# tsubo164/Fujiyama-Renderer

Hardware: AMD Instinct MI355X
Metric: Mray/s primary+secondary (and ms/frame) at 1920x1080 64spp (higher is better)
Workload: dtype f64; 1 GPU; dragon-class scene, 1920x1080, 8x8 spp, tile 32x32, 2040 tiles, 32 point lights; mesh=dragon, parallelism=tiles%1, tile_deal=auto, blas_build=host binned SAH

## Files before the change

### fujiyama-renderer_amd/csrc/device/fjgpu_api.hip

```cpp
#include <hip/hip_runtime.h>
#include <mutex>
#include <map>
#include <dlfcn.h>

#include <algorithm>
#include <array>
#include <cfloat>
#include <cmath>
#include <cstdio>
#include <cstdint>
#include <cstring>
#include <chrono>
#include <functional>
#include <memory>
#include <string>
#include <thread>
#include <vector>

#include "fjgpu.h"
#include "fjgpu_build.h"
#include "fjgpu_denoise.h"
#include "fjgpu_denoise_variance.h"
#include "fjgpu_temporal.h"
#include "fjgpu_kernels.h"
#include "fjgpu_lbvh.h"
#include "fjgpu_light_cone.h"
#include "fjgpu_raysort.h"
#include "fjgpu_tlas.h"

namespace {

thread_local std::string t_last_error;

int fail(int code, const std::string &msg)
{
  t_last_error = msg;
  return code;
}

#define HIP_TRY(expr) do { hipError_t e_ = (expr); if (e_ != hipSuccess) \
  return fail(FJGPU_ENODEV, std::string(#expr) + ": " + hipGetErrorString(e_)); } while (0)

#define FJ_LREC_BUFS 4

struct DeviceBuffers {
  std::vector<void *> ptrs;
  size_t bytes = 0;
  ~DeviceBuffers() { for (void *p : ptrs) (void) hipFree(p); }
  template <class T> int upload(const T *src, size_t n, const T **out)
  {
    *out = nullptr;
    if (n == 0 || src == nullptr) return 0;
    void *d = nullptr;
    if (hipMalloc(&d, n * sizeof(T)) != hipSuccess) return -1;
    ptrs.push_back(d);
    bytes += n * sizeof(T);
    if (hipMemcpy(d, src, n * sizeof(T), hipMemcpyHostToDevice) != hipSuccess) return -1;
    *out = static_cast<const T *>(d);
    return 0;
  }
  template <class T> int alloc(size_t n, T **out)
  {
    void *d = nullptr;
    if (hipMalloc(&d, std::max<size_t>(n, 1) * sizeof(T)) != hipSuccess) return -1;
    ptrs.push_back(d);
    bytes += std::max<size_t>(n, 1) * sizeof(T);
    *out = static_cast<T *>(d);
    return 0;
  }
};

struct Rccl {
  typedef void *comm_t;
  int (*CommInitAll)(comm_t *, int, const int *) = nullptr;
  int (*CommDestroy)(comm_t) = nullptr;
  int (*GroupStart)() = nullptr;
  int (*GroupEnd)() = nullptr;
  int (*Send)(const void *, size_t, int, int, comm_t, hipStream_t) = nullptr;
  int (*Recv)(void *, size_t, int, int, comm_t, hipStream_t) = nullptr;
  const char *(*GetErrorString)(int) = nullptr;
  void *handle = nullptr;
  bool ok = false;
  static constexpr int kFloat = 7;
};

Rccl &rccl()
{
  static Rccl R;
  static std::once_flag once;
  std::call_once(once, []() {
    for (const char *name : {"librccl.so.1", "librccl.so", "/opt/rocm/lib/librccl.so.1"}) { R.handle = dlopen(name, RTLD_NOW | RTLD_LOCAL); if (R.handle) break; }
    if (!R.handle) return;
    auto sym = [&](const char *n) { return dlsym(R.handle, n); };
    R.CommInitAll = (decltype(R.CommInitAll)) sym("ncclCommInitAll");
    R.CommDestroy = (decltype(R.CommDestroy)) sym("ncclCommDestroy");
    R.GroupStart = (decltype(R.GroupStart)) sym("ncclGroupStart");
    R.GroupEnd = (decltype(R.GroupEnd)) sym("ncclGroupEnd");
    R.Send = (decltype(R.Send)) sym("ncclSend");
    R.Recv = (decltype(R.Recv)) sym("ncclRecv");
    R.GetErrorString = (decltype(R.GetErrorString)) sym("ncclGetErrorString");
    R.ok = R.CommInitAll && R.CommDestroy && R.GroupStart && R.GroupEnd && R.Send && R.Recv;
  });
  return R;
}

#define FJ_RCCL_RETRY_CALLS 64
struct RcclSet { std::vector<Rccl::comm_t> comms; std::string why; int calls_since_failure = 0; };
std::mutex g_rccl_mu;
std::map<std::vector<int>, RcclSet> g_rccl_comms;

void rccl_destroy_all()
{
  Rccl &R = rccl();
  std::lock_guard<std::mutex> lock(g_rccl_mu);
  for (auto &kv : g_rccl_comms)
    for (Rccl::comm_t c : kv.second.comms) if (c && R.CommDestroy) (void) R.CommDestroy(c);
  g_rccl_comms.clear();
}

const std::vector<Rccl::comm_t> *rccl_comms(const std::vector<int> &devices, std::string *why)
{
  Rccl &R = rccl();
  if (!R.ok) { *why = "librccl.so not loadable"; return nullptr; }
  std::lock_guard<std::mutex> lock(g_rccl_mu);
  static bool hooked = false;
  if (!hooked) { hooked = true; atexit(rccl_destroy_all); }
  auto it = g_rccl_comms.find(devices);
  if (it != g_rccl_comms.end()) {
    if (!it->second.comms.empty()) return &it->second.comms;
    if (++it->second.calls_since_failure < FJ_RCCL_RETRY_CALLS) { *why = it->second.why + " (remembered)"; return nullptr; }
    g_rccl_comms.erase(it);
  }
  RcclSet set;
  set.comms.assign(devices.size(), nullptr);
  const int e = R.CommInitAll(set.comms.data(), (int) devices.size(), devices.data());
  if (e) { set.why = std::string("ncclCommInitAll: ") + (R.GetErrorString ? R.GetErrorString(e) : "error"); set.comms.clear(); *why = set.why; }
  auto &slot = g_rccl_comms[devices] = set;
  return slot.comms.empty() ? nullptr : &slot.comms;
}

}

struct fjgpu_scene {
  int device;
  DScene S;
  DeviceBuffers mem;
  double cam_fov;
  fj_camera_desc camera;
  int n_light_samples;
  long batch_tiles;
  long batch_samples = 0;
  long aov_batch_samples = 0;
  long render_calls = 0;
  long count_events;
  long light_cones = 1;
  int cone_rows = 0, cone_records = 0;
  long count_all_shadow;
  unsigned long long stack_peak_closest = 0, stack_peak_shadow = 0;
  std::unique_ptr<DeviceBuffers> work;
  size_t work_samples, work_rays;
  double *d_suv;
  uint32_t *d_stk = nullptr;
  float *d_accum;
  double *d_aseen = nullptr, *d_afinal = nullptr;
  uint8_t *d_apstate = nullptr, *d_acells = nullptr;
  const void *a_owner = nullptr;
  size_t a_samples = 0, a_cell_bytes = 0;
  struct Level { DRay *rays; DPath *paths; size_t cap; uint32_t *keys; float *fc; };
  bool has_filter_rays = false;
  std::vector<Level> levels;
  bool uses_sample_uid;
  int max_children;
  bool bounce_diffuse, bounce_reflect, bounce_refract;
  DHit *d_hits;
  DLightRec *d_lrecs[FJ_LREC_BUFS];
  DLightHair *d_lhair[FJ_LREC_BUFS];
  int lrec_bufs = 2;
  long overlap;
  bool overlap_now = false;
  size_t free_cached = 0;
  hipEvent_t ev_frame[2] = {nullptr, nullptr};
  long early_shadow = 0;
  hipStream_t shadow_stream;
  hipStream_t read_stream = nullptr;
  hipEvent_t ev_shaded = nullptr;
  hipEvent_t ev_shadow_done[FJ_LREC_BUFS];
  std::vector<hipEvent_t> ev_pool;
  DShadowRay *d_squeue;
  size_t squeue_rec_bytes = 0;
  size_t squeue_cap;
  uint32_t *d_join = nullptr; size_t join_cap = 0;
  bool split_overflowed = false;
  uint32_t split_kfac = 1;
  bool split_shadow = false;
  DCounters *d_cnt;
  TileDesc *d_tiles;
  double *d_jit, *d_tim;
  size_t tab_len;
  int tiles_cap;
  int stack_need;
  double tri_record_bytes;
  size_t blas_nodes;
  long blas_treelet_passes = 0;
  unsigned long long blas_treelets_changed = 0;
  double blas_sah_cost_initial = 0., blas_sah_cost = 0.;
  size_t squeue_max;
  size_t batch_fit_samples = 0;
  int ray_sort_bits = 0;
  double scene_box[6];
  uint32_t *d_sort[4] = {nullptr, nullptr, nullptr, nullptr};
  void *d_sort_tmp = nullptr; size_t sort_tmp_bytes = 0; size_t sort_cap = 0;
  float *d_frame = nullptr; size_t d_frame_n = 0;
  float *d_slab = nullptr; size_t d_slab_n = 0;
  int32_t *d_rects = nullptr; size_t d_rects_n = 0;
  fjgpu_batch_fn batch_fn = nullptr; void *batch_user = nullptr;
};

static int grow(void **p, size_t *have, size_t want, size_t elem)
{
  if (*have >= want && *p) return 0;
  if (*p) (void) hipFree(*p);
  *p = nullptr; *have = 0;
  if (hipMalloc(p, std::max<size_t>(want, 1) * elem) != hipSuccess) return -1;
  *have = want;
  return 0;
}

#ifndef FJ_OVERLAP_MAX_SAMPLES
#define FJ_OVERLAP_MAX_SAMPLES ((size_t) 24 << 20)
#endif
#ifndef FJ_OVERLAP_CULL_BLOCKS
#define FJ_OVERLAP_CULL_BLOCKS 1
#endif
static int enable_overlap(fjgpu_scene *sc)
{
  if (sc->shadow_stream) return 0;
  int prio_lo = 0, prio_hi = 0;
  if (getenv("FJGPU_OVERLAP_PRIO") && hipDeviceGetStreamPriorityRange(&prio_lo, &prio_hi) == hipSuccess && prio_lo != prio_hi) {
    if (hipStreamCreateWithPriority(&sc->shadow_stream, hipStreamNonBlocking, prio_lo) != hipSuccess) { sc->shadow_stream = nullptr; return -1; }
// ... 124 lines not shown
  for (size_t g = 0; g < hs.groups.size(); g++) if (!build_flat_group(hs, g, max_tris, &flats[g])) return false;
  out->swap(flats);
  return true;
}

static long g_ray_sort = -1;
static long g_ray_sort_min = FJ_RAY_SORT_MIN;
static long g_device_tlas = 1;
static long g_tlas_verify = 0;
static long g_split_shadow = 1;
static long g_compact_squeue = 1;
static long g_flat_groups = 1;
static long g_curve_anyhit = 1;
static long g_inst_lds = 1;
static long g_batch_tiles = 0;
static long g_device_build = -1;
static long g_treelet_passes = 0;
static long g_multi_exchange = 0;
static long g_spec_walk = 1;
static long g_cold_start = 1;
#ifndef FJ_COLD_BATCH_SAMPLES
#define FJ_COLD_BATCH_SAMPLES ((size_t) 16 << 20)
#endif
static long g_cold_batch_samples = (long) FJ_COLD_BATCH_SAMPLES;
static thread_local long g_single_frame = 0;

extern "C" {

int fjgpu_global_option(const char *name, long value)
{
  if (!name) return fail(FJGPU_EINVAL, "bad option call");
  if (std::string(name) == "ray_sort") { g_ray_sort = value < -1 ? -1 : (value > 9 ? 9 : value); return 0; }
  if (std::string(name) == "ray_sort_min") { g_ray_sort_min = value < 1 ? 1 : value; return 0; }
  if (std::string(name) == "device_tlas") { g_device_tlas = value != 0; return 0; }
  if (std::string(name) == "tlas_verify") { g_tlas_verify = value != 0; return 0; }
  if (std::string(name) == "split_shadow") { g_split_shadow = value != 0; return 0; }
  if (std::string(name) == "inst_lds") { g_inst_lds = value != 0; return 0; }
  if (std::string(name) == "curve_anyhit") { g_curve_anyhit = value != 0; return 0; }
  if (std::string(name) == "flat_groups") { g_flat_groups = value < 0 ? 0 : (value > 2 ? 2 : value); return 0; }
  if (std::string(name) == "compact_squeue") { g_compact_squeue = value != 0; return 0; }
  if (std::string(name) == "batch_tiles") { g_batch_tiles = value < 0 ? 0 : value; return 0; }
  if (std::string(name) == "device_build") { g_device_build = value < 0 ? -1 : (value > 2 ? 2 : value); return 0; }
  if (std::string(name) == "blas_treelet_passes") { g_treelet_passes = value < 0 ? 0 : (value > 8 ? 8 : value); return 0; }
  if (std::string(name) == "single_frame_build") { g_single_frame = value != 0; return 0; }
  if (std::string(name) == "speculative_walk") { g_spec_walk = value != 0; return 0; }
  if (std::string(name) == "anyhit_filter_off") { set_anyhit_filter_off(value); return 0; }
  if (std::string(name) == "cold_start") { g_cold_start = value != 0; return 0; }
  if (std::string(name) == "cold_batch_samples") { g_cold_batch_samples = value > 0 ? value : (long) FJ_COLD_BATCH_SAMPLES; return 0; }
  if (std::string(name) == "multi_exchange") { if (value < 0 || value > 1) return fail(FJGPU_EINVAL, "multi_exchange: 0 peer copies, 1 RCCL send / recv"); g_multi_exchange = value; return 0; }
  return fail(FJGPU_EINVAL, std::string("unknown global option ") + name);
}

const char *fjgpu_last_error(void) { return t_last_error.c_str(); }

int fjgpu_device_count(void)
{
  int n = 0;
  if (hipGetDeviceCount(&n) != hipSuccess) return 0;
  return n;
}

int fjgpu_tile_count(const fj_render_desc *render)
{
  if (!render) return 0;
  if (const char *why = bad_tiling(render)) { (void) fail(FJGPU_EINVAL, why); return 0; }
  std::vector<fjgpu::TileRect> t;
  fjgpu::GenerateTiles(*render, &t);
  return (int) t.size();
}

int fjgpu_tile_rect(const fj_render_desc *render, int tile_id, int32_t rect[4])
{
  if (!render || !rect) return fail(FJGPU_EINVAL, "null argument");
  if (const char *why = bad_tiling(render)) return fail(FJGPU_EINVAL, why);
  std::vector<fjgpu::TileRect> t;
  fjgpu::GenerateTiles(*render, &t);
  if (tile_id < 0 || tile_id >= (int) t.size()) return FJGPU_EINVAL;
  rect[0] = t[tile_id].xmin; rect[1] = t[tile_id].ymin; rect[2] = t[tile_id].xmax; rect[3] = t[tile_id].ymax;
  return 0;
}

}

static int upload_scene(const fj_scene_desc *desc, fjgpu::HostScene &hs, int device, fjgpu_scene **out)
{
  *out = nullptr;
  int ndev = 0;
  if (hipGetDeviceCount(&ndev) != hipSuccess || ndev == 0)
    return fail(FJGPU_ENODEV, "no HIP device visible: the fjgpu core has no CPU fallback");
  if (device < 0 || device >= ndev) return fail(FJGPU_EINVAL, "device index out of range");
  HIP_TRY(hipSetDevice(device));

  const auto t_up0 = std::chrono::steady_clock::now();
  auto lap = [&](const char *what) {
    if (getenv("FJGPU_VERBOSE")) { (void) hipDeviceSynchronize(); fprintf(stderr, "fjgpu: upload: %-28s at %.3f s\n", what,
        std::chrono::duration<double>(std::chrono::steady_clock::now() - t_up0).count()); }
  };
  std::unique_ptr<fjgpu_scene> sc(new fjgpu_scene());
  sc->device = device;
  sc->batch_tiles = g_batch_tiles;
  sc->count_events = 0;
  sc->count_all_shadow = 1;
  sc->work_samples = sc->work_rays = 0;
  sc->tab_len = 0;
  sc->overlap = 2;
  sc->shadow_stream = nullptr;
  for (int k = 0; k < FJ_LREC_BUFS; k++) { sc->ev_shadow_done[k] = nullptr; sc->d_lrecs[k] = nullptr; sc->d_lhair[k] = nullptr; }
  if (getenv("FJGPU_EARLY_SHADOW")) sc->early_shadow = atoi(getenv("FJGPU_EARLY_SHADOW"));
  if (const char *e = getenv("FJGPU_OVERLAP")) sc->overlap = std::max(0, std::min(2, atoi(e)));
  DeviceBuffers &M = sc->mem;
  int e = 0;

  std::vector<DPrimSet> dps(hs.primsets.size());
  for (size_t i = 0; i < hs.primsets.size(); i++) {
    const fjgpu::HostPrimSet &h = hs.primsets[i];
    DPrimSet &d = dps[i];
    std::memset(&d, 0, sizeof(d));
    d.type = h.type;
    d.root = h.root;
    d.n_prims = h.n_prims;
    std::memcpy(d.bounds, h.bounds, sizeof(d.bounds));
    for (int k = 0; k < 3; k++) { d.grid_cell[k] = h.grid_cell[k]; d.grid_n[k] = h.grid_n[k]; }
    if (!h.device_build) {
      e |= M.upload(h.nodes.data(), h.nodes.size(), &d.nodes);
      e |= M.upload(h.prim_ids.data(), h.prim_ids.size(), &d.prim_ids);
    }
    if (h.type == FJ_PRIMSET_MESH) {
      const fj_mesh_desc &m = *h.mesh;
      e |= M.upload(m.velocity, m.velocity ? (size_t) m.n_points * 3 : 0, &d.velocity);
      e |= M.upload(m.P, (size_t) m.n_points * 3, &d.P);
      e |= M.upload(m.N, m.N ? (size_t) m.n_points * 3 : 0, &d.N);
      e |= M.upload(m.vertex_N, m.vertex_N ? (size_t) m.n_faces * 9 : 0, &d.vN);
      e |= M.upload(m.uv, m.uv ? (size_t) m.n_points * 2 : 0, &d.uv);
      e |= M.upload(m.indices, (size_t) m.n_faces * 3, &d.indices);
      e |= M.upload(m.face_group, m.face_group ? (size_t) m.n_faces : 0, &d.face_group);
      if (h.device_build) {
        if (e) return fail(FJGPU_ENOMEM, "device allocation / upload failed while creating the scene");
        const auto tb0 = std::chrono::steady_clock::now();
        LbvhOut lo;
        std::string lerr;
        if (LbvhBuildMesh(d.P, d.velocity, d.indices, m.n_faces, m.n_points, h.bounds, h.f32_exact, hs.device_build_quality, hs.device_build_treelet_passes, &lo, &lerr))
          return fail(FJGPU_ENODEV, lerr);
        for (void *p : {(void *) lo.nodes, (void *) lo.prim_ids, (void *) lo.tri_verts, (void *) lo.tri_verts32, (void *) lo.tri_vel})
          if (p) M.ptrs.push_back(p);
        d.nodes = lo.nodes; d.prim_ids = lo.prim_ids; d.root = lo.root;
        d.tri_verts = lo.tri_verts; d.tri_verts32 = lo.tri_verts32; d.tri_vel = lo.tri_vel;
        hs.primsets[i].stack_need = lo.stack_need;
        sc->blas_treelet_passes += lo.treelet_passes; sc->blas_treelets_changed += lo.treelets_changed;
        sc->blas_sah_cost_initial += lo.sah_cost_initial; sc->blas_sah_cost += lo.sah_cost;
        hs.primsets[i].nodes.n = lo.n_nodes;
        if (lo.tri_verts32) hs.primsets[i].tri_verts32.resize(1);
        if (lo.tri_vel) hs.primsets[i].tri_vel.resize(1);
        if (getenv("FJGPU_VERBOSE") && m.n_faces > 100000)
          fprintf(stderr, "fjgpu: device BLAS build of %d triangles: %.3f s, %zu wide nodes\n", m.n_faces,
              std::chrono::duration<double>(std::chrono::steady_clock::now() - tb0).count(), lo.n_nodes);
      } else {
        e |= M.upload(h.tri_verts.data(), h.tri_verts.size(), &d.tri_verts);
        e |= M.upload(h.tri_verts32.data(), h.tri_verts32.size(), &d.tri_verts32);
        e |= M.upload(h.tri_vel.data(), h.tri_vel.size(), &d.tri_vel);
      }
    } else {
      e |= M.upload(h.curve_cp.data(), h.curve_cp.size(), &d.curve_cp);
      e |= M.upload(h.curve_width.data(), h.curve_width.size(), &d.curve_width);
      e |= M.upload(h.curve_Cd.data(), h.curve_Cd.size(), &d.curve_Cd);
      e |= M.upload(h.curve_depth.data(), h.curve_depth.size(), &d.curve_depth);
      e |= M.upload(h.curve_capsule.data(), h.curve_capsule.size(), &d.curve_capsule);
// ... 104 lines not shown
    }
    bool fits = lo != UINTPTR_MAX && lo % 128 == 0 && (hi - lo) / 128 < 0xffffffffull;
    for (size_t i = 0; i < dps.size(); i++) {
      const DPrimSet &P = dps[i];
      if (P.qnodes && (((uintptr_t) P.qnodes - lo) % 128 != 0 || (tris_of(P) - lo) % 128 != 0)) fits = false;
    }
    for (const DPrimSet &P : dps) if (P.qnodes && !P.tri_verts32) fits = false;
    S.blas_base = fits ? (const char *) lo : nullptr;
    if (!fits && lo != UINTPTR_MAX && getenv("FJGPU_VERBOSE"))
      fprintf(stderr, "fjgpu: BLAS arrays span %zu bytes from %p: no 32-bit offsets, the general shadow walk is used\n", (size_t) (hi - lo), (void *) lo);
    std::vector<DAnyInst> ai(hs.instances.size());
    for (size_t i = 0; i < hs.instances.size(); i++) {
      const DInstance &I = hs.instances[i];
      const DPrimSet &P = dps[I.primset];
      DAnyInst &a = ai[i];
      std::memset(&a, 0, sizeof(a));
      std::memcpy(a.Minv, I.Minv, sizeof(a.Minv));
      std::memcpy(a.bounds, P.bounds, sizeof(a.bounds));
      a.root = P.root;
      a.n_prims = (P.qnodes && S.blas_base) ? P.n_prims : 0;
      if (a.n_prims) {
        for (int k = 0; k < 3; k++) { a.qorigin[k] = qgrid[I.primset][k]; a.qcell[k] = qgrid[I.primset][3 + k]; }
        a.node_base = (uint32_t) (((uintptr_t) P.qnodes - lo) / 128);
        a.tri_base = (uint32_t) ((tris_of(P) - lo) / 128);
        a.tris_f32 = P.tri_verts32 ? 1 : 0;
        double bm = 0;
        for (int k = 0; k < 6; k++) bm = std::max(bm, std::fabs(P.bounds[k]));
        a.fbound = std::nextafter((float) bm, INFINITY);
      }
    }
    e |= M.upload(ai.data(), ai.size(), &S.any_insts);
  }
  if (g_device_tlas && e == 0 && !hs.groups.empty()) {
    std::vector<int> mcount(hs.groups.size()), nfirst, ncount;
    for (size_t g = 0; g < hs.groups.size(); g++) mcount[g] = hs.groups[g].n_instances;
    DTNode *d_nodes = nullptr;
    std::string terr;
    if (TlasBuildDevice(S.instances, hs.group_members, hs.group_member_first, mcount, &nfirst, &ncount, &d_nodes, &terr))
      return fail(FJGPU_ENODEV, terr);
    M.ptrs.push_back(d_nodes);
    size_t total = 0;
    for (int c : ncount) total += (size_t) c;
    if (g_tlas_verify) {
      std::vector<DTNode> got(total);
      HIP_TRY(hipMemcpy(got.data(), d_nodes, total * sizeof(DTNode), hipMemcpyDeviceToHost));
      bool same = total == hs.group_nodes.size();
      for (size_t g = 0; same && g < hs.groups.size(); g++) same = nfirst[g] == hs.groups[g].first && ncount[g] == hs.groups[g].count;
      if (same && total) same = std::memcmp(got.data(), hs.group_nodes.data(), total * sizeof(DTNode)) == 0;
      if (!same) return fail(FJGPU_ENODEV, "device TLAS build differs from the host's build");
    }
    std::vector<DGroup> groups = hs.groups;
    for (size_t g = 0; g < groups.size(); g++) { groups[g].first = nfirst[g]; groups[g].count = ncount[g]; }
    e |= M.upload(groups.data(), groups.size(), &S.groups);
    S.group_nodes = d_nodes;
    S.n_group_nodes = (int32_t) total;
  } else {
    e |= M.upload(hs.groups.data(), hs.groups.size(), &S.groups);
    e |= M.upload(hs.group_nodes.data(), hs.group_nodes.size(), &S.group_nodes);
    S.n_group_nodes = (int32_t) hs.group_nodes.size();
  }
  static_assert(sizeof(DInstEntry) == 8 * FJ_INST_LDS_ENTRY_WORDS && sizeof(DTNode) == 56 && sizeof(DGroup) == 64, "LDS copy of the instance level");
  S.curve_anyhit = (g_curve_anyhit && !getenv("FJGPU_NO_CURVE_ANYHIT")) ? 1 : 0;
  S.inst_lds = (g_inst_lds && !getenv("FJGPU_NO_INST_LDS")) ? 1 : 0;
  e |= M.upload(hs.shaders.data(), hs.shaders.size(), &S.shaders);
  e |= M.upload(hs.xforms.data(), hs.xforms.size(), &S.xforms);
  S.cam_xform = nullptr;
  if (!hs.cam_static) e |= M.upload(&hs.cam_xform, 1, &S.cam_xform);
  S.has_motion = hs.xforms.empty() ? 0 : 1;
  for (const auto &ps : hs.primsets) if (!ps.tri_vel.empty() || !ps.curve_vel.empty()) S.has_motion = 1;
  S.multi_shadow_groups = 0;
  for (const DInstance &I : hs.instances) {
    bool gathers = false;
    for (int k = 0; k < I.n_shaders; k++)
      if (I.shaders[k] >= 0 && (hs.shaders[I.shaders[k]].type == FJ_SHADER_PLASTIC || hs.shaders[I.shaders[k]].type == FJ_SHADER_HAIR)) gathers = true;
    if (gathers && I.shadow_target >= 0 && I.shadow_target < (int) hs.groups.size() && hs.groups[I.shadow_target].n_instances > 1)
      S.multi_shadow_groups = 1;
  }
  S.time_tab = nullptr; S.time_start = 0; S.time_end = 0;
  S.lrec_hair = nullptr;
  e |= M.upload(dtex.data(), dtex.size(), &S.textures);
  e |= M.upload(hs.light_samples.data(), hs.light_samples.size(), &S.light_samples);
  e |= M.upload(hs.area_lights.data(), hs.area_lights.size(), &S.area_lights);
  S.light_cones = nullptr; S.cone_rows = nullptr;
  {
    const size_t nl = hs.light_samples.size();
    std::vector<int32_t> rows(hs.groups.size(), -1);
    std::vector<DLightCone> cones;
    for (size_t g = 0; g < hs.groups.size() && nl; g++) {
      if (hs.groups[g].n_instances != 1) continue;
      const size_t at = cones.size();
      cones.resize(at + nl);
      int built = 0;
      double reach = 1e300;
      for (size_t l = 0; l < nl; l++) {
        DLightCone &C = cones[at + l];
        const DLightSample &LS = hs.light_samples[l];
        if (LS.type == FJ_POINT_LIGHT || LS.type == FJ_DOME_LIGHT) light_cone_build(LS.P, hs.groups[g].sbounds, &C);
        else std::memset(&C, 0, sizeof(C));
        if (C.count > 0) { built++; reach = std::min(reach, C.reach); }
      }
      if (!built) { cones.resize(at); continue; }
      for (size_t l = 0; l < nl; l++) cones[at + l].reach = reach;
      rows[g] = (int32_t) (at / nl);
      sc->cone_rows++; sc->cone_records += built;
    }
    if (!cones.empty()) {
      e |= M.upload(cones.data(), cones.size(), &S.light_cones);
      e |= M.upload(rows.data(), rows.size(), &S.cone_rows);
    }
  }
  S.has_area = hs.area_lights.empty() ? 0 : 1;
  if (e) return fail(FJGPU_ENOMEM, "device allocation / upload failed while creating the scene");
  S.n_light_samples = (int) hs.light_samples.size();
  S.n_instances = (int) hs.instances.size();
  S.n_groups = (int) hs.groups.size();
  S.n_primsets = (int) hs.primsets.size();
  int flat_stack_need = 0;
  S.flats = nullptr;
  {
    bool incoherent = false;
    for (int i = 0; i < desc->n_shaders; i++) {
      const fj_shader_desc &sh = desc->shaders[i];
      auto lum = [](const float *c) { return .298912 * c[0] + .586611 * c[1] + .114478 * c[2] > 0.; };
      if (sh.type == FJ_SHADER_GLASS) incoherent = true;
      if (sh.type == FJ_SHADER_PATHTRACING && (lum(sh.diffuse) || (int) lum(sh.reflect) + (int) lum(sh.refract) >= 2)) incoherent = true;
    }
    std::vector<HostFlat> hf;
    const bool flat_fits = S.inst_lds && S.n_instances <= FJ_FLAT_LDS_INSTS;
    const bool flat_wanted = incoherent || g_flat_groups >= 2 || getenv("FJGPU_FLAT_ALL");
    if (flat_wanted && flat_fits && g_flat_groups && !getenv("FJGPU_NO_FLAT") && FJ_CLOSEST_QNODES && build_flat_groups(hs, &hf)) {
      std::vector<DFlat> df(hf.size());
      for (size_t g = 0; g < hf.size() && !e; g++) {
        HostFlat &F = hf[g];
        DFlat &D = df[g];
        std::memset(&D, 0, sizeof(D));
        const DNode *d_nodes = nullptr;
        const size_t n_nodes = std::max<size_t>(1, F.tree.nodes.size());
        e |= M.upload(F.tree.nodes.data(), n_nodes, &d_nodes);
        DNodeQ *q = nullptr;
        if (!e && M.alloc(n_nodes, &q)) e = 1;
        if (!e && launch_quantize_nodes(nullptr, d_nodes, (uint32_t) n_nodes, &F.grid[0], &F.grid[3], q)) e = 1;
        D.nodes = q;
        e |= M.upload(F.refs.data(), F.refs.size(), &D.refs);
        e |= M.upload(F.refbox.data(), F.refbox.size(), &D.refbox);
        for (int a = 0; a < 3; a++) { D.qorigin[a] = F.grid[a]; D.qcell[a] = F.grid[3 + a]; }
        D.root = F.tree.root; D.n_inst = (int32_t) (F.refbox.size() / 6); D.n_prims = F.tree.n_prims;
        flat_stack_need = std::max(flat_stack_need, F.tree.stack_need);
      }
      if (!e) e |= M.upload(df.data(), df.size(), &S.flats);
      if (e) S.flats = nullptr;
      lap("flat groups");
    }
  }
  {
    int need = S.flats ? flat_stack_need : 0;
    for (const auto &ps : hs.primsets) need = std::max(need, ps.stack_need);
    S.stack_overflow = nullptr;
    S.stack_overflow_shadow = nullptr;
    bool any_curves = false;
    for (const auto &ps : hs.primsets) if (ps.type == FJ_PRIMSET_CURVE && ps.n_prims > 0) any_curves = true;
    (void) any_curves;
    const int lds_entries = FJ_STACK_LDS_MIN;
    if (need > lds_entries) {
      const size_t entries = (size_t) (need - lds_entries) * persistent_threads();
      if (M.alloc(entries, &S.stack_overflow) || M.alloc(entries, &S.stack_overflow_shadow)) return fail(FJGPU_ENOMEM, "device allocation failed for the traversal stack overflow area");
    }
    sc->stack_need = need;
    sc->tri_record_bytes = 36; sc->blas_nodes = 0;
    for (const auto &ps : hs.primsets) {
      sc->blas_nodes += ps.nodes.size();
      if (ps.type == FJ_PRIMSET_MESH && ps.n_prims > 0 && ps.tri_verts32.empty()) sc->tri_record_bytes = 72;
    }
    if (getenv("FJGPU_VERBOSE"))
      for (const auto &ps : hs.primsets)
        fprintf(stderr, "fjgpu: primset type %d prims %d nodes %zu binary depth %d stack need %d\n", ps.type, ps.n_prims,
            ps.nodes.size(), ps.max_depth, ps.stack_need);
  }
  S.has_curves = 0;
  S.all_opaque = 1;
  for (const auto &g : hs.groups) if (!g.all_opaque) S.all_opaque = 0;
  S.has_hair = 0;
  for (int i = 0; i < desc->n_shaders; i++) if (desc->shaders[i].type == FJ_SHADER_HAIR) S.has_hair = 1;
  for (const auto &ps : hs.primsets) if (ps.type == FJ_PRIMSET_CURVE && ps.n_prims > 0) S.has_curves = 1;
  S.target_group = hs.target_group;
  std::memcpy(S.cam_M, hs.cam_M, sizeof(S.cam_M));
  S.cam_znear = hs.cam_znear;
  S.cam_zfar = hs.cam_zfar;
  sc->cam_fov = hs.cam_fov;
  sc->camera = desc->camera;
  sc->n_light_samples = S.n_light_samples;
  sc->max_children = 0;
// ... 40 lines not shown
  lap("done");
  *out = sc.release();
  return 0;
}

static int build_host_scene(const fj_scene_desc *desc, fjgpu::HostScene *hs)
{
  std::string err;
  const auto t_build0 = std::chrono::steady_clock::now();
  long device_mode = g_device_build >= 0 ? g_device_build : (g_single_frame ? 1 : 0);
  if (const char *e = getenv("FJGPU_DEVICE_BUILD")) device_mode = std::max(0, std::min(2, atoi(e)));
  const bool device_build = device_mode != 0;
  hs->device_build_quality = device_mode == 2 ? 0 : 1;
  long passes = g_treelet_passes;
  if (const char *e = getenv("FJGPU_TREELET_PASSES")) passes = std::max(0, std::min(8, atoi(e)));
  hs->device_build_treelet_passes = (int) passes;
  const int be = fjgpu::BuildHostScene(desc, hs, &err, device_build);
  if (getenv("FJGPU_VERBOSE"))
    fprintf(stderr, "fjgpu: host scene build (BLAS, transforms, lights) %.3f s\n",
        std::chrono::duration<double>(std::chrono::steady_clock::now() - t_build0).count());
  if (be) return fail(be, err);
  return 0;
}

extern "C" {

int fjgpu_scene_create(const fj_scene_desc *desc, int device, fjgpu_scene **out)
{
  if (!out || !desc) return fail(FJGPU_EINVAL, "null argument");
  *out = nullptr;
  fjgpu::HostScene hs;
  if (const int be = build_host_scene(desc, &hs)) return be;
  return upload_scene(desc, hs, device, out);
}

int fjgpu_scene_create_multi(const fj_scene_desc *desc, const int *devices, int n_devices, fjgpu_scene **out)
{
  if (!out || !desc || !devices || n_devices < 1) return fail(FJGPU_EINVAL, "bad argument");
  for (int k = 0; k < n_devices; k++) out[k] = nullptr;
  fjgpu::HostScene hs;
  if (const int be = build_host_scene(desc, &hs)) return be;
  for (int k = 0; k < n_devices; k++) {
    const int e = upload_scene(desc, hs, devices[k], &out[k]);
    if (e) { for (int j = 0; j < k; j++) { fjgpu_scene_destroy(out[j]); out[j] = nullptr; } return e; }
  }
  return 0;
}

void fjgpu_scene_destroy(fjgpu_scene *scene)
{
  if (!scene) return;
  (void) hipSetDevice(scene->device);
  (void) hipDeviceSynchronize();
  if (getenv("FJGPU_PHASE_STATS")) debug_phase_stats();
  if (scene->shadow_stream) (void) hipStreamDestroy(scene->shadow_stream);
  if (scene->read_stream) (void) hipStreamDestroy(scene->read_stream);
  if (scene->ev_shaded) (void) hipEventDestroy(scene->ev_shaded);
  for (hipEvent_t e : scene->ev_shadow_done) if (e) (void) hipEventDestroy(e);
  for (hipEvent_t e : scene->ev_frame) if (e) (void) hipEventDestroy(e);
  for (hipEvent_t e : scene->ev_pool) (void) hipEventDestroy(e);
  if (scene->d_frame) (void) hipFree(scene->d_frame);
  if (scene->d_slab) (void) hipFree(scene->d_slab);
  if (scene->d_rects) (void) hipFree(scene->d_rects);
  delete scene;
}

int fjgpu_host_instance_level(const fj_scene_desc *desc, int group, int32_t *out_inst, int32_t *out_skip, double *out_box, int cap)
{
  if (!desc || group < 0 || group >= desc->n_groups) return fail(FJGPU_EINVAL, "bad instance-level query");
  fjgpu::HostScene hs;
  std::string err;
  const int e = fjgpu::BuildHostScene(desc, &hs, &err, true);
  if (e) return fail(e, err);
  const DGroup &G = hs.groups[group];
  for (int k = 0; k < G.count && k < cap; k++) {
    const DTNode &nd = hs.group_nodes[G.first + k];
    if (out_inst) out_inst[k] = nd.inst;
    if (out_skip) out_skip[k] = nd.inst < 0 ? nd.skip - G.first : 0;
    if (out_box) std::memcpy(out_box + 6 * (size_t) k, nd.box, sizeof(nd.box));
  }
  return G.count;
}

int fjgpu_scene_query(const fjgpu_scene *scene, const char *name, double *value)
{
  if (!scene || !name || !value) return fail(FJGPU_EINVAL, "bad query call");
  const std::string n(name);
  if (n == "node_record_bytes") { *value = (double) sizeof(DNode); return 0; }
  if (n == "anyhit_node_record_bytes") { *value = (double) sizeof(DNodeQ); return 0; }
  if (n == "tri_record_bytes") { *value = scene->tri_record_bytes; return 0; }
  if (n == "scene_bytes") { *value = (double) scene->mem.bytes; return 0; }
  if (n == "work_bytes") { *value = (double) (scene->work ? scene->work->bytes : 0); return 0; }
  if (n == "stack_need") { *value = scene->stack_need; return 0; }
  if (n == "blas_nodes") { *value = (double) scene->blas_nodes; return 0; }
  if (n == "blas_treelet_passes") { *value = (double) scene->blas_treelet_passes; return 0; }
  if (n == "blas_treelets_changed") { *value = (double) scene->blas_treelets_changed; return 0; }
  if (n == "blas_sah_cost_initial") { *value = scene->blas_sah_cost_initial; return 0; }
  if (n == "blas_sah_cost") { *value = scene->blas_sah_cost; return 0; }
  if (n == "stack_peak") { *value = (double) std::max(scene->stack_peak_closest, scene->stack_peak_shadow); return 0; }
  if (n == "stack_peak_closest") { *value = (double) scene->stack_peak_closest; return 0; }
  if (n == "stack_peak_shadow") { *value = (double) scene->stack_peak_shadow; return 0; }
  if (n == "stack_lds") { *value = FJ_STACK_LDS; return 0; }
  if (n == "stack_lds_anyhit") { *value = FJ_STACK_LDS_ANYHIT; return 0; }
  if (n == "stack_lds_curves") { *value = FJ_STACK_LDS_CURVES; return 0; }
  if (n == "stack_lds_min") { *value = FJ_STACK_LDS_MIN; return 0; }
  if (n == "curve_anyhit") {
    const DScene &S = scene->S;
    *value = (S.has_curves && !S.has_motion && S.all_opaque && S.curve_anyhit && S.inst_lds && S.n_group_nodes <= FJ_INST_LDS_NODES_CURVES &&
              S.n_instances <= FJ_INST_LDS_INSTS_CURVES && S.n_groups <= FJ_INST_LDS_GROUPS_CURVES && FJ_CURVE_QNODES && FJ_CLOSEST_QNODES) ? 1 : 0;
    return 0;
  }
  if (n == "lean_anyhit") { *value = (scene->S.all_opaque && !scene->S.has_curves && !scene->S.has_motion && scene->S.blas_base) ? 1 : 0; return 0; }
  if (n == "closest_kernel") {
    const DScene &S = scene->S;
    const bool flat = !S.has_motion && !S.has_curves && S.flats;
    *value = S.has_motion ? 3 : (S.has_curves ? 2 : (flat ? 4 : (S.incoherent_rays ? 1 : 0)));
    return 0;
  }
  if (n == "closest_node_record_bytes") { *value = (double) ((scene->S.has_motion || (scene->S.has_curves && !FJ_CURVE_QNODES) || !FJ_CLOSEST_QNODES) ? sizeof(DNode) : sizeof(DNodeQ)); return 0; }
  if (n == "light_cone_rows") { *value = scene->cone_rows; return 0; }
  if (n == "light_cone_records") { *value = scene->cone_records; return 0; }
  if (n == "light_cone_verdicts" || n == "light_cone_contradictions") {
    double v = -1, c = -1;
    if (hipSetDevice(scene->device) != hipSuccess || hipDeviceSynchronize() != hipSuccess) return fail(FJGPU_ENODEV, "hipSetDevice / hipDeviceSynchronize");
    light_cone_validate_counts(&v, &c);
    *value = n == "light_cone_verdicts" ? v : c;
    return 0;
  }
  if (n == "has_curves") { *value = scene->S.has_curves; return 0; }
  if (n == "has_motion") { *value = scene->S.has_motion; return 0; }
  return fail(FJGPU_EINVAL, "unknown query " + n);
}

int fjgpu_set_batch_callback(fjgpu_scene *scene, fjgpu_batch_fn fn, void *user)
{
  if (!scene) return fail(FJGPU_EINVAL, "null scene");
  scene->batch_fn = fn; scene->batch_user = fn ? user : nullptr;
  return 0;
}

int fjgpu_dev_rccl_selftest(int device, int n_floats)
{
  int nd = 0;
  if (hipGetDeviceCount(&nd) != hipSuccess || device < 0 || device >= nd) return fail(FJGPU_ENODEV, "no such HIP device");
  if (n_floats < 1) return fail(FJGPU_EINVAL, "bad size");
  HIP_TRY(hipSetDevice(device));
  std::string why;
  const std::vector<Rccl::comm_t> *comms = rccl_comms(std::vector<int>{device}, &why);
  if (!comms) return fail(FJGPU_ENODEV, "RCCL: " + why);
  Rccl &R = rccl();
  DeviceBuffers M;
  std::vector<float> src((size_t) n_floats), got((size_t) n_floats, -1.f);
  for (int i = 0; i < n_floats; i++) src[(size_t) i] = (float) (i % 1013) * .5f;
  const float *d_src = nullptr;
  float *d_dst = nullptr;
  if (M.upload(src.data(), src.size(), &d_src) || M.alloc(src.size(), &d_dst)) return fail(FJGPU_ENOMEM, "device allocation failed");
  HIP_TRY(hipMemset(d_dst, 0xff, sizeof(float) * src.size()));
  int e = R.GroupStart();
  if (!e) e = R.Send(d_src, src.size(), Rccl::kFloat, 0, (*comms)[0], nullptr);
  if (!e) e = R.Recv(d_dst, src.size(), Rccl::kFloat, 0, (*comms)[0], nullptr);
  const int e2 = R.GroupEnd();
  if (e || e2) return fail(FJGPU_ENODEV, std::string("RCCL self exchange: ") + (R.GetErrorString ? R.GetErrorString(e ? e : e2) : "error"));
  HIP_TRY(hipStreamSynchronize(nullptr));
  HIP_TRY(hipMemcpy(got.data(), d_dst, sizeof(float) * got.size(), hipMemcpyDeviceToHost));
  for (size_t i = 0; i < got.size(); i++) if (got[i] != src[i]) return fail(FJGPU_ENODEV, "RCCL self exchange returned other data");
  return 0;
}

int fjgpu_dev_sort_pairs(int device, const uint32_t *keys, int n, int key_bits, uint32_t *keys_out, uint32_t *perm, int repeats, double *sort_ms)
{
  if (n < 0 || key_bits < 1 || key_bits > 32 || (n > 0 && !keys)) return fail(FJGPU_EINVAL, "bad sort call");
  int nd = 0;
  if (hipGetDeviceCount(&nd) != hipSuccess || device < 0 || device >= nd) return fail(FJGPU_ENODEV, "no such HIP device");
  HIP_TRY(hipSetDevice(device));
  if (sort_ms) *sort_ms = 0;
  if (n == 0) return 0;
  DeviceBuffers M;
  const uint32_t *d_keys = nullptr;
  uint32_t *d_out = nullptr, *d_perm = nullptr;
  char *d_tmp = nullptr;
  const size_t tmp_bytes = ray_sort_pairs_temp_bytes((uint32_t) n, key_bits);
  if (M.upload(keys, (size_t) n, &d_keys) || M.alloc((size_t) n, &d_out) || M.alloc((size_t) n, &d_perm) || M.alloc(tmp_bytes, &d_tmp))
    return fail(FJGPU_ENOMEM, "device allocation failed for the sort");
  hipEvent_t e0, e1;
  HIP_TRY(hipEventCreate(&e0));
  HIP_TRY(hipEventCreate(&e1));
  double best = 1e30;
  for (int k = 0; k < std::max(1, repeats); k++) {
    (void) hipEventRecord(e0, nullptr);
    if (ray_sort_pairs(nullptr, d_keys, (uint32_t) n, key_bits, d_out, d_perm, d_tmp, tmp_bytes, keys_out != nullptr)) { (void) hipEventDestroy(e0); (void) hipEventDestroy(e1); return fail(FJGPU_ENODEV, "the sort's launches failed"); }
    (void) hipEventRecord(e1, nullptr);
    if (hipEventSynchronize(e1) != hipSuccess) { (void) hipEventDestroy(e0); (void) hipEventDestroy(e1); return fail(FJGPU_ENODEV, std::string("sort: ") + hipGetErrorString(hipGetLastError())); }
    float ms = 0.f;
    (void) hipEventElapsedTime(&ms, e0, e1);
    best = std::min(best, (double) ms);
  }
  (void) hipEventDestroy(e0); (void) hipEventDestroy(e1);
  if (sort_ms) *sort_ms = best;
  if (keys_out) HIP_TRY(hipMemcpy(keys_out, d_out, sizeof(uint32_t) * (size_t) n, hipMemcpyDeviceToHost));
  if (perm) HIP_TRY(hipMemcpy(perm, d_perm, sizeof(uint32_t) * (size_t) n, hipMemcpyDeviceToHost));
  return 0;
}

int fjgpu_set_option(fjgpu_scene *scene, const char *name, long value)
{
  if (!scene || !name) return fail(FJGPU_EINVAL, "bad option call");
  const std::string n(name);
  if (n == "batch_tiles") { scene->batch_tiles = value; return 0; }
  if (n == "batch_samples") { scene->batch_samples = value < 0 ? 0 : value; return 0; }
  if (n == "aov_batch_samples") { scene->aov_batch_samples = value < 0 ? 0 : value; return 0; }
  if (n == "count_nodes") { scene->count_events = value != 0; return 0; }
  if (n == "count_all_shadow") { scene->count_all_shadow = value != 0; return 0; }
  if (n == "light_cones") { scene->light_cones = value != 0; return 0; }
  if (n == "overlap_shadow") {
    if (value < 0 || value > 2) return fail(FJGPU_EINVAL, "overlap_shadow: 0 off, 1 on, 2 by the batch size");
    scene->overlap = value;
    return 0;
  }
  if (n == "release_work") {
    if (value && scene->work) {
      if (hipSetDevice(scene->device) != hipSuccess) return fail(FJGPU_ENODEV, "hipSetDevice");
      (void) hipDeviceSynchronize();
      scene->work.reset();
      scene->work_samples = scene->work_rays = 0; scene->tiles_cap = 0; scene->lrec_bufs = std::min(scene->lrec_bufs, 2); scene->squeue_rec_bytes = 0;
      scene->sort_cap = 0; scene->a_owner = nullptr; scene->a_samples = 0; scene->a_cell_bytes = 0;
      scene->d_aseen = scene->d_afinal = nullptr; scene->d_apstate = scene->d_acells = nullptr;
      for (auto &L : scene->levels) { L.rays = nullptr; L.paths = nullptr; L.cap = 0; L.keys = nullptr; }
    }
    return 0;
  }
  return fail(FJGPU_EINVAL, "unknown option " + n);
}

}

namespace {

struct BatchTile { fjgpu::TileRect r; int nx, ny; uint32_t offset; };


bool scene_compact_squeue(const DScene &S)
{
  const bool lean = S.all_opaque && !S.has_curves && !S.has_motion && S.blas_base;
  const bool curve_walk = S.has_curves && !S.has_motion && S.all_opaque && S.curve_anyhit && S.inst_lds && S.n_group_nodes <= FJ_INST_LDS_NODES_CURVES &&
      S.n_instances <= FJ_INST_LDS_INSTS_CURVES && S.n_groups <= FJ_INST_LDS_GROUPS_CURVES && FJ_CURVE_QNODES && FJ_CLOSEST_QNODES;
  return (lean || curve_walk) && !S.has_area && g_compact_squeue && !getenv("FJGPU_NO_COMPACT_SQUEUE");
}

int ensure_work(fjgpu_scene *sc, size_t samples, size_t rays, int tiles, size_t tab_len)
{
  const int want_bufs = sc->overlap_now ? FJ_LREC_BUFS : 2;
  const size_t rec_bytes = scene_compact_squeue(sc->S) ? sizeof(DShadowRayC) : sizeof(DShadowRay);
  if (samples > sc->work_samples || rays > sc->work_rays || tiles > sc->tiles_cap || want_bufs > sc->lrec_bufs || rec_bytes > sc->squeue_rec_bytes) {
    samples = std::max(samples, sc->work_samples); rays = std::max(rays, sc->work_rays); tiles = std::max(tiles, sc->tiles_cap);
    const int old_bufs = sc->lrec_bufs;
    sc->lrec_bufs = samples > sc->work_samples ? want_bufs : std::max(sc->lrec_bufs, want_bufs);
    sc->work.reset(new DeviceBuffers());
    sc->sort_cap = 0; sc->a_owner = nullptr; sc->a_samples = 0; sc->a_cell_bytes = 0;
    sc->d_aseen = sc->d_afinal = nullptr; sc->d_apstate = sc->d_acells = nullptr;
    DeviceBuffers &W = *sc->work;
    int e = 0;
    e |= W.alloc(samples * 2, &sc->d_suv);
    sc->d_stk = nullptr;
    if (sc->uses_sample_uid && !sc->S.has_motion && !sc->S.cam_xform) e |= W.alloc(samples * 2, &sc->d_stk);
    e |= W.alloc(samples * 4, &sc->d_accum);
    for (auto &L : sc->levels) { L.rays = nullptr; L.paths = nullptr; L.cap = 0; L.keys = nullptr; }
    e |= W.alloc(rays, &sc->d_hits);
    for (int k = 0; k < sc->lrec_bufs; k++) {
      e |= W.alloc(rays, &sc->d_lrecs[k]);
      sc->d_lhair[k] = nullptr;
      if (sc->S.has_hair) e |= W.alloc(rays, &sc->d_lhair[k]);
    }
    const size_t per_ray = std::max<size_t>(sc->split_shadow ? 16 : 8, std::min<size_t>(64, (size_t) std::max(1, sc->n_light_samples) * (sc->split_shadow ? 2 : 1)));
    const size_t lrec_bound = std::min<size_t>(rays, std::max<size_t>(samples * 4, (size_t) 1 << 16));
    sc->squeue_cap = std::min<size_t>(lrec_bound * per_ray, sc->squeue_max) + 4096 * 1024;
    { char *q = nullptr; e |= W.alloc(sc->squeue_cap * rec_bytes, &q); sc->d_squeue = (DShadowRay *) q; sc->squeue_rec_bytes = e ? 0 : rec_bytes; }
    sc->d_join = nullptr; sc->join_cap = 0;
    if (sc->split_shadow) { sc->join_cap = sc->squeue_cap + 1 + 32 * (persistent_threads() / 64) * 64; e |= W.alloc(sc->join_cap, &sc->d_join); }
    e |= W.alloc(1, &sc->d_cnt);
    e |= W.alloc((size_t) tiles, &sc->d_tiles);
    if (e) { sc->work.reset(); sc->work_samples = sc->work_rays = 0; sc->tiles_cap = 0; sc->lrec_bufs = std::min(old_bufs, 2); sc->squeue_rec_bytes = 0; return -1; }
    sc->work_samples = samples; sc->work_rays = rays; sc->tiles_cap = tiles;
  }
  if (tab_len > sc->tab_len) {
    std::vector<double> draws;
    fjgpu::XorShiftTable(2 * tab_len, &draws);
    if (sc->mem.upload(draws.data(), 2 * tab_len, const_cast<const double **>(&sc->d_jit))) return -1;
    if (sc->mem.upload(draws.data(), tab_len, const_cast<const double **>(&sc->d_tim))) return -1;
    sc->tab_len = tab_len;
  }
  return 0;
}

int ensure_adaptive(fjgpu_scene *sc, size_t samples, size_t cell_bytes)
{
  if (sc->a_owner == sc->work.get() && samples <= sc->a_samples && cell_bytes <= sc->a_cell_bytes) return 0;
  DeviceBuffers &W = *sc->work;
  if (W.alloc(samples * 4, &sc->d_aseen) || W.alloc(samples * 4, &sc->d_afinal) || W.alloc(samples, &sc->d_apstate) ||
      W.alloc(cell_bytes, &sc->d_acells)) { sc->a_owner = nullptr; return -1; }
  sc->a_owner = sc->work.get(); sc->a_samples = samples; sc->a_cell_bytes = cell_bytes;
  return 0;
}

int ensure_level(fjgpu_scene *sc, int level, size_t cap)
{
  fjgpu_scene::Level &L = sc->levels[level];
  if (L.cap >= cap) return 0;
  DeviceBuffers &W = *sc->work;
  if (W.alloc(cap, &L.rays) || W.alloc(cap, &L.paths)) return -1;
  L.keys = nullptr;
  L.fc = nullptr;
  if (sc->has_filter_rays && level >= 1 && W.alloc(cap * 3, &L.fc)) return -1;
  if (sc->ray_sort_bits > 0 && level >= 1 && W.alloc(cap, &L.keys)) return -1;
  L.cap = cap;
  return 0;
}

int ensure_sort(fjgpu_scene *sc, size_t cap)
{
  if (sc->sort_cap >= cap) return 0;
  DeviceBuffers &W = *sc->work;
  sc->d_sort[0] = sc->d_sort[2] = nullptr;
  if (W.alloc(cap, &sc->d_sort[1]) || W.alloc(cap, &sc->d_sort[3])) return -1;
  sc->sort_tmp_bytes = ray_sort_temp_bytes((uint32_t) cap, sc->ray_sort_bits);
  char *tmp = nullptr;
  if (W.alloc(sc->sort_tmp_bytes, &tmp)) return -1;
  sc->d_sort_tmp = tmp;
  sc->sort_cap = cap;
  return 0;
}


}

extern "C" {

static int render_tiles_once(fjgpu_scene *sc, const fj_render_desc *r, const int32_t *tile_ids, int n_tiles,
    float *d_fb, void *hip_stream, fjgpu_stats *stats);

int fjgpu_render_tiles(fjgpu_scene *sc, const fj_render_desc *r, const int32_t *tile_ids, int n_tiles,
    float *d_fb, void *hip_stream, fjgpu_stats *stats)
{
  if (!sc || !r || !d_fb) return fail(FJGPU_EINVAL, "null argument");
  sc->split_overflowed = false;
  int e = render_tiles_once(sc, r, tile_ids, n_tiles, d_fb, hip_stream, stats);
  if (e == FJGPU_ENOMEM && sc->split_overflowed) {
    fprintf(stderr, "fjgpu: shadow queue overflow with rays split per candidate instance: rendering the tiles again without the split, "
        "which stays off for this scene (option split_shadow)\n");
    sc->split_shadow = false;
    e = render_tiles_once(sc, r, tile_ids, n_tiles, d_fb, hip_stream, stats);
  }
  if (!e) sc->render_calls++;
  return e;
}

static int render_tiles_once(fjgpu_scene *sc, const fj_render_desc *r, const int32_t *tile_ids, int n_tiles,
    float *d_fb, void *hip_stream, fjgpu_stats *stats)
{
  const bool adaptive = r->sampler_type == 1;
  if (r->sampler_type != 0 && !adaptive) return fail(FJGPU_EINVAL, "unknown sampler_type");
  if (adaptive && (r->adaptive_max_subdivision < 0 || r->adaptive_max_subdivision > 8 || !(r->adaptive_subdivision_threshold >= 0)))
    return fail(FJGPU_EINVAL, "adaptive_max_subdivision must be in [0, 8] and adaptive_subdivision_threshold >= 0");
  if (const char *why = bad_render(r)) return fail(FJGPU_EINVAL, why);
  HIP_TRY(hipSetDevice(sc->device));
  hipStream_t st = static_cast<hipStream_t>(hip_stream);
  sc->stack_peak_closest = sc->stack_peak_shadow = 0;

  std::vector<fjgpu::TileRect> all;
  fjgpu::GenerateTiles(*r, &all);
  std::vector<int> ids;
  if (tile_ids) ids.assign(tile_ids, tile_ids + n_tiles);
  else for (size_t i = 0; i < all.size(); i++) ids.push_back((int) i);
  for (int id : ids) if (id < 0 || id >= (int) all.size()) return fail(FJGPU_EINVAL, "tile id out of range");

  int margin[2];
  fjgpu::SamplerMargin(*r, margin);
  const int a_div = adaptive ? 1 << r->adaptive_max_subdivision : 1;
  if (adaptive) {
    margin[0] = (int) std::ceil((double) r->filter_w - 1);
    margin[1] = (int) std::ceil((double) r->filter_h - 1);
  }
  const size_t full_tile_samples = adaptive
      ? (size_t) (a_div * (r->tile_w + 2 * margin[0]) + 1) * (size_t) (a_div * (r->tile_h + 2 * margin[1]) + 1)
      : (size_t) (r->rate_x * r->tile_w + 2 * margin[0]) * (r->rate_y * r->tile_h + 2 * margin[1]);

  auto query_free = [&]() {
    size_t free_b = 0, total_b = 0;
    if (hipMemGetInfo(&free_b, &total_b) != hipSuccess) free_b = (size_t) 16 << 30;
    sc->free_cached = free_b + (sc->work ? sc->work->bytes : 0);
  };
  if (!sc->work || sc->free_cached == 0) query_free();
  size_t free_now = sc->free_cached;
  const int deepest = (sc->bounce_diffuse ? std::max(0, r->max_diffuse_depth) : 0) +
      (sc->bounce_reflect ? std::max(0, r->max_reflect_depth) : 0) + (sc->bounce_refract ? std::max(0, r->max_refract_depth) : 0);
  if (sc->levels.size() < (size_t) deepest + 1) sc->levels.resize((size_t) deepest + 1, fjgpu_scene::Level{nullptr, nullptr, 0, nullptr});
  long bt = sc->batch_tiles;
  if (bt <= 0 && sc->batch_samples > 0) bt = std::max<long>(1, (long) ((size_t) sc->batch_samples / full_tile_samples));
  if (bt <= 0 && sc->render_calls == 0 && g_cold_start && !adaptive) {
    static const int on = [] { const char *e = getenv("FJGPU_COLD_START"); return e ? atoi(e) : 1; }();
    if (on) bt = std::max<long>(1, (long) ((size_t) g_cold_batch_samples / full_tile_samples));
  }
  if (bt <= 0) {
    const size_t per_sample = 32 + (size_t) (deepest + 1) * (sizeof(DRay) + sizeof(DPath) + (sc->has_filter_rays ? 12 : 0)) + sizeof(DHit) + 2 * sizeof(DLightRec) + (adaptive ? 72 : 0) +
        ((sc->ray_sort_bits > 0 && deepest >= 1) ? 24 : 0);
    const double share = sc->n_light_samples == 0 ? .6 : .4;
    const size_t target = std::min<size_t>((size_t) 160 << 20, (size_t) (share * (double) free_now) / per_sample);
    bt = std::max<long>(1, (long) (target / full_tile_samples));
  }
  bt = std::min<long>(bt, (long) ids.size());
  bt = std::min<long>(bt, (long) (((size_t) 1 << 31) / full_tile_samples));
  if (sc->batch_fit_samples && full_tile_samples * (size_t) bt > sc->batch_fit_samples) bt = std::max<long>(1, (long) (sc->batch_fit_samples / full_tile_samples));
  if (bt < 1) bt = 1;
  sc->overlap_now = !adaptive && sc->n_light_samples > 0 && (sc->overlap == 1 || (sc->overlap == 2 && deepest >= 1 && full_tile_samples * (size_t) bt <= FJ_OVERLAP_MAX_SAMPLES));
  if (sc->overlap_now && enable_overlap(sc)) sc->overlap_now = false;
  if (!sc->read_stream) {
    if (hipStreamCreateWithFlags(&sc->read_stream, hipStreamNonBlocking) != hipSuccess) sc->read_stream = nullptr;
    else if (hipEventCreateWithFlags(&sc->ev_shaded, hipEventDisableTiming) != hipSuccess) { (void) hipStreamDestroy(sc->read_stream); sc->read_stream = nullptr; sc->ev_shaded = nullptr; }
  }
  sc->squeue_max = std::max<size_t>((size_t) 4 << 20, std::min<size_t>((size_t) 512 << 20, (size_t) (.2 * (double) free_now) / sizeof(DShadowRay)));
  if (sc->n_light_samples == 0) sc->squeue_max = (size_t) 4 << 20;
  if (const char *e = getenv("FJGPU_SQUEUE_M")) sc->squeue_max = (size_t) std::max(1, atoi(e)) << 20;
  size_t cap_samples = 0, cap_rays = 0;
  bool requeried = false;
  for (;;) {
    cap_samples = full_tile_samples * (size_t) bt;
    cap_rays = std::max<size_t>(cap_samples, std::min<size_t>((size_t) 8 << 20, cap_samples * 16)) + 1024;
    if (!requeried && sc->work && (cap_samples > sc->work_samples || cap_rays > sc->work_rays || (int) bt > sc->tiles_cap ||
                                   (sc->overlap_now ? FJ_LREC_BUFS : 2) > sc->lrec_bufs)) {
      requeried = true;
      query_free();
      free_now = sc->free_cached;
      if (!getenv("FJGPU_SQUEUE_M") && sc->n_light_samples != 0)
        sc->squeue_max = std::max<size_t>((size_t) 4 << 20, std::min<size_t>((size_t) 512 << 20, (size_t) (.2 * (double) free_now) / sizeof(DShadowRay)));
    }
    bool ok = ensure_work(sc, cap_samples, cap_rays, (int) bt, full_tile_samples) == 0;
    const bool level0_implicit = !adaptive && sc->S.cam_xform == nullptr && (!sc->uses_sample_uid || !sc->S.has_motion) && !getenv("FJGPU_EXPLICIT_CAMERA_RAYS");
    for (int l = level0_implicit ? 1 : 0; ok && l <= deepest; l++) ok = ensure_level(sc, l, cap_rays) == 0;
    if (ok && sc->ray_sort_bits > 0 && deepest >= 1) ok = ensure_sort(sc, cap_rays) == 0;
    if (ok) break;
    (void) hipGetLastError();
    if (bt == 1) return fail(FJGPU_ENOMEM, "device allocation failed for the wavefront work buffers");
    sc->work.reset(); sc->work_samples = sc->work_rays = 0; sc->tiles_cap = 0; sc->free_cached = 0;
    for (auto &L : sc->levels) { L.rays = nullptr; L.paths = nullptr; L.cap = 0; L.keys = nullptr; }
    sc->a_owner = nullptr; sc->a_samples = 0; sc->a_cell_bytes = 0;
    sc->sort_cap = 0;
    bt = std::max<long>(1, bt / 2);
    sc->batch_fit_samples = full_tile_samples * (size_t) bt;
  }
  const size_t a_cells0_cap = adaptive ? (size_t) bt * (size_t) (r->tile_w + 2 * margin[0]) * (size_t) (r->tile_h + 2 * margin[1]) : 0;
  const size_t a_cell_bytes = a_cells0_cap * (((((size_t) 1) << (2 * (r->adaptive_max_subdivision + 1))) - 1) / 3);
  if (adaptive && a_cells0_cap >= ((size_t) 1 << 32)) return fail(FJGPU_EINVAL, "too many lattice cells per batch: lower the batch_tiles option");
  if (adaptive && ensure_adaptive(sc, cap_samples, a_cell_bytes))
    return fail(FJGPU_ENOMEM, "device allocation failed for the adaptive sampler's buffers");

  DScene S = sc->S;
  const double aspect = r->xres / (double) r->yres;
  S.cam_uv_size[1] = fjgpu::CameraUvSizeY(sc->cam_fov);
  S.cam_uv_size[0] = S.cam_uv_size[1] * aspect;
  S.time_tab = sc->d_tim; S.time_start = r->time_start; S.time_end = r->time_end;
  S.lrec_hair = nullptr;

  GenParams gp;
  gp.rate_x = r->rate_x; gp.rate_y = r->rate_y; gp.margin_x = margin[0]; gp.margin_y = margin[1];
  gp.udelta = 1. / (r->rate_x * r->xres);
  gp.vdelta = 1. / (r->rate_y * r->yres);
  gp.jitter = r->jitter;
  gp.jittered = r->jitter > 0 ? 1 : 0;
  gp.pad = 0;
  ShadeParams shp;
  shp.max_diffuse_depth = r->max_diffuse_depth; shp.max_reflect_depth = r->max_reflect_depth; shp.max_refract_depth = r->max_refract_depth;
  shp.count_all_shadow = (int) sc->count_all_shadow;
  shp.ray_capacity = (uint32_t) cap_rays; shp.light_capacity = (uint32_t) cap_rays;
  shp.fc_in = nullptr; shp.fc_out = nullptr;
  shp.next_keys = nullptr; shp.sort_bits = std::max(1, std::min(9, sc->ray_sort_bits)); shp.pad_ = 0;
  ray_sort_grid(sc->scene_box, shp.sort_bits, shp.sort_lo, shp.sort_scale);
  ShadowParams swp;
  swp.cos_half_pi = std::cos(3.14159265358979323846 / 2.);
  swp.cos_pi = std::cos(3.14159265358979323846);
  swp.pre_resolve = (S.all_opaque && !S.has_curves && !S.has_motion && S.blas_base) ? 1 : 0;
  swp.cast_shadow = r->cast_shadow;
  S.compact_squeue = scene_compact_squeue(S) ? 1 : 0;
  S.pad_cs_ = 0;
  swp.compact = S.compact_squeue;
  swp.light_cones = (sc->light_cones && S.light_cones && S.cone_rows) ? 1 : 0;
  swp.queue_capacity = (uint32_t) sc->squeue_cap;
  swp.join_capacity = (swp.pre_resolve && sc->split_shadow && sc->d_join) ? (uint32_t) sc->join_cap : 0u;
  S.shadow_join = swp.join_capacity ? sc->d_join : nullptr;
  S.shadow_queue_cap = (uint32_t) sc->squeue_cap;
  ResolveParams rp;
  rp.xres = r->xres; rp.yres = r->yres; rp.rate_x = r->rate_x; rp.rate_y = r->rate_y;
  rp.npx_x = r->rate_x + 2 * margin[0]; rp.npx_y = r->rate_y + 2 * margin[1];
  AdaptiveParams ap;
  std::memset(&ap, 0, sizeof(ap));
  if (adaptive) {
    ap.D = r->adaptive_max_subdivision; ap.div = a_div;
    ap.margin_x = margin[0]; ap.margin_y = margin[1];
    ap.udelta = 1. / (a_div * r->xres);
    ap.vdelta = 1. / (a_div * r->yres);
    ap.jitter = r->jitter;
    ap.jittered = r->jitter > 0 ? 1 : 0;
    ap.threshold = (double) r->adaptive_subdivision_threshold;
    ap.ray_capacity = (uint32_t) cap_rays;
    rp.rate_x = rp.rate_y = a_div;
    rp.npx_x = a_div * (1 + 2 * margin[0]) + 1; rp.npx_y = a_div * (1 + 2 * margin[1]) + 1;
  }
  rp.fw = (double) r->filter_w; rp.fh = (double) r->filter_h;

  fjgpu_stats acc;
  std::memset(&acc, 0, sizeof(acc));
  float ms = 0;
  struct Span { size_t a, b; double *bucket; };
  std::vector<Span> spans;
  size_t ev_used = 0;
  auto take_event = [&]() -> size_t {
    if (ev_used == sc->ev_pool.size()) { hipEvent_t e = nullptr; if (hipEventCreate(&e) != hipSuccess) return (size_t) -1; sc->ev_pool.push_back(e); }
    return ev_used++;
  };
  auto timed = [&](hipStream_t stream, double *bucket, auto &&launch) -> int {
    const size_t a = take_event(), b = take_event();
    if (a == (size_t) -1 || b == (size_t) -1) return -1;
    (void) hipEventRecord(sc->ev_pool[a], stream);
    const int le = launch();
    (void) hipEventRecord(sc->ev_pool[b], stream);
    if (le) return le;
    spans.push_back(Span{a, b, bucket});
    return 0;
  };
  hipStream_t sst = (sc->overlap_now && sc->shadow_stream) ? sc->shadow_stream : st;
  unsigned shade_seq = 0;
  bool shadow_pending[FJ_LREC_BUFS] = {false, false, false, false};
  const unsigned lrec_ring = (sst != st && sc->lrec_bufs >= FJ_LREC_BUFS) ? FJ_LREC_BUFS : 2;
  int rc = 0;
  hipEvent_t *ev_all = sc->ev_frame;
  if (!ev_all[0]) { HIP_TRY(hipEventCreate(&ev_all[0])); HIP_TRY(hipEventCreate(&ev_all[1])); }
  (void) hipEventRecord(ev_all[0], st);

  for (size_t b0 = 0; b0 < ids.size() && rc == 0; b0 += (size_t) bt) {
    const int nb = (int) std::min<size_t>((size_t) bt, ids.size() - b0);
    std::vector<TileDesc> td(nb);
    uint32_t off = 0, max_ts = 0, cell_off = 0;
    int max_px = 0, max_w0 = 0, max_h0 = 0;
    for (int k = 0; k < nb; k++) {
      const fjgpu::TileRect &t = all[ids[b0 + k]];
      TileDesc &d = td[k];
      d.xmin = t.xmin; d.ymin = t.ymin; d.xmax = t.xmax; d.ymax = t.ymax; d.id = t.id;
      d.nx = r->rate_x * (t.xmax - t.xmin) + 2 * margin[0];
      d.ny = r->rate_y * (t.ymax - t.ymin) + 2 * margin[1];
      d.cell_offset = cell_off; d.pad = 0;
      if (adaptive) {
        const int w0 = t.xmax - t.xmin + 2 * margin[0], h0 = t.ymax - t.ymin + 2 * margin[1];
        d.nx = a_div * w0 + 1; d.ny = a_div * h0 + 1;
        cell_off += (uint32_t) w0 * (uint32_t) h0;
        max_w0 = std::max(max_w0, w0); max_h0 = std::max(max_h0, h0);
      }
      d.sample_offset = off;
      off += (uint32_t) d.nx * (uint32_t) d.ny;
      max_ts = std::max(max_ts, (uint32_t) d.nx * (uint32_t) d.ny);
      max_px = std::max(max_px, (t.xmax - t.xmin) * (t.ymax - t.ymin));
    }
    const uint32_t n_samples = off;
    if ((hipMemcpyAsync(sc->d_tiles, td.data(), sizeof(TileDesc) * nb, hipMemcpyHostToDevice, st)) != hipSuccess) { rc = -1; break; }
    (void) hipMemsetAsync(sc->d_accum, 0, sizeof(float) * 4 * (size_t) n_samples, st);
    (void) hipMemsetAsync(sc->d_cnt, 0, sizeof(DCounters), st);

    const bool tk_cam = sc->uses_sample_uid && !S.has_motion && sc->d_stk != nullptr;
    const bool implicit_cam = !adaptive && S.cam_xform == nullptr && (!sc->uses_sample_uid || tk_cam) && !getenv("FJGPU_EXPLICIT_CAMERA_RAYS");
    if (!adaptive) {
// ... 122 lines not shown
            bound_is_exact = false;
            sq_dirty = true;
            b += can;
          }
          if (sst != st) { (void) hipEventRecord(sc->ev_shadow_done[lb], sst); shadow_pending[lb] = true; }
          if (sst != st && sc->early_shadow > 0 && level == (int) sc->early_shadow - 1 && can_emit && hc.next_count) { e = flush_shadow(Sl); if (e) return e; }
        }
        if (hc.next_count) {
          if (!can_emit) return fail(FJGPU_EINVAL, "ray recursion deeper than the depth limits allow");
          walk_launched = launched_next;
          e = process(level + 1, hc.next_count);
          if (e) return e;
        }
      }
      return 0;
    };
    auto finish_shadow = [&]() -> int {
      DScene Sf = S; Sf.lrec_hair = nullptr;
      const int fe = flush_shadow(Sf);
      if (fe) return fe;
      if (sst != st) { (void) hipEventRecord(sc->ev_shadow_done[0], sst); shadow_pending[0] = true; }
      for (int k = 0; k < FJ_LREC_BUFS; k++) if (shadow_pending[k] && sst != st) { (void) hipStreamWaitEvent(st, sc->ev_shadow_done[k], 0); shadow_pending[k] = false; }
      return 0;
    };
    if (!adaptive) {
      rc = process(0, n_samples);
      if (rc) break;
      rc = finish_shadow();
      if (rc) break;
    } else {
      ap.cells0 = cell_off;
      (void) hipMemsetAsync(sc->d_apstate, 0, (size_t) n_samples, st);
      (void) hipMemsetAsync(sc->d_acells, 0, (size_t) cell_off * (((((size_t) 1) << (2 * (ap.D + 1))) - 1) / 3), st);
      rc = timed(st, &acc.gen_ms, [&]() { return launch_adaptive_uv(st, ap, sc->d_tiles, nb, max_ts, sc->d_jit, sc->d_suv); });
      for (int level = 0; level <= ap.D && rc == 0; level++) {
        ap.level = level;
        (void) hipMemsetAsync(&sc->d_cnt->cam_count, 0, sizeof(uint32_t), st);
        const uint32_t max_pts = (uint32_t) ((max_w0 << level) + 1) * (uint32_t) ((max_h0 << level) + 1);
        rc = timed(st, &acc.gen_ms, [&]() {
          return launch_adaptive_points(st, S, ap, sc->d_tiles, nb, max_pts, sc->d_acells, sc->d_suv, sc->d_accum, sc->d_apstate,
              sc->d_aseen, sc->levels[0].rays, sc->levels[0].paths, sc->d_cnt);
        });
        if (rc) break;
        DCounters hc;
        if (hipMemcpyAsync(&hc, sc->d_cnt, sizeof(hc), hipMemcpyDeviceToHost, st) != hipSuccess || hipStreamSynchronize(st) != hipSuccess) { rc = -1; break; }
        if (hc.overflow) { rc = fail(FJGPU_ENOMEM, "camera ray queue overflow in the adaptive sampler"); break; }
        acc.rays.camera += hc.cam_count;
        if (hc.cam_count) {
          rc = process(0, hc.cam_count);
          if (rc) break;
          rc = finish_shadow();
          if (rc) break;
        }
        rc = timed(st, &acc.resolve_ms, [&]() {
          return launch_adaptive_decide(st, ap, sc->d_tiles, nb, (uint32_t) (max_w0 << level) * (uint32_t) (max_h0 << level),
              sc->d_acells, sc->d_accum, sc->d_apstate, sc->d_aseen);
        });
      }
      if (rc) break;
      rc = timed(st, &acc.resolve_ms, [&]() {
        return launch_adaptive_fill(st, ap, sc->d_tiles, nb, max_ts, sc->d_acells, sc->d_accum, sc->d_apstate, sc->d_aseen, sc->d_afinal);
      });
      if (rc) break;
    }
    rc = timed(st, &acc.resolve_ms, [&]() {
      return launch_resolve(st, rp, sc->d_tiles, nb, max_px, sc->d_suv, sc->d_accum, adaptive ? sc->d_afinal : nullptr, d_fb);
    });
    if (rc) break;
    DCounters hc;
    if (hipMemcpyAsync(&hc, sc->d_cnt, sizeof(hc), hipMemcpyDeviceToHost, st) != hipSuccess || hipStreamSynchronize(st) != hipSuccess) { rc = -1; break; }
    if (hc.overflow) { sc->split_overflowed = S.shadow_join != nullptr; rc = fail(FJGPU_ENOMEM, "wavefront queue overflow: lower the batch_tiles option"); break; }
    acc.rays.shadow += hc.rays[CXT_SHADOW_RAY];
    acc.rays.diffuse += hc.rays[CXT_DIFFUSE_RAY];
    acc.rays.reflect += hc.rays[CXT_REFLECT_RAY];
    acc.rays.refract += hc.rays[CXT_REFRACT_RAY];
    acc.nodes_visited += hc.nodes;
    acc.prims_tested += hc.prims;
    acc.insts_tested += hc.insts;
    acc.rays_traced += hc.traced;
    acc.shadow_traversed += hc.squeued;
    acc.shadow_nodes += hc.sh_nodes; acc.shadow_prims += hc.sh_prims; acc.shadow_insts += hc.sh_insts;
    sc->stack_peak_closest = std::max(sc->stack_peak_closest, hc.stack_peak);
    sc->stack_peak_shadow = std::max(sc->stack_peak_shadow, hc.sh_stack_peak);
    acc.batches++;
    if (sc->batch_fn) {
      const std::vector<int32_t> bids(ids.begin() + (long) b0, ids.begin() + (long) b0 + nb);
      if (sc->batch_fn(sc->batch_user, sc->device, bids.data(), nb)) { acc.interrupted = 1; break; }
    }
  }
  (void) hipEventRecord(ev_all[1], st);
  hipError_t se = hipStreamSynchronize(st);
  if (sst != st) { const hipError_t s2 = hipStreamSynchronize(sst); if (se == hipSuccess) se = s2; }
  if (rc == 0 && se == hipSuccess) {
    (void) hipEventElapsedTime(&ms, ev_all[0], ev_all[1]);
    acc.total_ms = ms;
    for (const Span &sp : spans)
      if (hipEventElapsedTime(&ms, sc->ev_pool[sp.a], sc->ev_pool[sp.b]) == hipSuccess) *sp.bucket += ms;
    acc.closest_ms += acc.sort_ms;
    acc.trace_ms = acc.closest_ms + acc.light_loop_ms + acc.shadow_walk_ms;
  }
  if (rc > 0 || rc == -1) return fail(FJGPU_ENODEV, std::string("HIP failure in the wavefront loop: ") + hipGetErrorString(hipGetLastError()));
  if (rc) return rc;
  if (se != hipSuccess) return fail(FJGPU_ENODEV, std::string("stream synchronize: ") + hipGetErrorString(se));
  if (stats) *stats = acc;
  return 0;
}

int fjgpu_render_frame_multi(fjgpu_scene *const *scenes, int n_scenes, const fj_render_desc *r,
    const int32_t *tile_ids, int n_tiles, float *h_fb, fjgpu_stats *stats)
{
  if (!scenes || n_scenes < 1 || !r || !h_fb) return fail(FJGPU_EINVAL, "null argument");
  for (int k = 0; k < n_scenes; k++) if (!scenes[k]) return fail(FJGPU_EINVAL, "null scene");
  if (const char *why = bad_render(r)) return fail(FJGPU_EINVAL, why);
  std::vector<fjgpu::TileRect> all;
  fjgpu::GenerateTiles(*r, &all);
  std::vector<int32_t> ids;
  if (tile_ids) ids.assign(tile_ids, tile_ids + std::max(0, n_tiles));
  else for (size_t i = 0; i < all.size(); i++) ids.push_back((int32_t) i);
  for (int32_t id : ids) if (id < 0 || id >= (int32_t) all.size()) return fail(FJGPU_EINVAL, "tile id out of range");
  const int G = n_scenes;
  const size_t npx = (size_t) r->xres * r->yres;
  const int tile_px = r->tile_w * r->tile_h;
  std::vector<std::vector<int32_t>> mine(G);
  for (size_t k = 0; k < ids.size(); k++) mine[k % G].push_back(ids[k]);
  fjgpu_scene *first = scenes[0];

  HIP_TRY(hipSetDevice(first->device));
  if (grow((void **) &first->d_frame, &first->d_frame_n, npx * 4, sizeof(float))) return fail(FJGPU_ENOMEM, "device allocation failed for the frame");
  HIP_TRY(hipMemset(first->d_frame, 0, npx * 4 * sizeof(float)));
  std::vector<size_t> stage_off(G, 0);
  size_t stage_px = 0, rects_n = 0;
  for (int d = 1; d < G; d++) { stage_off[d] = stage_px; stage_px += mine[d].size() * (size_t) tile_px; rects_n += mine[d].size(); }
  if (G > 1) {
    if (grow((void **) &first->d_slab, &first->d_slab_n, stage_px * 4, sizeof(float)) ||
        grow((void **) &first->d_rects, &first->d_rects_n, rects_n * 4, sizeof(int32_t)))
      return fail(FJGPU_ENOMEM, "device allocation failed for the tile slabs");
  }

  const std::vector<Rccl::comm_t> *comms = nullptr;
  {
    bool want = g_multi_exchange == 1;
    if (const char *e = getenv("FJGPU_MULTI_RCCL")) want = atoi(e) != 0;
    std::vector<int> devs(G);
    for (int d = 0; d < G; d++) devs[d] = scenes[d]->device;
    std::vector<int> uniq = devs;
    std::sort(uniq.begin(), uniq.end());
    const bool distinct = std::adjacent_find(uniq.begin(), uniq.end()) == uniq.end();
    if (want && G > 1 && distinct) {
      std::string why;
      comms = rccl_comms(devs, &why);
      if (!comms && getenv("FJGPU_VERBOSE")) fprintf(stderr, "fjgpu: RCCL exchange not available (%s): peer copies\n", why.c_str());
    }
  }
  std::vector<int> rcs(G, 0);
  std::vector<std::string> errs(G);
  std::vector<fjgpu_stats> sts(G);
  auto work = [&](int d) {
    fjgpu_scene *sc = scenes[d];
    fjgpu_stats &st = sts[d];
    std::memset(&st, 0, sizeof(st));
    auto bad = [&](int code, const std::string &m) { rcs[d] = code; errs[d] = m; };
    if (hipSetDevice(sc->device) != hipSuccess) return bad(FJGPU_ENODEV, "hipSetDevice failed");
    if (mine[d].empty()) return;
    float *fb = first->d_frame;
    if (d > 0) {
      if (grow((void **) &sc->d_frame, &sc->d_frame_n, npx * 4, sizeof(float)) ||
// ... 778 lines not shown
```

### fujiyama-renderer_amd/csrc/device/fjgpu_dev_anyhit.h

```cpp
#ifndef FJGPU_DEV_ANYHIT_H
#define FJGPU_DEV_ANYHIT_H


#ifndef FJ_ANYHIT_F32
#define FJ_ANYHIT_F32 1
#endif
#if FJ_ANYHIT_F32
#define FJ_ANYHIT_RAY_WORDS 10
#else
#define FJ_ANYHIT_RAY_WORDS 14
#endif

__device__ __forceinline__ uint32_t opaque_lane_id()
{
  uint32_t t;
  asm volatile("v_mbcnt_lo_u32_b32 %0, -1, 0\n\tv_mbcnt_hi_u32_b32 %0, -1, %0" : "=v"(t));
  return t;
}
#ifndef FJ_NO_SCHED_FENCE
#define FJ_SCHED_FENCE() __builtin_amdgcn_sched_barrier(0)
#else
#define FJ_SCHED_FENCE() do { } while (0)
#endif
__device__ __forceinline__ bool tri_ray_anyhit(V3 v0, V3 v1, V3 v2, V3 orig, V3 dir, double tmin, double tmax)
// ... 44 lines not shown
#define AH_TID() (wave_first + opaque_lane_id())
  typedef __attribute__((address_space(3))) uint32_t ah_lds_u32;
  typedef __attribute__((address_space(3))) double ah_lds_f64;
  ah_lds_u32 *const ls_stack = (ah_lds_u32 *) s_stack;
  const uint32_t ah_base = (uint32_t) (uintptr_t) ls_stack;
  const uint32_t ah_row1 = ah_base + BLOCK * 4u, ah_ovf0 = ah_base + (uint32_t) FJ_STACK_LDS_ANYHIT * BLOCK * 4u;
#define AH_AT(addr) (*(ah_lds_u32 *) (uintptr_t) (addr))
#define AH_OVF(addr) S.stack_overflow_shadow[(size_t) ((((addr) - ah_base) >> 10) - FJ_STACK_LDS_ANYHIT) * (gridDim.x * BLOCK) + (size_t) blockIdx.x * BLOCK + AH_TID()]
  auto push = [&](uint32_t &spa_, uint32_t v) { if (spa_ < ah_ovf0) AH_AT(spa_) = v; else AH_OVF(spa_) = v; spa_ += BLOCK * 4u; };
  auto pop = [&](uint32_t &spa_) -> uint32_t { spa_ -= BLOCK * 4u; uint32_t v_; if (spa_ < ah_ovf0) v_ = AH_AT(spa_); else v_ = AH_OVF(spa_); return v_; };
  bool head_live = true;
  uint32_t next = 0, range_end = 0;
  tune.grab = adaptive_grab(tune.grab, n);
  QueueClaim qc;
  qc.init(xheads, n, tune.grab);
  bool have = false;
  uint32_t idx = 0;
#if FJ_ANYHIT_F32
  typedef __attribute__((address_space(3))) float ah_lds_f32;
  ah_lds_f32 *const s_ray = (ah_lds_f32 *) (ls_stack + FJ_STACK_LDS_ANYHIT * BLOCK);
  uint32_t pex = TRAV_DONE;
#define AH_PEX_STALL 0x80000000u
  int winst = 0;
#else
  ah_lds_f64 *const s_ray = (ah_lds_f64 *) (ls_stack + FJ_STACK_LDS_ANYHIT * BLOCK);
#endif
  Slab32P s32;
  s32.ix = s32.iy = s32.iz = 0.f; s32.lhx = s32.lhy = s32.lhz = (fj_v2f) (0.f);
  float tmax32 = 0.f;
  const float tmin32 = 9.9999e-5f;
  int gi = 0, gend = 0;
  uint32_t node_base = 0, tri_base = 0;
  uint32_t cur = TRAV_DONE;
  uint32_t pleaf = TRAV_DONE;
#define AH_POSTPONE() do { if (cur != TRAV_DONE && (cur & FJ_LEAF_FLAG) && pleaf == TRAV_DONE && spa >= ah_row1) { pleaf = cur; cur = pop(spa); } } while (0)
#define AH_PLEAF_NEXT() do { pleaf = TRAV_DONE; } while (0)
#define AH_PLEAF_CLEAR() do { pleaf = TRAV_DONE; } while (0)
  uint32_t spa = ah_base;
  const double tmin = .0001;
#ifdef FJ_PHASE_STATS
  unsigned long long ph[16] = {0, 0, 0, 0, 0, 0, 0, 0, 0, 0, 0, 0, 0, 0, 0, 0};
#endif

#ifdef FJ_WAVE_TIMELINE
  uint32_t ray_steps = 0;
#endif
  FJ_TL_DECL();
  for (;;) {
    PH(0, 1);
    FJ_TL_ITER(!head_live && next >= range_end);
    AH_POSTPONE();
    const bool walk_over = cur == TRAV_DONE && pleaf == TRAV_DONE;
#if FJ_ANYHIT_F32
    const bool has_pex = pex != TRAV_DONE;
    const bool stalled = has_pex && (pex & AH_PEX_STALL);
#else
    const bool has_pex = false, stalled = false;
#endif
    const bool fin = walk_over && !has_pex;
    const bool at_inner = cur != TRAV_DONE && !(cur & FJ_LEAF_FLAG);
    const bool at_leaf = (pleaf != TRAV_DONE || (cur != TRAV_DONE && (cur & FJ_LEAF_FLAG))) && !stalled;
    const unsigned long long m_leaf = __ballot(at_leaf), m_inner = __ballot(at_inner);
    const unsigned n_leaf = (unsigned) __popcll(m_leaf), n_inner = (unsigned) __popcll(m_inner);
    const bool can_fetch = head_live || next < range_end;
    const unsigned long long m_turn = __ballot(fin && (have || can_fetch));
    const unsigned n_turn = (unsigned) __popcll(m_turn);

#if FJ_ANYHIT_F32
    {
      const unsigned long long m_ex = __ballot(has_pex);
      if (m_ex != 0ull && ((unsigned) __popcll(m_ex) >= tune.exact_min || __ballot(has_pex && (walk_over || stalled)) != 0ull)) {
        PH(12, 1); PH(13, __popcll(m_ex));
        if (has_pex) {
          V3 o, d;
          double tmax;
          sq_ray(S, squeue, idx, &o, &d, &tmax);
          const DAnyInst *A = &S.any_insts[kMulti ? winst : ~SQ_FIELD(S, squeue, idx, group)];
          const V3 oo_ = xpoint(A->Minv, o), od_ = xvector(A->Minv, d);
          FJ_SCHED_FENCE();
          V3 v0, v1, v2;
          load_tri(nullptr, (const float *) (S.blas_base + ((size_t) tri_base << 7)), pex & ~AH_PEX_STALL, &v0, &v1, &v2);
          if (tri_ray_anyhit(v0, v1, v2, oo_, od_, tmin, tmax)) {
            have = false; cur = TRAV_DONE; AH_PLEAF_CLEAR();
#ifdef FJ_WAVE_TIMELINE
            FJ_TL_RAY(ray_steps);
#endif
            PH(10, 1); PH(14, 1);
          }
          pex = TRAV_DONE;
        }
        continue;
      }
    }
#endif
    if (n_turn >= TRAV_REFILL || (n_inner == 0 && n_leaf == 0)) {
      if (m_turn == 0ull) { FJ_TL_END(); break; }
      PH(1, 1); PH(2, n_turn);
      if (next >= range_end && head_live) { head_live = qc.claim(lane, &next, &range_end); FJ_TL_CLAIM(); }
      bool fetch = false;
      if (fin) {
        fetch = true;
        if (have) {
          if (kMulti && gi < gend) fetch = false;
          else {
            bool add = true;
            if (!kMulti && S.shadow_join) {
              const uint32_t slot1 = SQ_FIELD(S, squeue, idx, tindex);
              if (slot1) { const uint32_t old = atomicAdd(&S.shadow_join[slot1 - 1u], 1u); add = ((old & 0xffffu) + 1u) == (old >> 16); }
            }
            if (add) {
              float *acc = s_accum + 4 * (size_t) SQ_FIELD(S, squeue, idx, sample);
              const float *qc_ = sq_colour(S, squeue, idx);
              const float r0 = qc_[0], r1 = qc_[1], r2 = qc_[2];
              if (r0 != 0.f) atomicAdd(acc + 0, r0);
              if (r1 != 0.f) atomicAdd(acc + 1, r1);
              if (r2 != 0.f) atomicAdd(acc + 2, r2);
            }
            have = false;
#ifdef FJ_WAVE_TIMELINE
            FJ_TL_RAY(ray_steps);
#endif
          }
        }
      }
      const unsigned long long m_fetch = __ballot(fetch);
      if (fetch) {
        const uint32_t my = next + __builtin_amdgcn_mbcnt_hi((uint32_t) (m_fetch >> 32), __builtin_amdgcn_mbcnt_lo((uint32_t) m_fetch, 0u));
        if (my < range_end) {
          const int g = SQ_FIELD(S, squeue, my, group);
          if (SQ_FIELD(S, squeue, my, sample) != SQ_INVALID) {
#ifdef FJ_WAVE_TIMELINE
            ray_steps = 0;
#endif
            have = true;
            idx = my;
            if (!kMulti || g < 0) { gi = g; gend = 0; }
            else { gi = S.groups[g].first; gend = gi + S.groups[g].count; }
          }
        }
      }
      next += (uint32_t) __popcll(m_fetch);
      if (next > range_end) next = range_end;
      if (fin && have) {
        V3 o, d;
        double tmax;
        sq_ray(S, squeue, idx, &o, &d, &tmax);
        V3 winv = o;
        bool plain = false, single = false, dead = false;
        if (kMulti && gi >= 0) {
          dead = has_negative_zero(d);
          winv = mk(filter_rcp(d.x), filter_rcp(d.y), filter_rcp(d.z));
          plain = plain_dir(d);
          single = S.groups[SQ_FIELD(S, squeue, idx, group)].n_instances == 1;
          if (dead) gi = gend;
        }
        for (;;) {
          int inst = -1;
          if (gi < 0) { inst = ~gi; gi = gend = 0; if (kCount) lc->insts++; }
          else if (!kMulti) break;
          else {
            while (gi < gend) {
              const DTNode *tn_ = &S.group_nodes[gi];
              if (tn_->inst < 0) {
                double tq;
                gi = slab(tn_->box, tn_->box + 3, o, winv, tmin, tmax, &tq) ? gi + 1 : tn_->skip;
                continue;
// ... 60 lines not shown
        const FJ_GLOBAL fj_v4u *nd = (const FJ_GLOBAL fj_v4u *) (S.blas_base + ((size_t) node_base << 7) + ((size_t) cur << 6));
        if (kCount) lc->nodes++;
#ifdef FJ_WAVE_TIMELINE
        ray_steps++;
#endif
        const fj_v4u w0 = nd[0], w1 = nd[1], w2 = nd[2], e = nd[3];
        const uint32_t shx = slab32_shift(s32.ix), shy = slab32_shift(s32.iy), shz = slab32_shift(s32.iz);
        const bool h0 = slab32q_test(w0.x, w0.y, w0.z, s32, shx, shy, shz, tmin32, tmax32);
        FJ_SCHED_FENCE();
        const bool h1 = slab32q_test(w0.w, w1.x, w1.y, s32, shx, shy, shz, tmin32, tmax32);
        FJ_SCHED_FENCE();
        const bool h2 = slab32q_test(w1.z, w1.w, w2.x, s32, shx, shy, shz, tmin32, tmax32) && e.z != FJ_NO_CHILD;
        FJ_SCHED_FENCE();
        const bool h3 = slab32q_test(w2.y, w2.z, w2.w, s32, shx, shy, shz, tmin32, tmax32) && e.w != FJ_NO_CHILD;
        FJ_SCHED_FENCE();
        uint32_t r0 = e.x, r1 = e.y, r2 = e.z, r3 = e.w;
        if (!h2) { r2 = r3; }
        if (!h1) { r1 = r2; r2 = r3; }
        if (!h0) { r0 = r1; r1 = r2; r2 = r3; }
        const int nh = (int) h0 + (int) h1 + (int) h2 + (int) h3;
        if (nh == 0) cur = (spa < ah_row1) ? TRAV_DONE : pop(spa);
        else {
          cur = r0;
          if (!deep) {
            ah_lds_u32 *top = &AH_AT(spa);
            top[0] = r1; top[BLOCK] = r2; top[2 * BLOCK] = r3;
            spa += (uint32_t) (nh - 1) * (BLOCK * 4u);
          } else {
            if (nh > 1) push(spa, r1);
            if (nh > 2) push(spa, r2);
            if (nh > 3) push(spa, r3);
          }
          if (kCount) { const uint32_t row = (spa - ah_base) / (BLOCK * 4u); if (row > lc->stack_peak) lc->stack_peak = row; }
        }
        AH_POSTPONE();
      }
      }
    } else {
      PH(5, 1); PH(6, n_leaf);
      PH(9, __popcll(__ballot(fin))); PH(11, __popcll(__ballot(!at_leaf && !fin)));
      if (at_leaf) {
        const bool from_p = pleaf != TRAV_DONE;
        const uint32_t lf = from_p ? pleaf : cur;
        const uint32_t first = (lf & 0x7fffffffu) >> 3;
        const uint32_t more = lf & 7u;
        if (kCount) lc->prims++;
#if FJ_ANYHIT_F32
        TriFilterRay fr;
        {
          ah_lds_f32 *const rp_ = &s_ray[AH_TID()];
          fr.ohx = rp_[0]; fr.ohy = rp_[BLOCK]; fr.ohz = rp_[2 * BLOCK]; fr.olx = rp_[3 * BLOCK]; fr.oly = rp_[4 * BLOCK]; fr.olz = rp_[5 * BLOCK];
          fr.dx = rp_[6 * BLOCK]; fr.dy = rp_[7 * BLOCK]; fr.dz = rp_[8 * BLOCK]; fr.tfl = rp_[9 * BLOCK];
          fr.tmin_lo = 9.9999800e-05f; fr.tmin_hi = 1.0000020e-04f; fr.tmax_lo = tmax32 * 0.99999619f; fr.tmax_hi = tmax32 * 1.0000039f;
        }
        const int verdict = tri_filter32<true>((const FJ_GLOBAL float *) (S.blas_base + ((size_t) tri_base << 7)) + (size_t) first * 9, fr);
#ifdef FJ_TRI_FILTER_VALIDATE
        {
          V3 o, d, v0, v1, v2;
          double tmax;
          sq_ray(S, squeue, idx, &o, &d, &tmax);
          const DAnyInst *A = &S.any_insts[kMulti ? winst : ~SQ_FIELD(S, squeue, idx, group)];
          load_tri(nullptr, (const float *) (S.blas_base + ((size_t) tri_base << 7)), first, &v0, &v1, &v2);
          const bool ex_ = tri_ray_anyhit(v0, v1, v2, xpoint(A->Minv, o), xvector(A->Minv, d), tmin, tmax);
          atomicAdd(&g_trifilter[verdict], 1ull);
          if ((verdict == FJ_TRI_MISS && ex_) || (verdict == FJ_TRI_HIT && !ex_)) atomicAdd(&g_trifilter[3], 1ull);
          if (ex_) atomicAdd(&g_trifilter[4], 1ull);
        }
#endif
        const bool stall_now = verdict == FJ_TRI_MAYBE && has_pex;
        if (verdict == FJ_TRI_MAYBE) pex = has_pex ? (pex | AH_PEX_STALL) : first;
        const bool occluded = verdict == FJ_TRI_HIT;
        if (occluded) pex = TRAV_DONE;
#else
        V3 v0, v1, v2;
        load_tri(nullptr, (const float *) (S.blas_base + ((size_t) tri_base << 7)), first, &v0, &v1, &v2);
        FJ_SCHED_FENCE();
        ah_lds_f64 *const rp_ = &s_ray[AH_TID()];
        const bool occluded = tri_ray_anyhit(v0, v1, v2, mk(rp_[0], rp_[BLOCK], rp_[2 * BLOCK]), mk(rp_[3 * BLOCK], rp_[4 * BLOCK], rp_[5 * BLOCK]), tmin, rp_[6 * BLOCK]);
        const bool stall_now = false;
#endif
        if (occluded) {
          have = false; cur = TRAV_DONE;
          AH_PLEAF_CLEAR();
#ifdef FJ_WAVE_TIMELINE
          FJ_TL_RAY(ray_steps);
#endif
          PH(10, 1);
        }
        else if (stall_now) { }
        else if (from_p) { if (more) pleaf = FJ_LEAF_FLAG | ((first + 1u) << 3) | (more - 1u); else AH_PLEAF_NEXT(); }
        else if (more) cur = FJ_LEAF_FLAG | ((first + 1u) << 3) | (more - 1u);
        else cur = (spa < ah_row1) ? TRAV_DONE : pop(spa);
      }
    }
  }
#undef AH_AT
#undef AH_OVF
#undef AH_POSTPONE
#undef AH_PLEAF_NEXT
#undef AH_PLEAF_CLEAR
#undef AH_TID
#ifdef FJ_PHASE_STATS
  for (int i = 0; i < 16; i++) {
    const unsigned long long v = (i == 10 || i == 14) ? wave_sum(ph[i]) : ph[i];
    if (lane == 0 && v) atomicAdd(&g_ahphase[i], v);
  }
#endif
}

#ifndef FJ_ANYHIT_MINB
#if FJ_ANYHIT_F32
#define FJ_ANYHIT_MINB 7
#else
#define FJ_ANYHIT_MINB 6
#endif
#endif
#ifndef FJ_ANYHIT_MINB_MULTI
#define FJ_ANYHIT_MINB_MULTI 5
#endif
static_assert((FJ_STACK_LDS_ANYHIT * BLOCK * 4) % 8 == 0, "the object-space rays behind the LDS stack are doubles");
template <bool kCount, bool kMulti>
__global__ void __launch_bounds__(BLOCK, kMulti ? FJ_ANYHIT_MINB_MULTI : FJ_ANYHIT_MINB) k_shadow_anyhit(DScene S, const DShadowRay *squeue, float *s_accum,
    DCounters *cnt, TravTune tune)
{
  __shared__ alignas(16) uint32_t s_stack[FJ_STACK_LDS_ANYHIT * BLOCK + FJ_ANYHIT_RAY_WORDS * BLOCK];
  const uint32_t n = cnt->shadow_count < S.shadow_queue_cap ? cnt->shadow_count : S.shadow_queue_cap;
  LocalCounters lc = {0, 0, 0, 0};
  traverse_anyhit<kCount, kMulti>(S, squeue, s_accum, tune, n, &cnt->shadow_xcd_head[0][0], s_stack, &lc);
  if (kCount) {
    flush_counters(cnt, lc.nodes, lc.prims, lc.insts, 0, 0);
    flush_stack_peak(&cnt->sh_stack_peak, lc.stack_peak);
    flush_shadow_walk_counters(cnt, lc.nodes, lc.prims, lc.insts);
    if (blockIdx.x == 0 && threadIdx.x == 0) atomicAdd(&cnt->squeued, (unsigned long long) n);
  }
}

#endif
```

### fujiyama-renderer_amd/csrc/device/fjgpu_dev_shadow.h

```cpp
#ifndef FJGPU_DEV_SHADOW_H
#define FJGPU_DEV_SHADOW_H

#ifndef SQ_CHUNK
#define SQ_CHUNK 512u
#endif
#ifndef JQ_CHUNK
#define JQ_CHUNK 64u
#endif
#define SQ_INVALID 0xffffffffu
__device__ __forceinline__ const DShadowRayC *sq_c(const DShadowRay *squeue, uint32_t i) { return (const DShadowRayC *) squeue + i; }
#define SQ_FIELD(S, squeue, i, f) ((S).compact_squeue ? sq_c(squeue, i)->f : (squeue)[i].f)
__device__ __forceinline__ const float *sq_colour(const DScene &S, const DShadowRay *squeue, uint32_t i) { return S.compact_squeue ? sq_c(squeue, i)->c : squeue[i].c; }
__device__ __forceinline__ void sq_ray(const DScene &S, const DShadowRay *squeue, uint32_t i, V3 *o, V3 *d, double *tmax)
{
  if (!S.compact_squeue) {
    const DShadowRay *q = &squeue[i];
    *o = mk(q->o[0], q->o[1], q->o[2]); *d = mk(q->d[0], q->d[1], q->d[2]); *tmax = q->tmax;
    return;
  }
  const DShadowRayC *q = sq_c(squeue, i);
  const V3 Ps = mk(q->o[0], q->o[1], q->o[2]);
  const DLightSample *LS = &S.light_samples[q->light];
  const V3 Pl = mk(LS->P[0], LS->P[1], LS->P[2]);
  V3 Ln = mk(Pl.x - Ps.x, Pl.y - Ps.y, Pl.z - Ps.z);
  const double distance = sqrt(dot(Ln, Ln));
  if (distance > 0) {
    const double inv = 1. / distance;
    Ln = mk(Ln.x * inv, Ln.y * inv, Ln.z * inv);
  }
  *o = Ps; *d = Ln; *tmax = distance;
}

__device__ __forceinline__ DLightSample ld_light_sample_k(const DLightSample *p)
{
  typedef const __attribute__((address_space(4))) double kd;
  typedef const __attribute__((address_space(4))) float kf;
  typedef const __attribute__((address_space(4))) int32_t ki;
  kd *q = (kd *) (uintptr_t) p;
  kf *f = (kf *) (uintptr_t) (p->Cl);
  ki *i = (ki *) (uintptr_t) (&p->light);
  DLightSample r;
  r.P[0] = q[0]; r.P[1] = q[1]; r.P[2] = q[2];
  r.Cl[0] = f[0]; r.Cl[1] = f[1]; r.Cl[2] = f[2];
  r.light = i[0]; r.type = i[1]; r.ordinal = i[2];
  return r;
}

__device__ __forceinline__ double ld_k_f64(const double *p) { return *(const __attribute__((address_space(4))) double *) (uintptr_t) p; }
__device__ __forceinline__ int32_t ld_k_i32(const int32_t *p) { return *(const __attribute__((address_space(4))) int32_t *) (uintptr_t) p; }
#ifdef FJ_LIGHT_CONE_VALIDATE
__device__ unsigned long long g_lightcone[2];
#endif

#ifndef FJ_CULL_MINB
#define FJ_CULL_MINB 1
#endif
#ifndef FJ_CULL_CLAIMS_PER_WAVE
#define FJ_CULL_CLAIMS_PER_WAVE 16u
#endif
#ifndef FJ_CULL_MINB_PLAIN
#define FJ_CULL_MINB_PLAIN 3
#endif
#ifndef FJ_CULL_MINB_WHOLE
#define FJ_CULL_MINB_WHOLE 4
#endif
#ifndef FJ_CULL_LDS_NODES
#define FJ_CULL_LDS_NODES 292
#endif
template <bool kHair, bool kArea, bool kSplit, bool kNodesLds = false, bool kCone = false>
__global__ void __launch_bounds__(BLOCK, (kHair || kArea) ? FJ_CULL_MINB : (kSplit ? FJ_CULL_MINB_PLAIN : FJ_CULL_MINB_WHOLE)) k_shadow_cull(DScene S, ShadowParams sp, const DLightRec *lrecs,
    uint32_t rec_begin, uint32_t rec_end, float *s_accum, DShadowRay *squeue, DCounters *cnt, int count_events)
{
  __shared__ double s_nodes[kNodesLds ? FJ_CULL_LDS_NODES * 7 : 1];
  if (kNodesLds) {
    const unsigned long long *src = (const unsigned long long *) S.group_nodes;
    for (uint32_t w = threadIdx.x; w < (uint32_t) S.n_group_nodes * 7u; w += BLOCK) ((unsigned long long *) s_nodes)[w] = src[w];
    __syncthreads();
  }
  const DTNode *gnodes = kNodesLds ? (const DTNode *) s_nodes : S.group_nodes;
  unsigned long long c_insts = 0, c_shadow = 0;
  const unsigned lane = __lane_id();
  const uint32_t n = rec_end - rec_begin;
  const uint32_t n_waves = (gridDim.x * BLOCK) >> 6;
  uint32_t claim = (n / (n_waves * FJ_CULL_CLAIMS_PER_WAVE)) & ~63u;
  claim = claim < 64u ? 64u : (claim > 1024u ? 1024u : claim);
  uint32_t chunk_base = 0, chunk_used = SQ_CHUNK;
  uint32_t jchunk_base = 0, jchunk_used = JQ_CHUNK;

  uint32_t slice_end = 0, r0 = 0;
  for (;; r0 += 64u) {
    if (r0 >= slice_end) {
      uint32_t base = 0;
      if (lane == 0) base = atomicAdd(&cnt->cull_head, claim);
      r0 = __shfl(base, 0);
      if (r0 >= n) break;
      slice_end = r0 + claim < n ? r0 + claim : n;
    }
    const uint32_t rec = rec_begin + r0 + lane;
    const bool active = (r0 + lane) < slice_end;

    float sum[3] = {0.f, 0.f, 0.f};
    uint32_t r_insts = 0, r_shadow = 0;
    uint32_t r_sample = 0;
    float W[3] = {0.f, 0.f, 0.f};
    const uint32_t nl = (uint32_t) S.n_light_samples;
    DLightRec R;
    DLightHair H;
    for (int q = 0; q < 6; q++) H.aux[q] = 0;
    H.Cd[0] = H.Cd[1] = H.Cd[2] = 0.f;
    R.uid = R.key = 0; R.kind = 0;
    XS xs = {0, 0, 0, 0};
    V3 Ps = mk(0, 0, 0), axis = Ps, nml_axis = Ps;
    int g_first = 0, g_count = 0;
    bool g_single = false;
    const double *g_sbounds = nullptr;
    double sb[6] = {0, 0, 0, 0, 0, 0};
    double cos_limit = kHair ? 0 : sp.cos_half_pi;
    if (active) {
      R = lrecs[rec];
      if (kHair && (R.kind & 1)) H = S.lrec_hair[rec];
      Ps = mk(R.P[0], R.P[1], R.P[2]);
      axis = mk(R.N[0], R.N[1], R.N[2]);
      nml_axis = normalize(axis);
      r_sample = R.sample;
      W[0] = R.W[0]; W[1] = R.W[1]; W[2] = R.W[2];
      if (kHair) cos_limit = (R.kind & 1) == 0 ? sp.cos_half_pi : sp.cos_pi;
      g_first = S.groups[R.group].first; g_count = S.groups[R.group].count;
      g_single = S.groups[R.group].n_instances == 1;
      g_sbounds = S.groups[R.group].sbounds;
      if (g_single) { for (int q = 0; q < 6; q++) sb[q] = g_sbounds[q]; g_first = gnodes[g_first].inst; }
    }
    const bool deep_inside = active && g_single &&
        Ps.x > sb[0] + 2e-4 && Ps.x < sb[3] - 2e-4 && Ps.y > sb[1] + 2e-4 && Ps.y < sb[4] - 2e-4 && Ps.z > sb[2] + 2e-4 && Ps.z < sb[5] - 2e-4;
    const DLightCone *cone_row = nullptr;
    bool cone_lane = false;
    if (kCone) {
      static_assert(!kCone || (!kHair && !kArea && !kSplit), "the cones serve whole rays to fixed light positions");
      const int grp = active ? R.group : -1;
      const int g0 = __builtin_amdgcn_readfirstlane(grp);
      if (__ballot(active && grp != g0) == 0ull) {
        const int row = ld_k_i32(S.cone_rows + g0);
        if (row >= 0) {
          cone_row = S.light_cones + (size_t) row * nl;
          const double reach = ld_k_f64(&cone_row->reach);
          cone_lane = active && !deep_inside && fmax(fmax(fabs(Ps.x), fabs(Ps.y)), fabs(Ps.z)) <= reach;
        }
      }
    }
    for (uint32_t l = 0; l < nl; l++) {
      bool emit = false;
      DShadowRay q;
      bool pending = false;
      int tcur = 0;
      uint32_t ncand = 0, jslot1 = 0, nb = 0, be = 0;
      int cb0 = 0, cb1 = 0, cb2 = 0, cb3 = 0;
      V3 winv_s = mk(0, 0, 0), Ln_s = winv_s;
      bool plain_s = false;
      double dist_s = 0;
      float k_s[3] = {0.f, 0.f, 0.f};
      int lc_count = 0;
      if (kCone && cone_row) lc_count = ld_k_i32(&cone_row[l].count);
      if (active) {
        const DLightSample LS = ld_light_sample_k(S.light_samples + l);
        V3 Pl = mk(LS.P[0], LS.P[1], LS.P[2]);
        float Cl[3] = {LS.Cl[0], LS.Cl[1], LS.Cl[2]};
        if (kArea && (LS.type == FJ_GRID_LIGHT || LS.type == FJ_SPHERE_LIGHT)) {
          const DAreaLight *A = &S.area_lights[LS.light];
          if (LS.ordinal == 0) xs = area_stream(R.uid, R.key, LS.light);
          V3 Nl;
          if (LS.type == FJ_GRID_LIGHT) {
            const double px = xs.f01() - .5;
            const double pz = xs.f01() - .5;
            Pl = xpoint(A->M, mk(px, 0, pz));
            Nl = mk(A->N[0], A->N[1], A->N[2]);
          } else {
            V3 o;
            double dd;
            for (;;) {
              o.x = 2 * xs.f01() - 1;
              o.y = 2 * xs.f01() - 1;
              o.z = 2 * xs.f01() - 1;
              dd = dot(o, o);
              if (dd > 0 && dd <= 1) break;
            }
            const double inv = 1. / sqrt(dd);
            const V3 p = mk(o.x * inv, o.y * inv, o.z * inv);
            Pl = xpoint(A->M, p);
            Nl = normalize(xvector(A->M, p));
          }
          const V3 Lq = normalize(mk(Ps.x - Pl.x, Ps.y - Pl.y, Ps.z - Pl.z));
          double dl = dot(Lq, Nl);
          float k;
          if (LS.type == FJ_GRID_LIGHT) {
            dl = A->double_sided ? fabs(dl) : (dl > 0. ? dl : 0.);
            k = (float) (dl * (double) A->sample_intensity);
          } else k = dl > 0 ? A->sample_intensity : 0.f;
          Cl[0] = k * A->color[0]; Cl[1] = k * A->color[1]; Cl[2] = k * A->color[2];
        }
        V3 Ln = mk(Pl.x - Ps.x, Pl.y - Ps.y, Pl.z - Ps.z);
        const double behind = nml_axis.x * Ln.x + nml_axis.y * Ln.y + nml_axis.z * Ln.z;
        const double terms = fabs(nml_axis.x * Ln.x) + fabs(nml_axis.y * Ln.y) + fabs(nml_axis.z * Ln.z);
        const bool surely_behind = cos_limit >= 0 && behind < -1e-12 * terms;
        double distance = 0, cosangle = -1;
        if (!surely_behind) {
          distance = sqrt(dot(Ln, Ln));
          if (distance > 0) {
            const double inv = 1. / distance;
            Ln = mk(Ln.x * inv, Ln.y * inv, Ln.z * inv);
          }
          cosangle = dot(nml_axis, Ln);
        }
        const bool lit = !surely_behind && !(cosangle < cos_limit) && !(Cl[0] < .0001 && Cl[1] < .0001 && Cl[2] < .0001);
        if (lit) {
          float k[3] = {0.f, 0.f, 0.f};
          if (!kHair || (R.kind & 1) == 0) {
            float Kd = (float) dot(axis, Ln);
            Kd = (float) (Kd > 0 ? (double) Kd : 0.);
            k[0] = Kd * Cl[0]; k[1] = Kd * Cl[1]; k[2] = Kd * Cl[2];
          } else {
            const V3 tangent = mk(H.aux[0], H.aux[1], H.aux[2]);
            const V3 Iv = mk(H.aux[3], H.aux[4], H.aux[5]);
            const float TL = (float) dot(tangent, Ln);
            const float diff = (float) sqrt((double) (1 - TL * TL));
            const float roughness = .05f;
            const float TI = (float) dot(tangent, Iv);
            float spec = (float) (sqrt((double) (1 - TL * TL)) * sqrt((double) (1 - TI * TI)) + (double) (TL * TI));
            static_assert(1 / .05f == 20.f, "the exponent of the hair shader's specular term");
            { const double s1 = (double) spec, s2 = s1 * s1, s4 = s2 * s2, s5 = s4 * s1, s10 = s5 * s5; spec = (float) (s10 * s10); }
            k[0] = (H.Cd[0] * diff + spec) * Cl[0];
            k[1] = (H.Cd[1] * diff + spec) * Cl[1];
            k[2] = (H.Cd[2] * diff + spec) * Cl[2];
          }
          const bool carries = !(W[0] * k[0] == 0.f && W[1] * k[1] == 0.f && W[2] * k[2] == 0.f);
          bool maybe_occluded = false;
          if (sp.cast_shadow) {
            r_shadow++;
            bool sure = false;
            if (kCone && lc_count > 0) {
              const bool cand = cone_lane && carries && plain_dir(Ln);
              if (__ballot(cand)) {
                const double *pn = &cone_row[l].n[0][0];
                const double m = light_cone_margin(Ln.x, Ln.y, Ln.z);
#define FJ_LC_PLANE(j) (cand & light_cone_plane_out(ld_k_f64(pn + 3 * (j)), ld_k_f64(pn + 3 * (j) + 1), ld_k_f64(pn + 3 * (j) + 2), Ln.x, Ln.y, Ln.z, m))
                sure = FJ_LC_PLANE(0) | FJ_LC_PLANE(1) | FJ_LC_PLANE(2) | FJ_LC_PLANE(3);
                if (lc_count > 4 && __ballot(cand && !sure) != 0ull) sure = sure | FJ_LC_PLANE(4) | FJ_LC_PLANE(5);
#undef FJ_LC_PLANE
              }
#ifdef FJ_LIGHT_CONE_VALIDATE
              {
                const bool wrong = sure && box_ray_ref(sb, Ps, Ln, .0001, distance);
                const unsigned long long mv = __ballot(sure), mw = __ballot(wrong);
                if (mv && lane == (unsigned) __builtin_ctzll(mv)) { atomicAdd(&g_lightcone[0], (unsigned long long) __popcll(mv)); if (mw) atomicAdd(&g_lightcone[1], (unsigned long long) __popcll(mw)); }
              }
#endif
              if (sure) r_insts++;
            }
            const bool need = carries && !(kCone && sure);
            bool test = false;
            if (!kCone || __ballot(need)) test = need && !has_negative_zero(Ln);
            if (deep_inside) maybe_occluded = test;
            else if (test) {
              const V3 winv = mk(filter_rcp(Ln.x), filter_rcp(Ln.y), filter_rcp(Ln.z));
              const bool plain = plain_dir(Ln);
              if (g_single) {
                maybe_occluded = box_ray_ref_fast(sb, Ps, Ln, winv, plain, .0001, distance);
                if (!maybe_occluded) r_insts++;
              }
              if (kSplit && !g_single && sp.join_capacity) {
                pending = true; tcur = g_first; winv_s = winv; plain_s = plain; Ln_s = Ln; dist_s = distance;
                k_s[0] = k[0]; k_s[1] = k[1]; k_s[2] = k[2];
              }
              for (int ti = g_first; !g_single && !pending && ti < g_first + g_count;) {
                const DTNode *tn_ = &gnodes[ti];
                if (tn_->inst < 0) {
                  double tq;
                  ti = slab(tn_->box, tn_->box + 3, Ps, winv, .0001, distance, &tq) ? ti + 1 : tn_->skip;
                  continue;
                }
                ti++;
                if (box_ray_ref_fast(tn_->box, Ps, Ln, winv, plain, .0001, distance)) { maybe_occluded = true; break; }
                r_insts++;
              }
            }
          }
          if (maybe_occluded) {
            emit = true;
            q.o[0] = Ps.x; q.o[1] = Ps.y; q.o[2] = Ps.z;
            q.d[0] = Ln.x; q.d[1] = Ln.y; q.d[2] = Ln.z;
            q.tmax = distance;
            q.c[0] = W[0] * k[0]; q.c[1] = W[1] * k[1]; q.c[2] = W[2] * k[2];
            q.sample = r_sample; q.group = (sp.pre_resolve && g_single) ? ~g_first : R.group; q.tindex = (kSplit && sp.join_capacity) ? 0u : ((uint32_t) R.kind >> 1);
          } else if (carries && (!kSplit || !pending)) {
            sum[0] += k[0]; sum[1] += k[1]; sum[2] += k[2];
          }
        }
      }
      for (;;) {
      bool need_slot = false;
      if (kSplit && pending && be == nb) {
        nb = 0; be = 0;
        while (tcur < g_first + g_count && nb < 4u) {
          const DTNode *tn_ = &gnodes[tcur];
          if (tn_->inst < 0) {
            double tq;
            tcur = slab(tn_->box, tn_->box + 3, Ps, winv_s, .0001, dist_s, &tq) ? tcur + 1 : tn_->skip;
            continue;
          }
          tcur++;
          if (box_ray_ref_fast(tn_->box, Ps, Ln_s, winv_s, plain_s, .0001, dist_s)) {
            if (nb == 0u) cb0 = tn_->inst; else if (nb == 1u) cb1 = tn_->inst; else if (nb == 2u) cb2 = tn_->inst; else cb3 = tn_->inst;
            nb++;
          } else r_insts++;
        }
        if (nb == 0u) {
          pending = false;
          if (ncand == 0u) { sum[0] += k_s[0]; sum[1] += k_s[1]; sum[2] += k_s[2]; }
        } else {
          need_slot = jslot1 == 0u && ncand + nb >= 2u;
          ncand += nb;
        }
      }
      const unsigned long long m_slot = kSplit ? __ballot(need_slot) : 0ull;
      if (kSplit && m_slot) {
        const uint32_t n_slot = (uint32_t) __popcll(m_slot);
        if (jchunk_used + n_slot > JQ_CHUNK) {
          uint32_t base = 0;
          if (lane == 0) base = atomicAdd(&cnt->join_count, JQ_CHUNK);
          jchunk_base = __shfl(base, 0);
          jchunk_used = 0;
        }
        if (need_slot) {
          jslot1 = jchunk_base + jchunk_used + (uint32_t) __popcll(m_slot & ((1ull << lane) - 1ull)) + 1u;
          if (jslot1 > sp.join_capacity) { cnt->overflow = 1; jslot1 = 1; }
        }
        jchunk_used += n_slot;
      }
      if (kSplit && pending && be < nb) {
        const int cand = be == 0u ? cb0 : (be == 1u ? cb1 : (be == 2u ? cb2 : cb3));
        be++;
        emit = true;
        q.o[0] = Ps.x; q.o[1] = Ps.y; q.o[2] = Ps.z;
        q.d[0] = Ln_s.x; q.d[1] = Ln_s.y; q.d[2] = Ln_s.z;
        q.tmax = dist_s;
        q.c[0] = W[0] * k_s[0]; q.c[1] = W[1] * k_s[1]; q.c[2] = W[2] * k_s[2];
        q.sample = r_sample; q.group = ~cand; q.tindex = jslot1;
        if (be == nb && tcur >= g_first + g_count) pending = false;
      }
      const unsigned long long mask = __ballot(emit);
      const uint32_t need = (uint32_t) __popcll(mask);
      if (need) {
        if (chunk_used + need > SQ_CHUNK) {
          if (chunk_used < SQ_CHUNK)
            for (uint32_t k = chunk_used + lane; k < SQ_CHUNK; k += 64)
              if (chunk_base + k < sp.queue_capacity) { if (sp.compact) ((DShadowRayC *) squeue)[chunk_base + k].sample = SQ_INVALID; else squeue[chunk_base + k].sample = SQ_INVALID; }
          uint32_t base = 0;
          if (lane == 0) base = atomicAdd(&cnt->shadow_count, SQ_CHUNK);
          chunk_base = __shfl(base, 0);
          chunk_used = 0;
        }
        if (emit) {
          const uint32_t slot = chunk_base + chunk_used + (uint32_t) __popcll(mask & ((1ull << lane) - 1ull));
          if (slot >= sp.queue_capacity) cnt->overflow = 1;
          else if (sp.compact) {
            DShadowRayC qc;
            qc.o[0] = q.o[0]; qc.o[1] = q.o[1]; qc.o[2] = q.o[2];
            qc.c[0] = q.c[0]; qc.c[1] = q.c[1]; qc.c[2] = q.c[2];
            qc.sample = q.sample; qc.group = q.group; qc.tindex = q.tindex; qc.light = l; qc.pad = 0;
            ((DShadowRayC *) squeue)[slot] = qc;
          }
          else squeue[slot] = q;
        }
        chunk_used += need;
      }
      emit = false;
      if (!kSplit || __ballot(pending) == 0ull) break;
      }
      if (kSplit && ncand >= 2) S.shadow_join[jslot1 - 1u] = ncand << 16;
    }
    c_insts += r_insts; c_shadow += r_shadow;
    if (active) {
      float *acc = s_accum + 4 * (size_t) r_sample;
      const float r0v = W[0] * sum[0], r1v = W[1] * sum[1], r2v = W[2] * sum[2];
      if (r0v != 0.f) atomicAdd(acc + 0, r0v);
      if (r1v != 0.f) atomicAdd(acc + 1, r1v);
      if (r2v != 0.f) atomicAdd(acc + 2, r2v);
    }
  }
  if (chunk_used < SQ_CHUNK)
    for (uint32_t k = chunk_used + lane; k < SQ_CHUNK; k += 64)
      if (chunk_base + k < sp.queue_capacity) { if (sp.compact) ((DShadowRayC *) squeue)[chunk_base + k].sample = SQ_INVALID; else squeue[chunk_base + k].sample = SQ_INVALID; }
  flush_counters(cnt, 0, 0, count_events ? c_insts : 0, count_events ? c_shadow : 0, c_shadow);
}

struct ShadowPolicy {
  const DScene *S;
  const DShadowRay *squeue;
  float *s_accum;
  __device__ bool fetch(uint32_t i, RayIn *r) const
  {
    const DShadowRay q = squeue[i];
    if (q.sample == SQ_INVALID) return false;
    r->o = mk(q.o[0], q.o[1], q.o[2]); r->d = mk(q.d[0], q.d[1], q.d[2]);
    r->tmin = .0001; r->tmax = q.tmax;
    r->time = S->has_motion ? sample_time(*S, q.tindex) : 0.;
    r->group = q.group;
    r->anyhit = S->groups[q.group].all_opaque != 0;
    return true;
  }
  __device__ void finish(uint32_t i, const Best &b) const
  {
    float ac = 1.f;
    if (b.inst >= 0) {
      float Os = 1.f;
      const DInstance *I = &S->instances[b.inst];
      const DPrimSet *P = &S->primsets[I->primset];
      const int sg = (P->face_group && b.prim >= 0) ? P->face_group[b.prim] : 0;
      int sid;
      if (sg < 0 || sg >= I->n_shaders) sid = I->shaders[0];
      else { sid = I->shaders[sg]; if (sid < 0) sid = I->shaders[0]; }
      if (sid >= 0 && S->shaders[sid].type == FJ_SHADER_PLASTIC) Os = S->shaders[sid].opacity;
      Os = (float) clampd(Os, 0, 1);
      ac = 1 - Os;
    }
    if (ac == 0.f) return;
    const DShadowRay *q = &squeue[i];
    const float r0 = q->c[0] * ac, r1 = q->c[1] * ac, r2 = q->c[2] * ac;
    float *acc = s_accum + 4 * (size_t) q->sample;
    if (r0 != 0.f) atomicAdd(acc + 0, r0);
    if (r1 != 0.f) atomicAdd(acc + 1, r1);
    if (r2 != 0.f) atomicAdd(acc + 2, r2);
  }
};

template <bool kCurves, bool kCount, bool kMotion, bool kInstLds = false, bool kAnyOnly = false>
__global__ void __launch_bounds__(BLOCK, kMotion ? FJ_MOTION_MINB : (kCurves ? FJ_CURVE_MINB : FJ_SHADOW_MINB)) k_shadow_trace(DScene S, const DShadowRay *squeue, float *s_accum,
    DCounters *cnt, TravTune tune)
{
  __shared__ uint32_t s_stack[(kCurves ? FJ_STACK_LDS_CURVES : FJ_STACK_LDS) * BLOCK];
  __shared__ double s_rayspace[kCurves ? FJ_RAYSPACE_DOUBLES * BLOCK : 1];
  __shared__ double s_inst[kInstLds ? InstLdsOf<kCurves>::T::WORDS : 1];
  if (kInstLds) InstLdsOf<kCurves>::T::fill(S, s_inst);
  const uint32_t n = cnt->shadow_count;
  ShadowPolicy pol;
  pol.S = &S; pol.squeue = squeue; pol.s_accum = s_accum;
  LocalCounters lc = {0, 0, 0, 0};
  traverse_persistent<kCurves, kCount, kMotion, kInstLds, kAnyOnly>(S, pol, tune, n, &cnt->shadow_xcd_head[0][0], make_stack(s_stack, S.stack_overflow_shadow, kCurves ? s_rayspace : nullptr), &lc, s_inst);
  if (kCount) {
    flush_counters(cnt, lc.nodes, lc.prims, lc.insts, 0, 0);
    flush_stack_peak(&cnt->sh_stack_peak, lc.stack_peak);
    flush_shadow_walk_counters(cnt, lc.nodes, lc.prims, lc.insts);
    if (blockIdx.x == 0 && threadIdx.x == 0) atomicAdd(&cnt->squeued, (unsigned long long) n);
  }
}

#endif
```

### fujiyama-renderer_amd/csrc/device/fjgpu_kernels.h

```cpp
#ifndef FJGPU_KERNELS_H
#define FJGPU_KERNELS_H

#include <hip/hip_runtime.h>
#include "fjgpu_types.h"

struct TileDesc {
  int32_t xmin, ymin, xmax, ymax;
  int32_t nx, ny;
  uint32_t sample_offset;
  int32_t id;
  uint32_t cell_offset;
  int32_t pad;
};

struct GenParams {
  int32_t rate_x, rate_y, margin_x, margin_y;
  double udelta, vdelta, jitter;
  int32_t jittered, pad;
};

struct AovParams {
  int32_t xres, rate_x, rate_y, margin_x, margin_y, pad;
  float *depth, *position, *normal, *uv;
  int32_t *ids;
  float *coverage;
};

struct AlbedoParams {
  int32_t xres, rate_x, rate_y, margin_x, margin_y;
  int32_t lanes, lanes_log2, pad;
  float *albedo;
};

struct AdaptiveParams {
  int32_t D, div;
  int32_t margin_x, margin_y;
  double udelta, vdelta, jitter, threshold;
  int32_t jittered, level;
  uint32_t cells0;
  uint32_t ray_capacity;
};

struct ShadeParams {
  int32_t max_diffuse_depth, max_reflect_depth, max_refract_depth;
  int32_t count_all_shadow;
  uint32_t ray_capacity, light_capacity;
  uint32_t *next_keys;
  const float *fc_in;
  float *fc_out;
  double sort_lo[3], sort_scale[3];
  int32_t sort_bits, pad_;
};

struct ShadowParams {
  double cos_half_pi, cos_pi;
  uint32_t pre_resolve;
  uint32_t queue_capacity;
  uint32_t join_capacity;
  int32_t cast_shadow;
  int32_t compact;
  int32_t light_cones;
};

struct ResolveParams {
  int32_t xres, yres, rate_x, rate_y, npx_x, npx_y;
  double fw, fh;
};

int launch_gen_camera(hipStream_t st, const DScene &S, const GenParams &gp, const TileDesc *d_tiles, int n_tiles,
    uint32_t max_tile_samples, const double *jit, const double *tim, double *s_uv, DRay *rays, DPath *paths, uint32_t *s_tk = nullptr);
int launch_trace_closest(hipStream_t st, const DScene &S, const DRay *rays, const DPath *paths, DHit *hits,
    uint32_t n, DCounters *cnt, int count_events);
int launch_shade(hipStream_t st, const DScene &S, const ShadeParams &sp, const DRay *rays, const DPath *paths,
    const DHit *hits, uint32_t n, float *s_accum, DRay *next_rays, DPath *next_paths, DLightRec *lrecs, DCounters *cnt);
uint32_t shadow_queue_padding();
void shadow_queue_reset(hipStream_t st, DCounters *cnt);
int launch_shadow_cull(hipStream_t st, const DScene &S, const ShadowParams &sp, const DLightRec *lrecs, uint32_t b, uint32_t e,
    float *s_accum, DShadowRay *squeue, DCounters *cnt, int count_events, int blocks_per_cu = 0);
int launch_shadow_trace(hipStream_t st, const DScene &S, const DShadowRay *squeue, float *s_accum, DCounters *cnt, int count_events);
int launch_quantize_nodes(hipStream_t st, const DNode *nodes, uint32_t n, const double *origin, const double *cell, DNodeQ *out);
int launch_move_tiles(hipStream_t st, bool unpack, float *fb, int xres, const int32_t *d_rects, int n_tiles, int tile_px, float *slab);
void set_anyhit_filter_off(long v);
void light_cone_validate_counts(double *verdicts, double *contradictions);
void debug_phase_stats();
size_t persistent_threads();

int launch_resolve(hipStream_t st, const ResolveParams &rp, const TileDesc *d_tiles, int n_tiles, int max_tile_pixels,
    const double *s_uv, const float *s_accum, const double *s_data64, float *fb);

int launch_aov_reduce(hipStream_t st, const DScene &S, const AovParams &ap, const TileDesc *d_tiles, int n_tiles, int max_tile_pixels,
    const DRay *rays, const DHit *hits);

int launch_aov_albedo(hipStream_t st, const DScene &S, const AlbedoParams &ap, const TileDesc *d_tiles, int n_tiles, int max_tile_pixels,
    const DHit *hits);

int launch_adaptive_uv(hipStream_t st, const AdaptiveParams &ap, const TileDesc *d_tiles, int n_tiles, uint32_t max_tile_samples,
    const double *jit, double *s_uv);
int launch_adaptive_points(hipStream_t st, const DScene &S, const AdaptiveParams &ap, const TileDesc *d_tiles, int n_tiles,
    uint32_t max_tile_points, const uint8_t *cells, const double *s_uv, const float *s_accum, uint8_t *pstate, double *seen,
    DRay *rays, DPath *paths, DCounters *cnt);
int launch_adaptive_decide(hipStream_t st, const AdaptiveParams &ap, const TileDesc *d_tiles, int n_tiles, uint32_t max_tile_cells,
    uint8_t *cells, const float *s_accum, const uint8_t *pstate, const double *seen);
int launch_adaptive_fill(hipStream_t st, const AdaptiveParams &ap, const TileDesc *d_tiles, int n_tiles, uint32_t max_tile_samples,
    const uint8_t *cells, const float *s_accum, const uint8_t *pstate, const double *seen, double *final_data);

#endif
```

### fujiyama-renderer_amd/csrc/device/fjgpu_kernels.hip

```cpp
#include <hip/hip_runtime.h>
#include <float.h>
#include <math.h>
#include <stdint.h>
#include <stdlib.h>
#include <stdio.h>

#include "fjgpu_types.h"
#include "fjgpu_kernels.h"
#include "fjgpu_xform_math.h"

#define BLOCK 256

#include "fjgpu_dev_math.h"
#include "fjgpu_tri_filter.h"
#include "fjgpu_light_cone.h"
#include "fjgpu_dev_curve.h"
#include "fjgpu_dev_traverse.h"
#include "fjgpu_dev_flat.h"
#include "fjgpu_dev_shade.h"
#include "fjgpu_dev_shadow.h"
#include "fjgpu_dev_anyhit.h"
#include "fjgpu_dev_anyhit_curves.h"
#include "fjgpu_dev_adaptive.h"
#include "fjgpu_dev_aov.h"
// ... 289 lines not shown
  else if (S.inst_lds && S.multi_shadow_groups && S.n_group_nodes <= FJ_CULL_LDS_NODES) {
    if (split) hipLaunchKernelGGL((k_shadow_cull<false, false, true, true>), dim3(persistent_grid((threads + BLOCK - 1) / BLOCK, cull_blocks_per_cu(blocks_per_cu))), dim3(BLOCK), 0, st, S, sp, lrecs, b, e, s_accum, squeue, cnt, count_events);
    else hipLaunchKernelGGL((k_shadow_cull<false, false, false, true>), dim3(persistent_grid((threads + BLOCK - 1) / BLOCK, cull_blocks_per_cu(blocks_per_cu))), dim3(BLOCK), 0, st, S, sp, lrecs, b, e, s_accum, squeue, cnt, count_events);
  }
  else if (split) FJ_LAUNCH_CULL(false, false, true);
  else if (sp.light_cones && S.light_cones && S.cone_rows)
    hipLaunchKernelGGL((k_shadow_cull<false, false, false, false, true>), dim3(persistent_grid((threads + BLOCK - 1) / BLOCK, cull_blocks_per_cu(blocks_per_cu))), dim3(BLOCK), 0, st, S, sp, lrecs, b, e, s_accum, squeue, cnt, count_events);
  else FJ_LAUNCH_CULL(false, false, false);
#undef FJ_LAUNCH_CULL
  LAUNCH_CHECK();
  return 0;
}

int launch_shadow_trace(hipStream_t st, const DScene &S, const DShadowRay *squeue, float *s_accum, DCounters *cnt, int count_events)
{
  TL_ZERO(st);
  if (S.all_opaque && !S.has_curves && !S.has_motion && S.blas_base) {
#define FJ_LAUNCH_ANYHIT(COUNT, MULTI) hipLaunchKernelGGL((k_shadow_anyhit<COUNT, MULTI>), dim3(persistent_grid(1ull << 30, anyhit_blocks_per_cu(MULTI))), dim3(BLOCK), 0, st, S, squeue, s_accum, cnt, trav_tune())
    if (S.multi_shadow_groups && !S.shadow_join) { if (count_events) FJ_LAUNCH_ANYHIT(true, true); else FJ_LAUNCH_ANYHIT(false, true); }
    else { if (count_events) FJ_LAUNCH_ANYHIT(true, false); else FJ_LAUNCH_ANYHIT(false, false); }
#undef FJ_LAUNCH_ANYHIT
  } else {
#define FJ_LAUNCH_SHADOW(CURVES, COUNT, MOTION) hipLaunchKernelGGL((k_shadow_trace<CURVES, COUNT, MOTION>), dim3(persistent_grid(1ull << 30)), dim3(BLOCK), 0, st, S, squeue, s_accum, cnt, trav_tune())
    if (S.has_motion) { if (count_events) FJ_LAUNCH_SHADOW(true, true, true); else FJ_LAUNCH_SHADOW(true, false, true); }
    else if (S.has_curves) {
      if (InstLdsCurves::fits(S) && S.all_opaque && S.curve_anyhit && FJ_CURVE_QNODES && FJ_CLOSEST_QNODES) {
        const dim3 cgrid(persistent_grid(1ull << 30, canyhit_blocks_per_cu()));
        if (count_events) hipLaunchKernelGGL((k_shadow_anyhit_curves<true>), cgrid, dim3(BLOCK), 0, st, S, squeue, s_accum, cnt, trav_tune());
        else hipLaunchKernelGGL((k_shadow_anyhit_curves<false>), cgrid, dim3(BLOCK), 0, st, S, squeue, s_accum, cnt, trav_tune());
      }
      else if (InstLdsCurves::fits(S) && S.all_opaque) {
        if (count_events) hipLaunchKernelGGL((k_shadow_trace<true, true, false, true, true>), dim3(persistent_grid(1ull << 30)), dim3(BLOCK), 0, st, S, squeue, s_accum, cnt, trav_tune());
        else hipLaunchKernelGGL((k_shadow_trace<true, false, false, true, true>), dim3(persistent_grid(1ull << 30)), dim3(BLOCK), 0, st, S, squeue, s_accum, cnt, trav_tune());
      }
      else if (InstLdsCurves::fits(S)) {
        if (count_events) hipLaunchKernelGGL((k_shadow_trace<true, true, false, true>), dim3(persistent_grid(1ull << 30)), dim3(BLOCK), 0, st, S, squeue, s_accum, cnt, trav_tune());
        else hipLaunchKernelGGL((k_shadow_trace<true, false, false, true>), dim3(persistent_grid(1ull << 30)), dim3(BLOCK), 0, st, S, squeue, s_accum, cnt, trav_tune());
      }
      else if (count_events) FJ_LAUNCH_SHADOW(true, true, false); else FJ_LAUNCH_SHADOW(true, false, false);
    }
    else if (InstLdsBig::fits(S)) {
      if (count_events) hipLaunchKernelGGL((k_shadow_trace<false, true, false, true>), dim3(persistent_grid(1ull << 30)), dim3(BLOCK), 0, st, S, squeue, s_accum, cnt, trav_tune());
      else hipLaunchKernelGGL((k_shadow_trace<false, false, false, true>), dim3(persistent_grid(1ull << 30)), dim3(BLOCK), 0, st, S, squeue, s_accum, cnt, trav_tune());
    }
    else { if (count_events) FJ_LAUNCH_SHADOW(false, true, false); else FJ_LAUNCH_SHADOW(false, false, false); }
#undef FJ_LAUNCH_SHADOW
  }
  LAUNCH_CHECK();
  TL_DUMP(st, "shadow", persistent_grid(1ull << 30, PERSIST_BLOCKS_PER_CU_MAX));
  return 0;
}

int launch_quantize_nodes(hipStream_t st, const DNode *nodes, uint32_t n, const double *origin, const double *cell, DNodeQ *out)
{
  if (n == 0) return 0;
  hipLaunchKernelGGL(k_quantize_nodes, dim3((n + BLOCK - 1) / BLOCK), dim3(BLOCK), 0, st, nodes, n, origin[0], origin[1], origin[2],
      cell[0], cell[1], cell[2], out);
  LAUNCH_CHECK();
  return 0;
}

int launch_move_tiles(hipStream_t st, bool unpack, float *fb, int xres, const int32_t *d_rects, int n_tiles, int tile_px, float *slab)
{
  for (int t0 = 0; t0 < n_tiles; t0 += 65535) {
    const int nt = n_tiles - t0 < 65535 ? n_tiles - t0 : 65535;
    const dim3 grid((tile_px + BLOCK - 1) / BLOCK, nt);
    float4 *sl = (float4 *) slab + (size_t) t0 * tile_px;
    if (unpack) hipLaunchKernelGGL(k_move_tiles<true>, grid, dim3(BLOCK), 0, st, (float4 *) fb, xres, (const int4 *) d_rects + t0, tile_px, sl);
    else hipLaunchKernelGGL(k_move_tiles<false>, grid, dim3(BLOCK), 0, st, (float4 *) fb, xres, (const int4 *) d_rects + t0, tile_px, sl);
    LAUNCH_CHECK();
  }
  return 0;
}

void light_cone_validate_counts(double *verdicts, double *contradictions)
{
  *verdicts = -1; *contradictions = -1;
#ifdef FJ_LIGHT_CONE_VALIDATE
  unsigned long long c[2];
  if (hipMemcpyFromSymbol(c, HIP_SYMBOL(g_lightcone), sizeof(c)) == hipSuccess) { *verdicts = (double) c[0]; *contradictions = (double) c[1]; }
#endif
}

void debug_phase_stats()
{
#ifdef FJ_TRI_FILTER_VALIDATE
  {
    unsigned long long c[8];
    if (hipMemcpyFromSymbol(c, HIP_SYMBOL(g_trifilter), sizeof(c)) == hipSuccess && (c[0] | c[1] | c[2])) {
      fprintf(stderr, "fjgpu tri filter: miss %llu hit %llu maybe %llu | exact hits %llu | CONTRADICTIONS %llu\n", c[0], c[1], c[2], c[4], c[3]);
      unsigned long long z[8] = {0};
      (void) hipMemcpyToSymbol(HIP_SYMBOL(g_trifilter), z, sizeof(z));
    }
  }
#endif
#ifdef FJ_PHASE_STATS
  {
    unsigned long long c[8];
    if (hipMemcpyFromSymbol(c, HIP_SYMBOL(g_curve_stat), sizeof(c)) == hipSuccess && c[2]) {
      fprintf(stderr, "fjgpu phase curves: second-stage execs %llu lanes %llu tests-hit %llu leaf-walks %llu nodes %llu\n", c[2], c[3], c[4], c[0], c[1]);
      unsigned long long z[8] = {0};
      (void) hipMemcpyToSymbol(HIP_SYMBOL(g_curve_stat), z, sizeof(z));
    }
  }
  {
    unsigned long long c[16];
    if (hipMemcpyFromSymbol(c, HIP_SYMBOL(g_cphase), sizeof(c)) == hipSuccess && c[12]) {
      static const char *pn[4] = {"turnover", "inner", "leaf", "ribbon"};
      const double all = (double) (c[0] + c[1] + c[2] + c[3]);
      fprintf(stderr, "fjgpu phase curve-anyhit: %llu iterations", c[12]);
      for (int k = 0; k < 4; k++) fprintf(stderr, " | %s %.1f %% of ticks, %llu execs, %.1f lanes, %.0f ticks each", pn[k], 100. * c[k] / all, c[4 + k], (double) c[8 + k] / (c[4 + k] ? c[4 + k] : 1), (double) c[k] / (c[4 + k] ? c[4 + k] : 1));
      fprintf(stderr, "\n");
      unsigned long long z[16] = {0};
      (void) hipMemcpyToSymbol(HIP_SYMBOL(g_cphase), z, sizeof(z));
    }
  }
  unsigned long long h[16];
  if (hipMemcpyFromSymbol(h, HIP_SYMBOL(g_phase), sizeof(h)) != hipSuccess) return;
  static const char *names[16] = {"iters", "entry_execs|entry_ticks", "entry_lanes", "inner_execs|inner_ticks", "inner_lanes", "leaf_execs|leaf_ticks", "leaf_lanes",
      "tri_execs|stage2_ticks", "tri_lanes", "", "hits", "refills", "tail_iters_max", "tail_iters_sum", "walk_iters_sum", "walk_waves"};
  for (int i = 0; i < 16; i++) if (names[i][0]) fprintf(stderr, "fjgpu phase %-24s %llu\n", names[i], h[i]);
  {
    unsigned long long a[16];
    if (hipMemcpyFromSymbol(a, HIP_SYMBOL(g_ahphase), sizeof(a)) == hipSuccess && a[3] && a[5]) {
      fprintf(stderr, "fjgpu phase anyhit-lanes: %llu iterations | inner steps %llu with %.1f lanes at inner nodes, %.1f idle, %.1f held at a leaf | leaf steps %llu with %.1f lanes, %.1f idle, "
          "%.1f at inner nodes | turnovers %llu with %.1f lanes | %llu rays occluded\n", a[0], a[3], (double) a[4] / a[3], (double) a[7] / a[3], (double) a[8] / a[3], a[5], (double) a[6] / a[5],
          (double) a[9] / a[5], (double) a[11] / a[5], a[1], (double) a[2] / (a[1] ? a[1] : 1), a[10]);
      if (a[12]) fprintf(stderr, "fjgpu phase anyhit-exact: %llu exact phases with %.1f lanes, %llu of them hits\n", a[12], (double) a[13] / a[12], a[14]);
      unsigned long long z[16] = {0};
      (void) hipMemcpyToSymbol(HIP_SYMBOL(g_ahphase), z, sizeof(z));
    }
  }
  if (h[7] && h[11]) fprintf(stderr, "fjgpu phase phased-walk: turnover %llu execs %.1f lanes %.0f ticks | inner %llu execs %.1f lanes %.0f ticks | leaf %llu execs %.1f lanes %.0f ticks | "
      "instance loop %.2f trips per turnover lane, %.2f wave trips per turnover\n", h[7], (double) h[2] / h[7], (double) h[1] / h[7], h[8], (double) h[4] / (h[8] ? h[8] : 1), (double) h[3] / (h[8] ? h[8] : 1),
      h[9], (double) h[6] / (h[9] ? h[9] : 1), (double) h[5] / (h[9] ? h[9] : 1), (double) h[10] / (h[2] ? h[2] : 1), (double) h[11] / h[7]);
  unsigned long long z[16] = {0};
  (void) hipMemcpyToSymbol(HIP_SYMBOL(g_phase), z, sizeof(z));
#endif
}

int launch_resolve(hipStream_t st, const ResolveParams &rp, const TileDesc *d_tiles, int n_tiles, int max_tile_pixels,
    const double *s_uv, const float *s_accum, const double *s_data64, float *fb)
{
  const dim3 grid((max_tile_pixels + BLOCK / 64 - 1) / (BLOCK / 64), n_tiles);
  if (s_data64)
    hipLaunchKernelGGL(k_resolve<double4>, grid, dim3(BLOCK), 0, st, rp, d_tiles, s_uv, reinterpret_cast<const double4 *>(s_data64), fb);
  else
    hipLaunchKernelGGL(k_resolve<float4>, grid, dim3(BLOCK), 0, st, rp, d_tiles, s_uv, reinterpret_cast<const float4 *>(s_accum), fb);
  LAUNCH_CHECK();
  return 0;
}

int launch_aov_reduce(hipStream_t st, const DScene &S, const AovParams &ap, const TileDesc *d_tiles, int n_tiles, int max_tile_pixels,
    const DRay *rays, const DHit *hits)
{
  if (n_tiles <= 0 || max_tile_pixels <= 0) return 0;
  const dim3 grid((max_tile_pixels + BLOCK / 64 - 1) / (BLOCK / 64), n_tiles);
  hipLaunchKernelGGL(k_aov_reduce, grid, dim3(BLOCK), 0, st, S, ap, d_tiles, rays, hits);
  LAUNCH_CHECK();
  return 0;
}

int launch_aov_albedo(hipStream_t st, const DScene &S, const AlbedoParams &ap, const TileDesc *d_tiles, int n_tiles, int max_tile_pixels,
    const DHit *hits)
{
  if (n_tiles <= 0 || max_tile_pixels <= 0) return 0;
// ... 47 lines not shown
```

### fujiyama-renderer_amd/csrc/device/fjgpu_types.h

```cpp
#ifndef FJGPU_TYPES_H
#define FJGPU_TYPES_H

#include <stdint.h>
#include "fj_scene_desc.h"

struct DNode {
  float box[4][6];
  uint32_t child[4];
  uint32_t pad[4];
};
static_assert(sizeof(DNode) == 128, "DNode must be 128 bytes");

struct DNodeQ {
  uint16_t q[4][6];
  uint32_t child[4];
};
static_assert(sizeof(DNodeQ) == 64, "DNodeQ must be 64 bytes");

#ifndef FJ_CURVE_QNODES
#define FJ_CURVE_QNODES 1
#endif
#ifndef FJ_CLOSEST_QNODES
#define FJ_CLOSEST_QNODES 1
#endif
// ... 98 lines not shown
#define FJ_INST_LDS_NODES_CURVES 15
#define FJ_INST_LDS_INSTS_CURVES 6
#define FJ_INST_LDS_GROUPS_CURVES 12
#define FJ_FLAT_LDS_INSTS 80
#define FJ_INST_LDS_BYTES (FJ_INST_LDS_NODES * 56 + FJ_INST_LDS_INSTS * 8 * FJ_INST_LDS_ENTRY_WORDS + FJ_INST_LDS_GROUPS * 64)

struct DAnyInst {
  double Minv[12];
  double bounds[6];
  double qorigin[3], qcell[3];
  uint32_t node_base;
  uint32_t tri_base;
  uint32_t root;
  uint32_t tris_f32;
  int32_t n_prims;
  float fbound;
  uint32_t pad[2];
};
static_assert(sizeof(DAnyInst) == 224, "DAnyInst layout");

#define FJ_TLAS_FLAT 4
struct DTNode {
  double box[6];
  int32_t inst;
  int32_t skip;
};

struct DGroup {
  int32_t first, count;
  int32_t all_opaque;
  int32_t n_instances;
  double sbounds[6];
};

struct DFlatRef { float v[9]; uint32_t inst_ord; uint32_t pid; uint32_t pad; };
static_assert(sizeof(DFlatRef) == 48, "DFlatRef must be 48 bytes");
struct DFlat {
  const DNodeQ *nodes;
  const DFlatRef *refs;
  const double *refbox;
  double qorigin[3], qcell[3];
  uint32_t root;
  int32_t n_inst, n_prims, pad;
};

struct DTexture {
  const float *tiles;
  int32_t width, height, nchannels, tilesize;
};

struct DLightSample {
  double P[3];
  float Cl[3];
  int32_t light;
  int32_t type;
  int32_t ordinal;
};

struct DAreaLight {
  double M[12];
  double N[3];
  float color[3];
  float sample_intensity;
  int32_t double_sided;
  int32_t pad;
};

struct DLightHair;
struct DLightCone;

struct DScene {
  const DPrimSet *primsets;
  const DInstance *instances;
  const DGroup *groups;
  const DTNode *group_nodes;
  const DInstEntry *inst_entries;
  int32_t n_group_nodes;
  int32_t inst_lds;
  const fj_shader_desc *shaders;
  const DTexture *textures;
  const DLightSample *light_samples;
  const DLightCone *light_cones;
  const int32_t *cone_rows;
  DLightHair *lrec_hair;
  uint32_t shadow_queue_cap;
  uint32_t cam_slot0;
  uint32_t *shadow_join;
  const DFlat *flats;
  const DAreaLight *area_lights;
  const DAnyInst *any_insts;
  const char *blas_base;
  int32_t n_light_samples;
  int32_t n_instances, n_groups, n_primsets;
  uint32_t *stack_overflow;
  uint32_t *stack_overflow_shadow;
  int32_t all_opaque;
  int32_t has_area;
  int32_t has_hair;
  int32_t has_curves;
  int32_t target_group;
  int32_t curve_anyhit;
  int32_t incoherent_rays;
  const double *cam_uv;
  int32_t compact_squeue;
  int32_t pad_cs_;
  const uint32_t *cam_tk;
  const uint32_t *ray_perm;
  const double *trace_ranges;
  const uint32_t *trace_n_dev;
  const fj_xform_desc *xforms;
  const fj_xform_desc *cam_xform;
  const double *time_tab;
  double time_start, time_end;
  int32_t has_motion;
  int32_t multi_shadow_groups;
  double cam_M[12];
  double cam_uv_size[2];
  double cam_znear, cam_zfar;
};

struct DRay {
  double o[3], d[3];
};
static_assert(sizeof(DRay) == 48, "DRay must be 48 bytes");
#define FJ_CXT_TMIN_1E4 0x80u

enum { CXT_CAMERA_RAY = 0, CXT_SHADOW_RAY, CXT_DIFFUSE_RAY, CXT_REFLECT_RAY, CXT_REFRACT_RAY };

struct DPath {
  uint32_t sample;
  float T[3];
  uint8_t cxt, ddepth, rdepth, tdepth;
  int32_t group;
  uint32_t flags;
  uint32_t rng;
  uint32_t uid;
};
static_assert(sizeof(DPath) == 36, "DPath must be 36 bytes");

struct DHit {
  double t, u, v;
  int32_t inst, prim;
};

struct DLightRec {
  double P[3];
  double N[3];
  float W[3];
  uint32_t sample;
  int32_t group;
  int32_t kind;
  uint32_t uid;
  uint32_t key;
};

struct DLightHair {
  double aux[6];
  float Cd[3];
  uint32_t pad;
};

struct DShadowRay {
  double o[3], d[3], tmax;
  float c[3];
  uint32_t sample;
  int32_t group;
  uint32_t tindex;
};

struct DShadowRayC {
  double o[3];
  float c[3];
  uint32_t sample;
  int32_t group;
  uint32_t tindex;
  uint32_t light;
  uint32_t pad;
};
static_assert(sizeof(DShadowRayC) == 56, "DShadowRayC must be 56 bytes");

struct DCounters {
  unsigned long long rays[5];
  unsigned long long nodes, prims, insts, traced, squeued;
  unsigned long long sh_nodes, sh_prims, sh_insts;
  unsigned long long stack_peak, sh_stack_peak;
  unsigned long long pad0_[1];
  uint32_t next_count;
  uint32_t light_count;
  uint32_t overflow;
  uint32_t cam_count;
  uint32_t pad1_[28];
  uint32_t shadow_count;
  uint32_t shadow_head;
  uint32_t pad2_[30];
  uint32_t trace_head;
  uint32_t cull_head;
  uint32_t pad3_[30];
  uint32_t shadow_xcd_head[8][32];
  uint32_t trace_xcd_head[8][32];
  uint32_t join_count;
  uint32_t pad4_[31];
};

#endif
```

### fujiyama-renderer_amd/gpu.py

```python
import ctypes as C

import numpy as np

from . import ffi

_lib = None


class GpuError(RuntimeError):
    pass


def lib():
    global _lib
    if _lib is None:
        L = ffi.load("libfjgpu.so")
        L.fjgpu_last_error.restype = C.c_char_p
        L.fjgpu_device_count.restype = C.c_int
        L.fjgpu_scene_create.argtypes = [C.c_void_p, C.c_int, C.POINTER(C.c_void_p)]
        L.fjgpu_scene_destroy.argtypes = [C.c_void_p]
        L.fjgpu_scene_destroy.restype = None
        L.fjgpu_tile_count.argtypes = [C.POINTER(ffi.RenderDesc)]
        L.fjgpu_tile_rect.argtypes = [C.POINTER(ffi.RenderDesc), C.c_int, C.POINTER(C.c_int32)]
        L.fjgpu_render_tiles.argtypes = [C.c_void_p, C.POINTER(ffi.RenderDesc), C.c_void_p, C.c_int,
# ... 186 lines not shown
            info["denoise_stats"] = res[-1]
            return res[0], info
        out, info["denoise_stats"] = denoise(fb, aov["normal"], aov["position"], aov["ids"], region=region, device=self._device,
                                             stream=stream, out=fb, **kw)
        return out, info

    def get_camera(self):
        cam = ffi.CameraDesc()
        _check(lib().fjgpu_scene_get_camera(self._h, C.byref(cam)))
        return cam

    def set_camera(self, camera=None, translate=None, rotate=None, fov=None):
        cam = self.get_camera() if camera is None else camera.copy()
        if translate is not None:
            cam.xform.translate[0].v[:] = tuple(float(v) for v in translate)
        if rotate is not None:
            cam.xform.rotate[0].v[:] = tuple(float(v) for v in rotate)
        if fov is not None:
            cam.fov = float(fov)
        _check(lib().fjgpu_scene_set_camera(self._h, C.byref(cam)))
        return cam

    def view(self, render):
        v = ffi.View()
        _check(lib().fjgpu_scene_view(self._h, C.byref(render), C.byref(v)))
        return v

    def camera_samples(self, render, tile_id):
        n = lib().fjgpu_camera_samples(self._h, C.byref(render), int(tile_id), None, 0)
        if n < 0:
            _check(n)
        rays = np.empty((n, 8), dtype=np.float64)
        m = lib().fjgpu_camera_samples(self._h, C.byref(render), int(tile_id), rays.ctypes.data_as(C.c_void_p), n)
        if m < 0:
            _check(m)
        return rays


class MultiScene(object):

    def __init__(self, scene_desc_ptr, devices):
        self.n = len(devices)
        self._h = (C.c_void_p * self.n)()
        devs = (C.c_int * self.n)(*devices)
        _check(lib().fjgpu_scene_create_multi(scene_desc_ptr, devs, self.n, self._h))

    def close(self):
        for k in range(self.n):
            if self._h[k]:
                lib().fjgpu_scene_destroy(self._h[k])
                self._h[k] = None

    def __del__(self):
        try:
            self.close()
        except Exception:
            pass

    def render_frame(self, render, tile_ids=None):
        fb = np.zeros((render.yres, render.xres, 4), dtype=np.float32)
        st = (ffi.GpuStats * self.n)()
        if tile_ids is None:
            ids_p, n = None, 0
        else:
            ids = np.ascontiguousarray(tile_ids, dtype=np.int32)
            ids_p, n = ids.ctypes.data_as(C.c_void_p), len(ids)
        _check(lib().fjgpu_render_frame_multi(self._h, self.n, C.byref(render), ids_p, n, fb.ctypes.data_as(C.c_void_p), st))
        return fb, list(st)


def host_instance_level(scene_desc_ptr, group):
    L = lib()
    L.fjgpu_host_instance_level.argtypes = [C.c_void_p, C.c_int, C.c_void_p, C.c_void_p, C.c_void_p, C.c_int]
    L.fjgpu_host_instance_level.restype = C.c_int
    n = L.fjgpu_host_instance_level(scene_desc_ptr, group, None, None, None, 0)
    if n < 0:
        _check(n)
    inst = np.zeros(n, dtype=np.int32)
    skip = np.zeros(n, dtype=np.int32)
    box = np.zeros((n, 6), dtype=np.float64)
    _check(min(0, L.fjgpu_host_instance_level(scene_desc_ptr, group, inst.ctypes.data_as(C.c_void_p), skip.ctypes.data_as(C.c_void_p),
                                              box.ctypes.data_as(C.c_void_p), n)))
    return inst, skip, box


DENOISE_ITERATIONS = 5
SIGMA_COLOR = 3.0
SIGMA_NORMAL = 1.0
SIGMA_POSITION_FRACTION = 0.1
ALBEDO_FLOOR = 1e-4


def _device_tensor(a, name, dtype, channels, dev, shape=None):
    import torch
    if a is None:
        return None
    t = a if torch.is_tensor(a) else torch.from_numpy(np.ascontiguousarray(a))
    t = t.to(device=dev, dtype=dtype).contiguous()
    if t.dim() != 3 or t.shape[2] != channels or (shape is not None and tuple(t.shape[:2]) != tuple(shape)):
        raise ValueError("%s must be [H, W, %d]%s, not %s" % (name, channels, "" if shape is None else " with H, W = %d, %d" % tuple(shape),
                                                             tuple(t.shape)))
    return t


def denoise(color, normal=None, position=None, ids=None, iterations=DENOISE_ITERATIONS, sigma_color=SIGMA_COLOR,
            sigma_normal=SIGMA_NORMAL, sigma_position=None, stop_at_ids=True, region=None, device=0, stream=None, out=None,
            albedo=None, albedo_floor=ALBEDO_FLOOR):
    import torch
    dev = torch.device("cuda", device)
    c = _device_tensor(color, "color", torch.float32, 4, dev)
    hw = tuple(c.shape[:2])
    n = _device_tensor(normal, "normal", torch.float32, 3, dev, hw)
    p = _device_tensor(position, "position", torch.float32, 3, dev, hw)
    i = _device_tensor(ids, "ids", torch.int32, 4, dev, hw)
    a = _device_tensor(albedo, "albedo", torch.float32, 3, dev, hw)
    if out is None:
        out = c.clone()
    elif not (torch.is_tensor(out) and out.device == dev and out.dtype == torch.float32 and out.is_contiguous() and tuple(out.shape) == tuple(c.shape)):
        raise ValueError("out must be a contiguous float32 tensor of color's shape on the device")
    d = ffi.DenoiseDesc()
    d.yres, d.xres = hw
    d.region[:] = (0, 0, d.xres, d.yres) if region is None else tuple(int(v) for v in region)
    d.iterations = int(iterations)
    d.sigma_color, d.sigma_normal = float(sigma_color), float(sigma_normal)
    d.sigma_position = 0.0 if sigma_position is None else float(sigma_position)
    d.stop_at_ids = 1 if stop_at_ids else 0
    torch.cuda.synchronize(dev)
    st = ffi.GpuStats()
    ptr = lambda t: C.c_void_p(t.data_ptr()) if t is not None else None
    if a is not None:
        _check(lib().fjgpu_denoise_albedo(device, C.byref(d), ptr(c), ptr(n), ptr(p), ptr(i), ptr(a), C.c_float(float(albedo_floor)), ptr(out),
                                          C.c_void_p(stream or 0), C.byref(st)))
    else:
        _check(lib().fjgpu_denoise(device, C.byref(d), ptr(c), ptr(n), ptr(p), ptr(i), ptr(out), C.c_void_p(stream or 0), C.byref(st)))
    return out.cpu().numpy(), st


SIGMA_LUMINANCE = 4.0
SIGMA_POSITION_FRACTION_VARIANCE = 0.03


def _variance_tensor(v, name, dev, hw):
    import torch
    if v is None:
        return None
    t = v if torch.is_tensor(v) else torch.from_numpy(np.ascontiguousarray(v))
    t = t.to(device=dev, dtype=torch.float32).contiguous()
    if tuple(t.shape) != tuple(hw):
        raise ValueError("%s must be [H, W] = %d, %d, not %s" % ((name,) + tuple(hw) + (tuple(t.shape),)))
    return t


def _denoise_desc(hw, region, iterations, sigma_normal, sigma_position, stop_at_ids):
    d = ffi.DenoiseDesc()
    d.yres, d.xres = hw
    d.region[:] = (0, 0, d.xres, d.yres) if region is None else tuple(int(v) for v in region)
    d.iterations = int(iterations)
    d.sigma_color, d.sigma_normal = 0.0, float(sigma_normal)
    d.sigma_position = 0.0 if sigma_position is None else float(sigma_position)
    d.stop_at_ids = 1 if stop_at_ids else 0
    return d


def estimate_variance(color, normal=None, position=None, ids=None, region=None, sigma_normal=SIGMA_NORMAL, sigma_position=None,
                      stop_at_ids=True, device=0, stream=None):
    import torch
# ... 266 lines not shown
```

### include/fjgpu.h

```cpp
#ifndef FJGPU_H
#define FJGPU_H

#include <stdint.h>
#include "fj_scene_desc.h"

#ifdef __cplusplus
extern "C" {
#endif

enum {
  FJGPU_OK = 0,
  FJGPU_ENODEV = -1,
  FJGPU_EINVAL = -2,
  FJGPU_EUNSUPPORTED = -3,
  FJGPU_ENOMEM = -4
};

typedef struct fjgpu_scene fjgpu_scene;

typedef struct fjgpu_stats {
  fj_ray_counts rays;
  uint64_t nodes_visited;
  uint64_t prims_tested;
  uint64_t insts_tested;
// ... 62 lines not shown
    const fjgpu_aov_buffers *buffers , float *d_albedo ,
    void *hip_stream, fjgpu_stats *stats);

int fjgpu_camera_samples(fjgpu_scene *scene, const fj_render_desc *render, int tile_id, double *rays8, int cap);

typedef struct fjgpu_denoise_desc {
  int32_t xres, yres;
  int32_t region[4];
  int32_t iterations;
  float   sigma_color;
  float   sigma_normal;
  float   sigma_position;
  int32_t stop_at_ids;
} fjgpu_denoise_desc;

int fjgpu_denoise(int device, const fjgpu_denoise_desc *desc,
                  const float *color_in,
                  const float *normal,
                  const float *position,
                  const int32_t *ids,
                  float *color_out,
                  void *hip_stream, fjgpu_stats *stats);

int fjgpu_denoise_albedo(int device, const fjgpu_denoise_desc *desc, const float *color_in, const float *normal, const float *position,
    const int32_t *ids, const float *albedo , float albedo_floor, float *color_out,
    void *hip_stream, fjgpu_stats *stats);

int fjgpu_denoise_estimate_variance(int device, const fjgpu_denoise_desc *desc,
    const float *color, const float *normal, const float *position, const int32_t *ids,
    float *variance_out , void *hip_stream, fjgpu_stats *stats);

int fjgpu_denoise_variance(int device, const fjgpu_denoise_desc *desc, float sigma_luminance,
    const float *color_in, const float *normal, const float *position, const int32_t *ids,
    const float *albedo , float albedo_floor,
    const float *variance_in  ,
    float *color_out, float *variance_out , void *hip_stream, fjgpu_stats *stats);

int fjgpu_denoise_estimate_variance_albedo(int device, const fjgpu_denoise_desc *desc,
    const float *color, const float *normal, const float *position, const int32_t *ids,
    const float *albedo , float albedo_floor,
    float *variance_out , void *hip_stream, fjgpu_stats *stats);

int fjgpu_scene_get_camera(const fjgpu_scene *scene, fj_camera_desc *out);
int fjgpu_scene_set_camera(fjgpu_scene *scene, const fj_camera_desc *camera);

typedef struct fjgpu_view {
  double world_to_camera[12];
  double uv_size[2];
  int32_t xres, yres;
} fjgpu_view;
int fjgpu_scene_view(const fjgpu_scene *scene, const fj_render_desc *render, fjgpu_view *out);

typedef struct fjgpu_temporal_history {
  float *color;
  float *moments;
  float *length;
} fjgpu_temporal_history;

typedef struct fjgpu_temporal_desc {
  int32_t xres, yres;
  int32_t region[4];
  float   alpha_min;
  float   max_history;
  float   tol_position;
  float   cos_normal;
  float   min_history_variance;
  float   albedo_floor;
} fjgpu_temporal_desc;

int fjgpu_denoise_temporal(int device, const fjgpu_temporal_desc *desc,
     const float *color, const float *position, const float *normal, const int32_t *ids,
                         const float *albedo , const float *variance_spatial ,
     const fjgpu_view *prev_view, const float *prev_position, const float *prev_normal, const int32_t *prev_ids,
                         const fjgpu_temporal_history *prev ,
     const fjgpu_temporal_history *next, float *variance_out ,
    void *hip_stream, fjgpu_stats *stats);

int fjgpu_set_option(fjgpu_scene *scene, const char *name, long value);

int fjgpu_global_option(const char *name, long value);

int fjgpu_host_instance_level(const fj_scene_desc *desc, int group, int32_t *out_inst, int32_t *out_skip, double *out_box, int cap);

int fjgpu_scene_query(const fjgpu_scene *scene, const char *name, double *value);

void fjgpu_host_make_transform(int transform_order, int rotate_order, const double *trs9, double *M16, double *Minv16);
void fjgpu_host_xorshift_f01(int n, double *out);
void fjgpu_host_sampler_margin(const fj_render_desc *render, int32_t *margin2);
double fjgpu_host_camera_uv_size_y(double fov);

int fjgpu_dev_rccl_selftest(int device, int n_floats);

int fjgpu_dev_sort_pairs(int device, const uint32_t *keys, int n, int key_bits, uint32_t *keys_out, uint32_t *perm, int repeats, double *sort_ms);

const char *fjgpu_last_error(void);

#ifdef __cplusplus
}
#endif
#endif
```

Baseline: 37380 Mray/s.

## Add per-light hexagonal hull culling to settle unoccluded shadow rays early

Builds, on the host, a six-plane hull around each single-instance static mesh as seen from each point light, using threaded passes over the vertices with verification and widening. In the shadow kernel, rays whose direction falls outside the hull are settled as unoccluded without traversal, and the existing box cone test runs only for rays that were not settled. This is meant to skip BVH traversal for shadow rays that clearly miss the mesh silhouette. In exchange it adds host build time at upload, extra per-lane plane tests in double precision, and some register pressure; correctness depends on the conservative margins.

```diff
diff --git a/fujiyama-renderer_amd/csrc/device/fjgpu_api.hip b/fujiyama-renderer_amd/csrc/device/fjgpu_api.hip
--- a/fujiyama-renderer_amd/csrc/device/fjgpu_api.hip
+++ b/fujiyama-renderer_amd/csrc/device/fjgpu_api.hip
@@ -5,6 +5,7 @@
 
 #include <algorithm>
 #include <array>
+#include <atomic>
 #include <cfloat>
 #include <cmath>
 #include <cstdio>
@@ -25,6 +26,7 @@
 #include "fjgpu_kernels.h"
 #include "fjgpu_lbvh.h"
 #include "fjgpu_light_cone.h"
+#include "fjgpu_light_hull.h"
 #include "fjgpu_raysort.h"
 #include "fjgpu_tlas.h"
 
@@ -155,6 +157,9 @@
   long count_events;
   long light_cones = 1;
   int cone_rows = 0, cone_records = 0;
+  long light_hulls = 1;
+  int hull_rows = 0, hull_records = 0;
+  unsigned long long hull_verdicts = 0;
   long count_all_shadow;
   unsigned long long stack_peak_closest = 0, stack_peak_shadow = 0;
   std::unique_ptr<DeviceBuffers> work;
@@ -445,6 +450,102 @@
 
 }
 
+static void build_light_hull_rows(const fjgpu::HostScene &hs, const std::vector<double> &cone_reach, std::vector<DLightCone> &hulls,
+    std::vector<int32_t> &rows, int *n_rows, int *n_records)
+{
+  const size_t nl = hs.light_samples.size();
+  rows.assign(hs.groups.size(), -1);
+  hulls.clear();
+  if (!hs.area_lights.empty()) return;
+  for (size_t g = 0; g < hs.groups.size() && nl; g++) {
+    if (hs.groups[g].n_instances != 1) continue;
+    const DInstance &I = hs.instances[hs.group_members[hs.group_member_first[g]]];
+    const fjgpu::HostPrimSet &ps = hs.primsets[I.primset];
+    if (I.xform >= 0 || ps.type != FJ_PRIMSET_MESH || !ps.mesh || ps.mesh->velocity || ps.mesh->n_points <= 0) continue;
+    std::vector<size_t> lights;
+    for (size_t l = 0; l < nl; l++) if (hs.light_samples[l].type == FJ_POINT_LIGHT) lights.push_back(l);
+    if (lights.empty()) continue;
+    const size_t nv = (size_t) ps.mesh->n_points, nk = lights.size();
+    const size_t chunk = 16384, nchunks = (nv + chunk - 1) / chunk;
+    size_t workers = std::min(16u, std::max(1u, std::thread::hardware_concurrency()));
+    if (const char *omp = getenv("OMP_NUM_THREADS")) { const long v = atol(omp); if (v >= 1) workers = std::min<size_t>(workers, (size_t) v); }
+    const unsigned hc = (unsigned) std::max<size_t>(1, std::min(workers, nchunks));
+    auto over_chunks = [&](const std::function<void(size_t)> &fn) {
+      std::atomic<size_t> next(0);
+      std::vector<std::thread> th;
+      for (unsigned t = 0; t < hc; t++) th.emplace_back([&]() { for (size_t c; (c = next.fetch_add(1)) < nchunks;) fn(c); });
+      for (auto &t : th) t.join();
+    };
+    std::vector<double> W(3 * nv), csum(3 * nchunks, 0.);
+    over_chunks([&](size_t c) {
+      double s[3] = {0., 0., 0.};
+      for (size_t i = c * chunk; i < std::min(nv, (c + 1) * chunk); i++) {
+        light_hull_world(I.M, ps.mesh->P + 3 * i, &W[3 * i]);
+        for (int k = 0; k < 3; k++) s[k] += W[3 * i + k];
+      }
+      for (int k = 0; k < 3; k++) csum[3 * c + k] = s[k];
+    });
+    double ctr[3] = {0., 0., 0.};
+    for (size_t c = 0; c < nchunks; c++) for (int k = 0; k < 3; k++) ctr[k] += csum[3 * c + k];
+    for (int k = 0; k < 3; k++) ctr[k] /= (double) nv;
+    std::vector<LightHullAcc> acc(nk), part(nk * nchunks);
+    for (size_t k = 0; k < nk; k++) light_hull_frame(hs.light_samples[lights[k]].P, ctr, &acc[k]);
+    over_chunks([&](size_t c) {
+      for (size_t k = 0; k < nk; k++) {
+        LightHullAcc A = acc[k];
+        for (size_t i = c * chunk; i < std::min(nv, (c + 1) * chunk) && A.ok; i++) light_hull_add(&A, &W[3 * i]);
+        part[k * nchunks + c] = A;
+      }
+    });
+    for (size_t k = 0; k < nk; k++) for (size_t c = 0; c < nchunks; c++) light_hull_merge(&acc[k], &part[k * nchunks + c]);
+    const size_t at = hulls.size();
+    hulls.resize(at + nl);
+    std::memset(&hulls[at], 0, nl * sizeof(DLightCone));
+    std::vector<char> open(nk, 1);
+    std::vector<uint32_t> bad(nk * nchunks);
+    for (int round = 0; round <= FJ_LH_WIDENINGS; round++) {
+      bool any = false;
+      for (size_t k = 0; k < nk; k++) if (open[k]) { if (light_hull_finish(&acc[k], hs.groups[g].sbounds, &hulls[at + lights[k]])) any = true; else open[k] = 0; }
+      if (!any) break;
+      over_chunks([&](size_t c) {
+        for (size_t k = 0; k < nk; k++) {
+          uint32_t b = 0;
+          if (open[k]) for (size_t i = c * chunk; i < std::min(nv, (c + 1) * chunk); i++) b |= light_hull_verify(&hulls[at + lights[k]], acc[k].Pl, &W[3 * i]);
+          bad[k * nchunks + c] = b;
+        }
+      });
+      for (size_t k = 0; k < nk; k++) {
+        if (!open[k]) continue;
+        uint32_t b = 0;
+        for (size_t c = 0; c < nchunks; c++) b |= bad[k * nchunks + c];
+        if (!b) open[k] = 0;
+        else light_hull_widen(&acc[k], b);
+      }
+    }
+    for (size_t k = 0; k < nk; k++) if (open[k]) std::memset(&hulls[at + lights[k]], 0, sizeof(DLightCone));
+    int built = 0;
+    double reach = 1e300;
+    for (size_t l = 0; l < nl; l++) if (hulls[at + l].count > 0) { built++; reach = std::min(reach, hulls[at + l].reach); }
+    if (!built) { hulls.resize(at); continue; }
+    if (g < cone_reach.size() && cone_reach[g] >= 0) reach = std::min(reach, cone_reach[g]);
+    for (size_t l = 0; l < nl; l++) hulls[at + l].reach = reach;
+    rows[g] = (int32_t) (at / nl);
+    (*n_rows)++; *n_records += built;
+  }
+}
+
+static double box_cone_row_reach(const fjgpu::HostScene &hs, size_t g)
+{
+  if (hs.groups[g].n_instances != 1) return -1.;
+  double reach = 1e300;
+  int built = 0;
+  for (const DLightSample &LS : hs.light_samples) {
+    DLightCone C;
+    if ((LS.type == FJ_POINT_LIGHT || LS.type == FJ_DOME_LIGHT) && light_cone_build(LS.P, hs.groups[g].sbounds, &C) > 0) { built++; reach = std::min(reach, C.reach); }
+  }
+  return built ? reach : -1.;
+}
+
 static int upload_scene(const fj_scene_desc *desc, fjgpu::HostScene &hs, int device, fjgpu_scene **out)
 {
   *out = nullptr;
@@ -715,10 +816,12 @@
   e |= M.upload(hs.light_samples.data(), hs.light_samples.size(), &S.light_samples);
   e |= M.upload(hs.area_lights.data(), hs.area_lights.size(), &S.area_lights);
   S.light_cones = nullptr; S.cone_rows = nullptr;
+  std::vector<double> cone_reach;
   {
     const size_t nl = hs.light_samples.size();
     std::vector<int32_t> rows(hs.groups.size(), -1);
     std::vector<DLightCone> cones;
+    cone_reach.assign(hs.groups.size(), -1.);
     for (size_t g = 0; g < hs.groups.size() && nl; g++) {
       if (hs.groups[g].n_instances != 1) continue;
       const size_t at = cones.size();
@@ -735,11 +838,22 @@
       if (!built) { cones.resize(at); continue; }
       for (size_t l = 0; l < nl; l++) cones[at + l].reach = reach;
       rows[g] = (int32_t) (at / nl);
+      cone_reach[g] = reach;
       sc->cone_rows++; sc->cone_records += built;
     }
     if (!cones.empty()) {
       e |= M.upload(cones.data(), cones.size(), &S.light_cones);
       e |= M.upload(rows.data(), rows.size(), &S.cone_rows);
+    }
+  }
+  S.light_hulls = nullptr; S.hull_rows = nullptr;
+  {
+    std::vector<int32_t> rows;
+    std::vector<DLightCone> hulls;
+    build_light_hull_rows(hs, cone_reach, hulls, rows, &sc->hull_rows, &sc->hull_records);
+    if (!hulls.empty()) {
+      e |= M.upload(hulls.data(), hulls.size(), &S.light_hulls);
+      e |= M.upload(rows.data(), rows.size(), &S.hull_rows);
     }
   }
   S.has_area = hs.area_lights.empty() ? 0 : 1;
@@ -946,6 +1060,34 @@
   return G.count;
 }
 
+int fjgpu_host_light_hulls(const fj_scene_desc *desc, int group, void *out_records, double *out_Pl, int cap, double *out_M)
+{
+  if (!desc || group < 0 || group >= desc->n_groups) return fail(FJGPU_EINVAL, "bad light-hull query");
+  fjgpu::HostScene hs;
+  std::string err;
+  const int e = fjgpu::BuildHostScene(desc, &hs, &err, true);
+  if (e) return fail(e, err);
+  std::vector<int32_t> rows;
+  std::vector<DLightCone> hulls;
+  int n_rows = 0, n_records = 0;
+  std::vector<double> cone_reach(hs.groups.size(), -1.);
+  for (size_t g = 0; g < hs.groups.size(); g++) cone_reach[g] = box_cone_row_reach(hs, g);
+  build_light_hull_rows(hs, cone_reach, hulls, rows, &n_rows, &n_records);
+  if (out_M) {
+    if (hs.groups[group].n_instances != 1) return fail(FJGPU_EINVAL, "light-hull query: the group has several instances");
+    std::memcpy(out_M, hs.instances[hs.group_members[hs.group_member_first[group]]].M, 12 * sizeof(double));
+  }
+  const size_t nl = hs.light_samples.size();
+  for (size_t l = 0; l < nl && (int) l < cap; l++) {
+    if (out_records) {
+      if (rows[group] >= 0) std::memcpy((char *) out_records + l * sizeof(DLightCone), &hulls[(size_t) rows[group] * nl + l], sizeof(DLightCone));
+      else std::memset((char *) out_records + l * sizeof(DLightCone), 0, sizeof(DLightCone));
+    }
+    if (out_Pl) for (int k = 0; k < 3; k++) out_Pl[3 * l + k] = hs.light_samples[l].P[k];
+  }
+  return (int) nl;
+}
+
 int fjgpu_scene_query(const fjgpu_scene *scene, const char *name, double *value)
 {
   if (!scene || !name || !value) return fail(FJGPU_EINVAL, "bad query call");
@@ -991,6 +1133,16 @@
     *value = n == "light_cone_verdicts" ? v : c;
     return 0;
   }
+  if (n == "light_hull_rows") { *value = scene->hull_rows; return 0; }
+  if (n == "light_hull_records") { *value = scene->hull_records; return 0; }
+  if (n == "light_hull_verdicts" || n == "light_hull_contradictions") {
+    double v = -1, c = -1;
+    if (hipSetDevice(scene->device) != hipSuccess || hipDeviceSynchronize() != hipSuccess) return fail(FJGPU_ENODEV, "hipSetDevice / hipDeviceSynchronize");
+    light_hull_validate_counts(&v, &c);
+    if (n == "light_hull_verdicts") *value = v >= 0 ? v : (double) scene->hull_verdicts;
+    else *value = c;
+    return 0;
+  }
   if (n == "has_curves") { *value = scene->S.has_curves; return 0; }
   if (n == "has_motion") { *value = scene->S.has_motion; return 0; }
   return fail(FJGPU_EINVAL, "unknown query " + n);
@@ -1076,6 +1228,7 @@
   if (n == "count_nodes") { scene->count_events = value != 0; return 0; }
   if (n == "count_all_shadow") { scene->count_all_shadow = value != 0; return 0; }
   if (n == "light_cones") { scene->light_cones = value != 0; return 0; }
+  if (n == "light_hulls") { scene->light_hulls = value != 0; return 0; }
   if (n == "overlap_shadow") {
     if (value < 0 || value > 2) return fail(FJGPU_EINVAL, "overlap_shadow: 0 off, 1 on, 2 by the batch size");
     scene->overlap = value;
@@ -1229,6 +1382,7 @@
   HIP_TRY(hipSetDevice(sc->device));
   hipStream_t st = static_cast<hipStream_t>(hip_stream);
   sc->stack_peak_closest = sc->stack_peak_shadow = 0;
+  sc->hull_verdicts = 0;
 
   std::vector<fjgpu::TileRect> all;
   fjgpu::GenerateTiles(*r, &all);
@@ -1347,6 +1501,8 @@
   S.pad_cs_ = 0;
   swp.compact = S.compact_squeue;
   swp.light_cones = (sc->light_cones && S.light_cones && S.cone_rows) ? 1 : 0;
+  swp.pad_ = 0;
+  swp.light_hulls = (swp.light_cones && sc->light_hulls && S.light_hulls && S.hull_rows) ? 1 : 0;
   swp.queue_capacity = (uint32_t) sc->squeue_cap;
   swp.join_capacity = (swp.pre_resolve && sc->split_shadow && sc->d_join) ? (uint32_t) sc->join_cap : 0u;
   S.shadow_join = swp.join_capacity ? sc->d_join : nullptr;
@@ -1635,6 +1791,7 @@
     acc.shadow_nodes += hc.sh_nodes; acc.shadow_prims += hc.sh_prims; acc.shadow_insts += hc.sh_insts;
     sc->stack_peak_closest = std::max(sc->stack_peak_closest, hc.stack_peak);
     sc->stack_peak_shadow = std::max(sc->stack_peak_shadow, hc.sh_stack_peak);
+    sc->hull_verdicts += hc.hull_settled;
     acc.batches++;
     if (sc->batch_fn) {
       const std::vector<int32_t> bids(ids.begin() + (long) b0, ids.begin() + (long) b0 + nb);
diff --git a/fujiyama-renderer_amd/csrc/device/fjgpu_dev_anyhit.h b/fujiyama-renderer_amd/csrc/device/fjgpu_dev_anyhit.h
--- a/fujiyama-renderer_amd/csrc/device/fjgpu_dev_anyhit.h
+++ b/fujiyama-renderer_amd/csrc/device/fjgpu_dev_anyhit.h
@@ -150,6 +150,9 @@
           load_tri(nullptr, (const float *) (S.blas_base + ((size_t) tri_base << 7)), pex & ~AH_PEX_STALL, &v0, &v1, &v2);
           if (tri_ray_anyhit(v0, v1, v2, oo_, od_, tmin, tmax)) {
             have = false; cur = TRAV_DONE; AH_PLEAF_CLEAR();
+#ifdef FJ_LIGHT_HULL_VALIDATE
+            lh_validate_occluded(S, squeue, idx, s_accum);
+#endif
 #ifdef FJ_WAVE_TIMELINE
             FJ_TL_RAY(ray_steps);
 #endif
@@ -376,6 +379,9 @@
         if (occluded) {
           have = false; cur = TRAV_DONE;
           AH_PLEAF_CLEAR();
+#ifdef FJ_LIGHT_HULL_VALIDATE
+          lh_validate_occluded(S, squeue, idx, s_accum);
+#endif
 #ifdef FJ_WAVE_TIMELINE
           FJ_TL_RAY(ray_steps);
 #endif
diff --git a/fujiyama-renderer_amd/csrc/device/fjgpu_dev_shadow.h b/fujiyama-renderer_amd/csrc/device/fjgpu_dev_shadow.h
--- a/fujiyama-renderer_amd/csrc/device/fjgpu_dev_shadow.h
+++ b/fujiyama-renderer_amd/csrc/device/fjgpu_dev_shadow.h
@@ -50,6 +50,20 @@
 __device__ __forceinline__ int32_t ld_k_i32(const int32_t *p) { return *(const __attribute__((address_space(4))) int32_t *) (uintptr_t) p; }
 #ifdef FJ_LIGHT_CONE_VALIDATE
 __device__ unsigned long long g_lightcone[2];
+#endif
+
+#ifdef FJ_LIGHT_HULL_VALIDATE
+__device__ unsigned long long g_lighthull[2];
+__device__ __forceinline__ void lh_validate_occluded(const DScene &S, const DShadowRay *squeue, uint32_t i, float *s_accum)
+{
+  if (!S.compact_squeue || !sq_c(squeue, i)->pad) return;
+  atomicAdd(&g_lighthull[1], 1ull);
+  const DShadowRayC *q = sq_c(squeue, i);
+  float *acc = s_accum + 4 * (size_t) q->sample;
+  if (q->c[0] != 0.f) atomicAdd(acc + 0, q->c[0]);
+  if (q->c[1] != 0.f) atomicAdd(acc + 1, q->c[1]);
+  if (q->c[2] != 0.f) atomicAdd(acc + 2, q->c[2]);
+}
 #endif
 
 #ifndef FJ_CULL_MINB
@@ -132,8 +146,9 @@
     }
     const bool deep_inside = active && g_single &&
         Ps.x > sb[0] + 2e-4 && Ps.x < sb[3] - 2e-4 && Ps.y > sb[1] + 2e-4 && Ps.y < sb[4] - 2e-4 && Ps.z > sb[2] + 2e-4 && Ps.z < sb[5] - 2e-4;
-    const DLightCone *cone_row = nullptr;
+    const DLightCone *cone_row = nullptr, *hull_row = nullptr;
     bool cone_lane = false;
+    uint32_t s_hull = 0;
     if (kCone) {
       static_assert(!kCone || (!kHair && !kArea && !kSplit), "the cones serve whole rays to fixed light positions");
       const int grp = active ? R.group : -1;
@@ -145,11 +160,20 @@
           const double reach = ld_k_f64(&cone_row->reach);
           cone_lane = active && !deep_inside && fmax(fmax(fabs(Ps.x), fabs(Ps.y)), fabs(Ps.z)) <= reach;
         }
+        const int hrow = sp.light_hulls ? ld_k_i32(S.hull_rows + g0) : -1;
+        if (hrow >= 0) {
+          hull_row = S.light_hulls + (size_t) hrow * nl;
+          const double reach = ld_k_f64(&hull_row->reach);
+          cone_lane = active && !deep_inside && fmax(fmax(fabs(Ps.x), fabs(Ps.y)), fabs(Ps.z)) <= reach;
+        }
       }
     }
     for (uint32_t l = 0; l < nl; l++) {
       bool emit = false;
       DShadowRay q;
+#ifdef FJ_LIGHT_HULL_VALIDATE
+      bool hull_flag = false;
+#endif
       bool pending = false;
       int tcur = 0;
       uint32_t ncand = 0, jslot1 = 0, nb = 0, be = 0;
@@ -160,6 +184,8 @@
       float k_s[3] = {0.f, 0.f, 0.f};
       int lc_count = 0;
       if (kCone && cone_row) lc_count = ld_k_i32(&cone_row[l].count);
+      int lh_count = 0;
+      if (kCone && hull_row) lh_count = ld_k_i32(&hull_row[l].count);
       if (active) {
         const DLightSample LS = ld_light_sample_k(S.light_samples + l);
         V3 Pl = mk(LS.P[0], LS.P[1], LS.P[2]);
@@ -235,9 +261,23 @@
           bool maybe_occluded = false;
           if (sp.cast_shadow) {
             r_shadow++;
+            bool settled = false;
+            if (kCone && lh_count > 0) {
+              const bool cand = cone_lane && carries && plain_dir(Ln);
+              if (__ballot(cand)) {
+                const double *pn = &hull_row[l].n[0][0];
+                const double m = light_cone_margin(Ln.x, Ln.y, Ln.z);
+#define FJ_LC_PLANE(j) (cand & light_cone_plane_out(ld_k_f64(pn + 3 * (j)), ld_k_f64(pn + 3 * (j) + 1), ld_k_f64(pn + 3 * (j) + 2), Ln.x, Ln.y, Ln.z, m))
+                settled = FJ_LC_PLANE(0) | FJ_LC_PLANE(1) | FJ_LC_PLANE(2) | FJ_LC_PLANE(3);
+                if (__ballot(cand && !settled) != 0ull) settled = settled | FJ_LC_PLANE(4) | FJ_LC_PLANE(5);
+#undef FJ_LC_PLANE
+                if (count_events) { s_hull += (uint32_t) __popcll(__ballot(settled)); if (settled) r_insts++; }
+              }
+            }
+            const bool boxed = !(kCone && settled);
             bool sure = false;
             if (kCone && lc_count > 0) {
-              const bool cand = cone_lane && carries && plain_dir(Ln);
+              const bool cand = cone_lane && carries && boxed && plain_dir(Ln);
               if (__ballot(cand)) {
                 const double *pn = &cone_row[l].n[0][0];
                 const double m = light_cone_margin(Ln.x, Ln.y, Ln.z);
@@ -255,7 +295,7 @@
 #endif
               if (sure) r_insts++;
             }
-            const bool need = carries && !(kCone && sure);
+            const bool need = carries && boxed && !(kCone && sure);
             bool test = false;
             if (!kCone || __ballot(need)) test = need && !has_negative_zero(Ln);
             if (deep_inside) maybe_occluded = test;
@@ -282,6 +322,12 @@
                 r_insts++;
               }
             }
+            if (kCone && settled) {
+              maybe_occluded = false;
+#ifdef FJ_LIGHT_HULL_VALIDATE
+              if (sp.compact && sp.pre_resolve) { maybe_occluded = true; hull_flag = true; }
+#endif
+            }
           }
           if (maybe_occluded) {
             emit = true;
@@ -366,6 +412,10 @@
             qc.o[0] = q.o[0]; qc.o[1] = q.o[1]; qc.o[2] = q.o[2];
             qc.c[0] = q.c[0]; qc.c[1] = q.c[1]; qc.c[2] = q.c[2];
             qc.sample = q.sample; qc.group = q.group; qc.tindex = q.tindex; qc.light = l; qc.pad = 0;
+#ifdef FJ_LIGHT_HULL_VALIDATE
+            qc.pad = hull_flag ? 1u : 0u;
+            if (hull_flag) atomicAdd(&g_lighthull[0], 1ull);
+#endif
             ((DShadowRayC *) squeue)[slot] = qc;
           }
           else squeue[slot] = q;
@@ -378,6 +428,7 @@
       if (kSplit && ncand >= 2) S.shadow_join[jslot1 - 1u] = ncand << 16;
     }
     c_insts += r_insts; c_shadow += r_shadow;
+    if (kCone && s_hull && lane == 0) atomicAdd(&cnt->hull_settled, (unsigned long long) s_hull);
     if (active) {
       float *acc = s_accum + 4 * (size_t) r_sample;
       const float r0v = W[0] * sum[0], r1v = W[1] * sum[1], r2v = W[2] * sum[2];
diff --git a/fujiyama-renderer_amd/csrc/device/fjgpu_kernels.h b/fujiyama-renderer_amd/csrc/device/fjgpu_kernels.h
--- a/fujiyama-renderer_amd/csrc/device/fjgpu_kernels.h
+++ b/fujiyama-renderer_amd/csrc/device/fjgpu_kernels.h
@@ -60,6 +60,8 @@
   int32_t cast_shadow;
   int32_t compact;
   int32_t light_cones;
+  int32_t light_hulls;
+  int32_t pad_;
 };
 
 struct ResolveParams {
@@ -82,6 +84,7 @@
 int launch_move_tiles(hipStream_t st, bool unpack, float *fb, int xres, const int32_t *d_rects, int n_tiles, int tile_px, float *slab);
 void set_anyhit_filter_off(long v);
 void light_cone_validate_counts(double *verdicts, double *contradictions);
+void light_hull_validate_counts(double *verdicts, double *contradictions);
 void debug_phase_stats();
 size_t persistent_threads();
 
diff --git a/fujiyama-renderer_amd/csrc/device/fjgpu_kernels.hip b/fujiyama-renderer_amd/csrc/device/fjgpu_kernels.hip
--- a/fujiyama-renderer_amd/csrc/device/fjgpu_kernels.hip
+++ b/fujiyama-renderer_amd/csrc/device/fjgpu_kernels.hip
@@ -395,6 +395,15 @@
 #endif
 }
 
+void light_hull_validate_counts(double *verdicts, double *contradictions)
+{
+  *verdicts = -1; *contradictions = -1;
+#ifdef FJ_LIGHT_HULL_VALIDATE
+  unsigned long long c[2];
+  if (hipMemcpyFromSymbol(c, HIP_SYMBOL(g_lighthull), sizeof(c)) == hipSuccess) { *verdicts = (double) c[0]; *contradictions = (double) c[1]; }
+#endif
+}
+
 void debug_phase_stats()
 {
 #ifdef FJ_TRI_FILTER_VALIDATE
diff --git a/fujiyama-renderer_amd/csrc/device/fjgpu_light_hull.h b/fujiyama-renderer_amd/csrc/device/fjgpu_light_hull.h
--- /dev/null
+++ b/fujiyama-renderer_amd/csrc/device/fjgpu_light_hull.h
@@ -0,0 +1,142 @@
+#ifndef FJGPU_LIGHT_HULL_H
+#define FJGPU_LIGHT_HULL_H
+
+#include "fjgpu_light_cone.h"
+
+#define FJ_LH_PLANES 6
+#define FJ_LH_PUSH 1e-9
+#define FJ_LH_SLACK 1e-12
+#define FJ_LH_WIDENINGS 3
+
+struct LightHullAcc {
+  double Pl[3], c[3], e[FJ_LH_PLANES][3];
+  double s[FJ_LH_PLANES];
+  double gap;
+  double push[FJ_LH_PLANES];
+  int32_t ok;
+  int32_t pad;
+};
+
+FJ_LC_FN void light_hull_world(const double *M, const double *v, double *w)
+{
+  for (int a = 0; a < 3; a++) w[a] = M[4 * a] * v[0] + M[4 * a + 1] * v[1] + M[4 * a + 2] * v[2] + M[4 * a + 3];
+}
+
+FJ_LC_FN void light_hull_frame(const double *Pl, const double *centroid, LightHullAcc *A)
+{
+  for (int j = 0; j < FJ_LH_PLANES; j++) { A->s[j] = -1e300; A->push[j] = FJ_LH_PUSH; A->e[j][0] = A->e[j][1] = A->e[j][2] = 0.; }
+  A->gap = 1e300; A->ok = 0; A->pad = 0;
+  double c[3] = {centroid[0] - Pl[0], centroid[1] - Pl[1], centroid[2] - Pl[2]};
+  for (int k = 0; k < 3; k++) { A->Pl[k] = Pl[k]; A->c[k] = 0.; }
+  const double m = lc_max(lc_max(lc_abs(c[0]), lc_abs(c[1])), lc_abs(c[2]));
+  if (!(m > 0.) || !(m < 1e300)) return;
+  for (int k = 0; k < 3; k++) c[k] /= m;
+  const double len = __builtin_sqrt(c[0] * c[0] + c[1] * c[1] + c[2] * c[2]);
+  for (int k = 0; k < 3; k++) c[k] /= len;
+  int k0 = 0;
+  if (lc_abs(c[1]) < lc_abs(c[k0])) k0 = 1;
+  if (lc_abs(c[2]) < lc_abs(c[k0])) k0 = 2;
+  double a[3] = {0., 0., 0.};
+  a[k0] = 1.;
+  const double ca = c[k0];
+  for (int k = 0; k < 3; k++) a[k] -= ca * c[k];
+  const double la = __builtin_sqrt(a[0] * a[0] + a[1] * a[1] + a[2] * a[2]);
+  if (!(la > 0.)) return;
+  for (int k = 0; k < 3; k++) a[k] /= la;
+  const double b[3] = {c[1] * a[2] - c[2] * a[1], c[2] * a[0] - c[0] * a[2], c[0] * a[1] - c[1] * a[0]};
+  const double h = .86602540378443864676;
+  const double cs[FJ_LH_PLANES] = {1., .5, -.5, -1., -.5, .5}, sn[FJ_LH_PLANES] = {0., h, h, 0., -h, -h};
+  for (int j = 0; j < FJ_LH_PLANES; j++) for (int k = 0; k < 3; k++) A->e[j][k] = cs[j] * a[k] + sn[j] * b[k];
+  for (int k = 0; k < 3; k++) A->c[k] = c[k];
+  A->ok = 1;
+}
+
+FJ_LC_FN void light_hull_add(LightHullAcc *A, const double *P)
+{
+  const double w[3] = {P[0] - A->Pl[0], P[1] - A->Pl[1], P[2] - A->Pl[2]};
+  const double cw = A->c[0] * w[0] + A->c[1] * w[1] + A->c[2] * w[2];
+  if (!(cw > 0.) || !(cw < 1e300)) { A->ok = 0; return; }
+  if (cw < A->gap) A->gap = cw;
+  const double inv = 1. / cw;
+  for (int j = 0; j < FJ_LH_PLANES; j++) {
+    const double t = (A->e[j][0] * w[0] + A->e[j][1] * w[1] + A->e[j][2] * w[2]) * inv;
+    if (t > A->s[j]) A->s[j] = t;
+  }
+}
+FJ_LC_FN void light_hull_merge(LightHullAcc *A, const LightHullAcc *B)
+{
+  if (!B->ok) A->ok = 0;
+  if (B->gap < A->gap) A->gap = B->gap;
+  for (int j = 0; j < FJ_LH_PLANES; j++) if (B->s[j] > A->s[j]) A->s[j] = B->s[j];
+}
+
+FJ_LC_FN int light_hull_finish(const LightHullAcc *A, const double *b, DLightCone *out)
+{
+  for (int j = 0; j < FJ_LC_MAX_PLANES; j++) out->n[j][0] = out->n[j][1] = out->n[j][2] = 0.;
+  out->reach = 0.; out->count = 0; out->pad = 0;
+  if (!A->ok) return 0;
+  double ext = 0.;
+  for (int k = 0; k < 6; k++) ext = lc_max(ext, lc_abs(b[k]));
+  for (int k = 0; k < 3; k++) ext = lc_max(ext, lc_abs(A->Pl[k]));
+  if (!(ext > 0.) || !(ext < 1e300)) return 0;
+  const double dx = b[3] - b[0], dy = b[4] - b[1], dz = b[5] - b[2];
+  const double diag = __builtin_sqrt(dx * dx + dy * dy + dz * dz);
+  const double gap = A->gap;
+  if (!(gap >= FJ_LC_MIN_GAP * ext) || !(gap <= FJ_LC_MAX_DIST * diag)) return 0;
+  const int order[FJ_LH_PLANES] = {0, 2, 4, 1, 3, 5};
+  for (int q = 0; q < FJ_LH_PLANES; q++) {
+    const int j = order[q];
+    const double s = A->s[j];
+    if (!(s > -1e150) || !(s < 1e150)) { for (int i = 0; i < FJ_LC_MAX_PLANES; i++) out->n[i][0] = out->n[i][1] = out->n[i][2] = 0.; return 0; }
+    const double sp = s + A->push[j] * (1. + s * s);
+    double n[3] = {A->e[j][0] - sp * A->c[0], A->e[j][1] - sp * A->c[1], A->e[j][2] - sp * A->c[2]};
+    const double m = lc_max(lc_max(lc_abs(n[0]), lc_abs(n[1])), lc_abs(n[2]));
+    if (!(m > 0.)) { for (int i = 0; i < FJ_LC_MAX_PLANES; i++) out->n[i][0] = out->n[i][1] = out->n[i][2] = 0.; return 0; }
+    for (int k = 0; k < 3; k++) n[k] /= m;
+    const double inv = 1. / __builtin_sqrt(n[0] * n[0] + n[1] * n[1] + n[2] * n[2]);
+    out->n[q][0] = n[0] * inv; out->n[q][1] = n[1] * inv; out->n[q][2] = n[2] * inv;
+  }
+  out->count = FJ_LH_PLANES;
+  out->reach = FJ_LC_REACH * gap - ext;
+  return FJ_LH_PLANES;
+}
+
+FJ_LC_FN uint32_t light_hull_verify(const DLightCone *C, const double *Pl, const double *P)
+{
+  const double w[3] = {P[0] - Pl[0], P[1] - Pl[1], P[2] - Pl[2]};
+  const double lim = -FJ_LH_SLACK * ((lc_abs(w[0]) + lc_abs(w[1])) + lc_abs(w[2]));
+  uint32_t bad = 0;
+  for (int q = 0; q < FJ_LH_PLANES; q++)
+    if (!(C->n[q][0] * w[0] + C->n[q][1] * w[1] + C->n[q][2] * w[2] <= lim)) bad |= 1u << q;
+  return bad;
+}
+FJ_LC_FN void light_hull_widen(LightHullAcc *A, uint32_t bad)
+{
+  const int order[FJ_LH_PLANES] = {0, 2, 4, 1, 3, 5};
+  for (int q = 0; q < FJ_LH_PLANES; q++) if (bad & (1u << q)) A->push[order[q]] *= 16.;
+}
+
+FJ_LC_FN int light_hull_build(const double *Pl, const double *P, int64_t n, const double *b, DLightCone *out)
+{
+  for (int j = 0; j < FJ_LC_MAX_PLANES; j++) out->n[j][0] = out->n[j][1] = out->n[j][2] = 0.;
+  out->reach = 0.; out->count = 0; out->pad = 0;
+  if (n <= 0) return 0;
+  double ctr[3] = {0., 0., 0.};
+  for (int64_t i = 0; i < n; i++) for (int k = 0; k < 3; k++) ctr[k] += P[3 * i + k];
+  for (int k = 0; k < 3; k++) ctr[k] /= (double) n;
+  LightHullAcc A;
+  light_hull_frame(Pl, ctr, &A);
+  for (int64_t i = 0; i < n && A.ok; i++) light_hull_add(&A, P + 3 * i);
+  for (int round = 0; round <= FJ_LH_WIDENINGS; round++) {
+    if (!light_hull_finish(&A, b, out)) return 0;
+    uint32_t bad = 0;
+    for (int64_t i = 0; i < n; i++) bad |= light_hull_verify(out, Pl, P + 3 * i);
+    if (!bad) return out->count;
+    light_hull_widen(&A, bad);
+  }
+  for (int j = 0; j < FJ_LC_MAX_PLANES; j++) out->n[j][0] = out->n[j][1] = out->n[j][2] = 0.;
+  out->reach = 0.; out->count = 0;
+  return 0;
+}
+
+#endif
diff --git a/fujiyama-renderer_amd/csrc/device/fjgpu_types.h b/fujiyama-renderer_amd/csrc/device/fjgpu_types.h
--- a/fujiyama-renderer_amd/csrc/device/fjgpu_types.h
+++ b/fujiyama-renderer_amd/csrc/device/fjgpu_types.h
@@ -204,6 +204,8 @@
   const DLightSample *light_samples;
   const DLightCone *light_cones;
   const int32_t *cone_rows;
+  const DLightCone *light_hulls;
+  const int32_t *hull_rows;
   DLightHair *lrec_hair;
   uint32_t shadow_queue_cap;
   uint32_t cam_slot0;
@@ -306,7 +308,7 @@
   unsigned long long nodes, prims, insts, traced, squeued;
   unsigned long long sh_nodes, sh_prims, sh_insts;
   unsigned long long stack_peak, sh_stack_peak;
-  unsigned long long pad0_[1];
+  unsigned long long hull_settled;
   uint32_t next_count;
   uint32_t light_count;
   uint32_t overflow;
diff --git a/fujiyama-renderer_amd/gpu.py b/fujiyama-renderer_amd/gpu.py
--- a/fujiyama-renderer_amd/gpu.py
+++ b/fujiyama-renderer_amd/gpu.py
@@ -292,6 +292,24 @@
     _check(min(0, L.fjgpu_host_instance_level(scene_desc_ptr, group, inst.ctypes.data_as(C.c_void_p), skip.ctypes.data_as(C.c_void_p),
                                               box.ctypes.data_as(C.c_void_p), n)))
     return inst, skip, box
+
+
+LIGHT_HULL = np.dtype([("n", np.float64, (6, 3)), ("reach", np.float64), ("count", np.int32), ("pad", np.int32)])
+
+
+def host_light_hulls(scene_desc_ptr, group):
+    L = lib()
+    L.fjgpu_host_light_hulls.argtypes = [C.c_void_p, C.c_int, C.c_void_p, C.c_void_p, C.c_int, C.c_void_p]
+    L.fjgpu_host_light_hulls.restype = C.c_int
+    n = L.fjgpu_host_light_hulls(scene_desc_ptr, group, None, None, 0, None)
+    if n < 0:
+        _check(n)
+    rec = np.zeros(n, dtype=LIGHT_HULL)
+    Pl = np.zeros((n, 3), dtype=np.float64)
+    M = np.zeros((3, 4), dtype=np.float64)
+    _check(min(0, L.fjgpu_host_light_hulls(scene_desc_ptr, group, rec.ctypes.data_as(C.c_void_p), Pl.ctypes.data_as(C.c_void_p), n,
+                                           M.ctypes.data_as(C.c_void_p))))
+    return rec, Pl, M
 
 
 DENOISE_ITERATIONS = 5
diff --git a/include/fjgpu.h b/include/fjgpu.h
--- a/include/fjgpu.h
+++ b/include/fjgpu.h
@@ -168,6 +168,8 @@
 
 int fjgpu_host_instance_level(const fj_scene_desc *desc, int group, int32_t *out_inst, int32_t *out_skip, double *out_box, int cap);
 
+int fjgpu_host_light_hulls(const fj_scene_desc *desc, int group, void *out_records, double *out_Pl, int cap, double *out_M);
+
 int fjgpu_scene_query(const fjgpu_scene *scene, const char *name, double *value);
 
 void fjgpu_host_make_transform(int transform_order, int rotate_order, const double *trs9, double *M16, double *Minv16);
```

Result: faster. 40060 Mray/s, median of 6 (+7.2%).
